# selftok-team/SelftokTokenizer

Measured on AMD Instinct MI355X. Metric: images/sec encode+decode, 256x256 512-token, higher is better.
Workload: dtype f32

## Files before the change

include/selftok_hip_ext.h:

```cpp
#ifndef SELFTOK_HIP_EXT_H
#define SELFTOK_HIP_EXT_H

#include "selftok_hip.h"

#ifdef __cplusplus
extern "C" {
#endif

int selftok_attn_kmask_f32(const selftok_attn_desc* desc, const unsigned* kmask, long kmask_bs, hipStream_t stream);

int selftok_ex_attention_kmask_f32(const float* q, long qs, const float* k1, const float* v1, long kvs1, int Tk1, int valid1, int rows1, const float* k2, const float* v2,
                                   long kvs2, int Tk2, float* out, void* workspace, int B, int H, int Tq, int D, const unsigned* kmask, long kmask_bs, hipStream_t stream);
int selftok_ex_attention_kmask_fused_f32(const float* q, long qs, const float* k1, const float* v1, long kvs1, int Tk1, int valid1, int rows1, const float* k2, const float* v2,
                                         long kvs2, int Tk2, float* out, int B, int H, int Tq, int D, const unsigned* kmask, long kmask_bs, hipStream_t stream);

size_t selftok_img_resize_crop_norm_u8_workspace_bytes(const long* table_host, int B, int S);
int selftok_img_resize_tables_layout(const long* table_host, int B, int S, long* layout4);
int selftok_img_resize_crop_norm_u8(const unsigned char* packed, size_t packed_bytes, const long* table_host, const long* table_dev, int B, int S, void* out,
                                    int out_bf16, const void* lut, void* workspace, size_t workspace_bytes, hipStream_t stream);

size_t selftok_img_views_u8_workspace_bytes(const long* views_host, int V, int S);
int selftok_img_views_tables_layout(const long* views_host, int V, int S, long* layout4);
int selftok_img_views_u8(const unsigned char* packed, size_t packed_bytes, const long* views_host, const long* views_dev, int V, int S, void* out, int out_bf16,
                         const void* lut, void* workspace, size_t workspace_bytes, hipStream_t stream);

size_t selftok_img_views_filter_u8_workspace_bytes(const long* views_host, int V, int S, int filter);
int selftok_img_views_filter_tables_layout(const long* views_host, int V, int S, int filter, long* layout4);
int selftok_img_views_filter_u8(const unsigned char* packed, size_t packed_bytes, const long* views_host, const long* views_dev, int V, int S, int filter, void* out,
                                int out_bf16, const void* lut, void* workspace, size_t workspace_bytes, hipStream_t stream);

size_t selftok_img_resize_u8_workspace_bytes(const long* frames_host, int N, int filter);
int selftok_img_resize_u8(unsigned char* packed, size_t packed_bytes, const long* frames_host, const long* frames_dev, int N, int filter, void* workspace,
                          size_t workspace_bytes, hipStream_t stream);

int selftok_img_to_u8(const void* img, int in_bf16, unsigned char* out, int B, int H, int W, hipStream_t stream);

size_t selftok_img_metrics_workspace_bytes(int B, int H, int W);
int selftok_img_metrics(const void* recon, int recon_bf16, const void* orig, int orig_bf16, int orig_signed, int quantize, const double* window11_host, double* out,
                        void* workspace, size_t workspace_bytes, int B, int H, int W, hipStream_t stream);

size_t selftok_vq_topk_workspace_bytes(int N, int C, int k);
int selftok_vq_topk_packed_f32(const float* z, const float* packed, void* ids, float* scores, void* workspace,
                               int N, int C, int D, int k, int flags, hipStream_t stream);

int selftok_linear_f16_split(const void* a_blk, const void* packed, const float* bias, float* out, void* out_blk, long ldo,
                             int M, int N, int K, int flags, int* overflow, hipStream_t stream);
int selftok_linear_f16_split_residual(const void* a_blk, const void* packed, const float* bias,
                                      const float* resid, long ldr, const float* gate, long gate_stride_b, long gate_stride_t, int T,
                                      float* out, long ldo, int M, int N, int K, int* overflow, hipStream_t stream);

int selftok_linear_f16_split_k(const void* a_blk, const void* packed, const float* bias, float* out, void* out_blk, long ldo,
                               int M, int N, int K, int flags, int ksplit, void* workspace, int* overflow, hipStream_t stream);
int selftok_linear_f16_split_residual_k(const void* a_blk, const void* packed, const float* bias,
                                        const float* resid, long ldr, const float* gate, long gate_stride_b, long gate_stride_t, int T,
                                        float* out, long ldo, int M, int N, int K, int ksplit, void* workspace, int* overflow, hipStream_t stream);

int selftok_attn_f16(const selftok_attn_desc* desc, const unsigned* kmask, long kmask_bs, hipStream_t stream);

size_t selftok_lpips_conv2d_packed_floats(int Cin, int Cout, int KH, int KW);
int selftok_lpips_conv2d_f32(const float* in, const float* packed, const float* bias, float* out, int N, int H, int W, int Cin, int Cout,
                             int KH, int KW, int stride, int pad, int relu, hipStream_t stream);
int selftok_lpips_maxpool3s2_f32(const float* in, float* out, int N, int H, int W, int C, hipStream_t stream);
int selftok_lpips_input(const void* recon, int recon_bf16, const void* orig, int orig_bf16, int orig_signed, int quantize, float* out,
                        int B, int H, int W, hipStream_t stream);
size_t selftok_lpips_distance_workspace_bytes(int B, int npix);
int selftok_lpips_distance(const float* feat, const float* w, double* out, void* workspace, size_t workspace_bytes, int B, int npix, int C,
                           int accumulate, hipStream_t stream);

int selftok_lpips_maxpool2s2_f32(const float* in, float* out, int N, int H, int W, int C, hipStream_t stream);

size_t selftok_img_ssim_workspace_bytes(int B, int H, int W, int taps);
int selftok_img_ssim(const void* recon, int recon_bf16, const void* orig, int orig_bf16, int orig_signed, int quantize, const double* window_host, int taps,
                     double cov_norm, int signed_range, double* out, void* workspace, size_t workspace_bytes, int B, int H, int W, hipStream_t stream);

int selftok_fid_conv2d_f32(const float* in, const float* packed, const float* bias, float* out, int N, int H, int W, int Cin, int Cout,
                           int KH, int KW, int stride, int pad_h, int pad_w, int ldo, int co_off, int relu, hipStream_t stream);
int selftok_fid_pool3_f32(const float* in, float* out, int N, int H, int W, int C, int mode, int ldo, int co_off, hipStream_t stream);
int selftok_fid_input(const void* src, int src_bf16, int src_signed, int quantize, float* out, int B, int H, int W, int OH, int OW,
                      const int* ytab, const int* xtab, hipStream_t stream);
int selftok_fid_spatial_mean_f32(const float* in, float* out, int N, int npix, int C, hipStream_t stream);
size_t selftok_fid_stats_workspace_bytes(int N, int D);
int selftok_fid_stats(const float* x, double* mu, double* sigma, void* workspace, size_t workspace_bytes, int N, int D, hipStream_t stream);

size_t selftok_knn_radius_f32_workspace_bytes(int N, int D, int k);
int selftok_knn_radius_f32(const float* a, float* r2, void* workspace, size_t workspace_bytes, int N, int D, int k, int split, hipStream_t stream);
size_t selftok_manifold_member_f32_workspace_bytes(int M, int N, int D);
int selftok_manifold_member_f32(const float* x, const float* a, const float* r2, int* member, void* workspace, size_t workspace_bytes, int M, int N, int D,
                                int split, hipStream_t stream);
size_t selftok_is_colmean_workspace_bytes(int N, int C, int split_size);
int selftok_is_colmean(const float* logits, double* colmean, void* workspace, size_t workspace_bytes, int N, int C, int split_size, hipStream_t stream);
size_t selftok_is_kl_rows_workspace_bytes(int N, int C, int split_size);
int selftok_is_kl_rows(const float* logits, const double* colmean, double* kl, void* workspace, size_t workspace_bytes, int N, int C, int split_size,
                       hipStream_t stream);

size_t selftok_manifold_count_nn_f32_workspace_bytes(int M, int N, int D);
int selftok_manifold_count_nn_f32(const float* x, const float* a, const float* r2, int* count, float* nn_d2, int* nn_idx, void* workspace, size_t workspace_bytes,
                                  int M, int N, int D, int split, hipStream_t stream);
size_t selftok_kid_sums_f32_workspace_bytes(int S, int m, int D);
int selftok_kid_sums_f32(const float* xs, const float* ys, double* sums, void* workspace, size_t workspace_bytes, int S, int m, int D, hipStream_t stream);

int selftok_stream_prepare(const int* step, const int* limit, const float* coef, const unsigned* pattern_words, const float* mod_table,
                           const float* mod_table_uncond, const int* segs_host, int n_segs, unsigned* kwords_out, float* coef_out,
                           float* mods_out, float* mods_uncond_out, int B, int K, int n_steps, long R, hipStream_t stream);
int selftok_unpatchify_cfg_euler_rows_f32(const float* y_cond, const float* y_uncond, const float* x, float* x_out, const float* coef_rows,
                                          const int* step, int* step_out, int B, int C, int hp, int wp, float cfg_scale, int x0_param,
                                          hipStream_t stream);

#ifdef __cplusplus
}
#endif

#endif
```

selftoktokenizer_amd/_lib.py:

```python
from __future__ import annotations

import ctypes as C
import os

_HERE = os.path.dirname(os.path.abspath(__file__))
LIB_PATH = os.environ.get("SELFTOK_HIP_LIB") or os.path.join(_HERE, "libselftok_hip.so")

_vp, _i, _f, _sz, _l, _d = C.c_void_p, C.c_int, C.c_float, C.c_size_t, C.c_long, C.c_double

SIGNATURES = {
    "selftok_version": (_i, []),
    "selftok_last_error": (C.c_char_p, []),
    "selftok_vq_workspace_bytes": (_sz, [_i, _i]),
    "selftok_vq_encode_f32": (_i, [_vp, _vp, _vp, _vp, _vp, _i, _i, _i, _i, _vp]),
    "selftok_vq_packed_bytes": (_sz, [_i, _i]),
    "selftok_vq_pack_codebook": (_i, [_vp, _vp, _i, _i, _vp]),
    "selftok_vq_encode_packed_f32": (_i, [_vp, _vp, _vp, _vp, _vp, _i, _i, _i, _i, _vp]),
    "selftok_vq_argmax_partial_packed_f32": (_i, [_vp, _vp, _vp, _vp, _i, _i, _i, _i, _vp]),
    "selftok_vq_finalize_packed": (_i, [_vp, _vp, _vp, _vp, _vp, _i, _i, _i, _i, _i, _vp]),
    "selftok_vq_ema_accumulate_f32": (_i, [_vp, _vp, _vp, _vp, _i, _i, _i, _i, _vp]),
    "selftok_vq_tpc_update_f32": (_i, [_vp, _vp, _i, _i, _i, _f, _i, _vp]),
    "selftok_vq_softmax_workspace_bytes": (_sz, [_i]),
    "selftok_vq_softmax_stats_f32": (_i, [_vp, _vp, _vp, _vp, _vp, _i, _i, _i, _i, _f, _i, _vp]),
    "selftok_vq_softmax_backward_f32": (_i, [_vp, _vp, _vp, _vp, _vp, _vp, _i, _i, _i, _i, _f, _i, _vp]),
    "selftok_code_gather_ln_f32": (_i, [_vp, _vp, _vp, _vp, _vp, _i, _i, _i, _f, _i, _vp]),
    "selftok_residual_ln_mod_f32": (_i, [_vp] * 7 + [_i, _i, _i, _l, _l, _l, _l, _f, _vp]),
    "selftok_bias_gelu_f32": (_i, [_vp, _vp, _l, _i, _vp]),
    "selftok_silu_f32": (_i, [_vp, _vp, _l, _vp]),
    "selftok_add_rows_f32": (_i, [_vp, _vp, _vp, _i, _l, _vp]),
    "selftok_timestep_embed_f32": (_i, [_vp, _vp, _vp, _i, _i, _f, _vp]),
    "selftok_patchify_f32": (_i, [_vp, _vp, _i, _i, _i, _i, _vp]),
    "selftok_unpatchify_cfg_euler_f32": (_i, [_vp] * 5 + [_i, _i, _i, _i, _f, _f, _vp]),
    "selftok_rmsnorm_f32": (_i, [_vp, _vp, _vp, _l, _i, _f, _vp]),
    "selftok_rotary_f32": (_i, [_vp, _vp, _vp, _l, _i, _i, _f, _vp]),
    "selftok_attn_f32": (_i, [_vp, _vp]),
    "selftok_residual_ln_mod_split": (_i, [_vp] * 8 + [_i, _i, _i, _l, _l, _l, _l, _f, _vp]),
    "selftok_linear_f16x2_packed_bytes": (_sz, [_i, _i]),
    "selftok_linear_f16x2_pack_weight": (_i, [_vp, _vp, _i, _i, _vp, _vp]),
    "selftok_linear_f16x2_f32": (_i, [_vp, _l, _vp, _vp, _vp, _l, _i, _i, _i, _i, _vp, _vp]),
    "selftok_split_f16x2_bytes": (_sz, [_l, _i]),
    "selftok_split_f16x2_f32": (_i, [_vp, _l, _vp, _l, _i, _vp, _vp]),
    "selftok_linear_f16x2_split": (_i, [_vp, _vp, _vp, _vp, _vp, _l, _i, _i, _i, _i, _vp, _vp]),
    "selftok_linear_f16x2_split_residual": (_i, [_vp, _vp, _vp, _vp, _l, _vp, _l, _l, _i, _vp, _l, _i, _i, _i, _vp, _vp]),
    "selftok_linear_f16x2_splitk_workspace_bytes": (_sz, [_i, _i, _i]),
    "selftok_linear_f16x2_split_k": (_i, [_vp, _vp, _vp, _vp, _vp, _l, _i, _i, _i, _i, _i, _vp, _vp, _vp]),
    "selftok_linear_f16x2_split_residual_k": (_i, [_vp, _vp, _vp, _vp, _l, _vp, _l, _l, _i, _vp, _l, _i, _i, _i, _i, _vp, _vp, _vp]),
    "selftok_groupnorm_silu_bf16": (_i, [_vp, _vp, _vp, _vp, _i, _i, _i, _i, _f, _i, _vp]),
    "selftok_latent_process_in": (_i, [_vp, _vp, _i, _i, _i, _i, _f, _f, _vp]),
    "selftok_latent_process_out": (_i, [_vp, _vp, _l, _f, _f, _vp]),
    "selftok_clamp01_bf16": (_i, [_vp, _l, _vp]),
    "selftok_conv2d_packed_bytes": (_sz, [_i, _i, _i, _i]),
    "selftok_conv2d_pack_weight_bf16": (_i, [_vp, _vp, _i, _i, _i, _i, _vp]),
    "selftok_conv2d_nhwc_bf16": (_i, [_vp, _vp, _vp, _vp, _vp] + [_i] * 11 + [_vp]),
    "selftok_groupnorm_nhwc_workspace_bytes": (_sz, [_i, _i, _i]),
    "selftok_groupnorm_silu_nhwc_bf16": (_i, [_vp, _vp, _vp, _vp, _vp, _i, _i, _i, _i, _f, _i, _vp]),
    "selftok_vx_conv2d_bf16": (_i, [_vp] * 5 + [_i] * 9 + [_vp]),
    "selftok_vx_groupnorm_workspace_bytes": (_sz, [_i, _i, _i]),
    "selftok_vx_groupnorm_bf16": (_i, [_vp] * 7 + [_i, _i, _i, _i, C.c_double, _vp]),
    "selftok_vx_silu_table_bf16": (_i, [_vp, _vp]),
    "selftok_vx_attention_workspace_bytes": (_sz, [_i, _i, _i]),
    "selftok_vx_attention_bf16": (_i, [_vp] * 5 + [_i, _i, _i, _vp]),
    "selftok_vx_expf_f32": (_i, [_vp, _vp, _l, _vp]),
    "selftok_ex_linear_f32": (_i, [_vp, _l, _vp, _vp, _vp, _l, _i, _vp, _l, _i, _vp, _l, _l, _i, _i, _i, _vp]),
    "selftok_linear_f32_workspace_bytes": (_sz, [_l, _i, _i, _i]),
    "selftok_linear_f32": (_i, [_vp, _l, _vp, _vp, _vp, _l, _i, _vp, _l, _i, _vp, _l, _l, _i, _i, _i, _vp, _sz, _vp]),
    "selftok_ex_layernorm_mod_f32": (_i, [_vp, _l, _vp, _l, _vp, _vp, _l, _i, _vp, _vp, _vp, _l, _i, _f, _vp]),
    "selftok_ex_res_layernorm_mod_f32": (_i, [_vp, _l, _vp, _l, _vp, _vp, _l, _i, _vp, _l, _vp, _l, _vp, _vp, _l, _i, _l, _i, _f, _vp]),
    "selftok_ex_unary_f32": (_i, [_vp, _vp, _l, _i, _vp]),
    "selftok_ex_attention_workspace_bytes": (_sz, [_i, _i, _i, _i, _i]),
    "selftok_ex_attention_f32": (_i, [_vp, _l, _vp, _vp, _l, _i, _i, _i, _vp, _vp, _l, _i, _vp, _vp, _i, _i, _i, _i, _vp]),
    "selftok_ex_attention_fused_supported": (_i, [_i, _i, _i]),
    "selftok_ex_attention_fused_f32": (_i, [_vp, _l, _vp, _vp, _l, _i, _i, _i, _vp, _vp, _l, _i, _vp, _i, _i, _i, _i, _vp]),
}


EXT_SIGNATURES = {
    "selftok_attn_kmask_f32": (_i, [_vp, _vp, _l, _vp]),
    "selftok_ex_attention_kmask_f32": (_i, [_vp, _l, _vp, _vp, _l, _i, _i, _i, _vp, _vp, _l, _i, _vp, _vp, _i, _i, _i, _i, _vp, _l, _vp]),
    "selftok_ex_attention_kmask_fused_f32": (_i, [_vp, _l, _vp, _vp, _l, _i, _i, _i, _vp, _vp, _l, _i, _vp, _i, _i, _i, _i, _vp, _l, _vp]),
    "selftok_img_resize_crop_norm_u8_workspace_bytes": (_sz, [_vp, _i, _i]),
    "selftok_img_resize_tables_layout": (_i, [_vp, _i, _i, _vp]),
    "selftok_img_resize_crop_norm_u8": (_i, [_vp, _sz, _vp, _vp, _i, _i, _vp, _i, _vp, _vp, _sz, _vp]),
    "selftok_img_views_u8_workspace_bytes": (_sz, [_vp, _i, _i]),
    "selftok_img_views_tables_layout": (_i, [_vp, _i, _i, _vp]),
    "selftok_img_views_u8": (_i, [_vp, _sz, _vp, _vp, _i, _i, _vp, _i, _vp, _vp, _sz, _vp]),
    "selftok_img_views_filter_u8_workspace_bytes": (_sz, [_vp, _i, _i, _i]),
    "selftok_img_views_filter_tables_layout": (_i, [_vp, _i, _i, _i, _vp]),
    "selftok_img_views_filter_u8": (_i, [_vp, _sz, _vp, _vp, _i, _i, _i, _vp, _i, _vp, _vp, _sz, _vp]),
    "selftok_img_resize_u8_workspace_bytes": (_sz, [_vp, _i, _i]),
    "selftok_img_resize_u8": (_i, [_vp, _sz, _vp, _vp, _i, _i, _vp, _sz, _vp]),
    "selftok_img_to_u8": (_i, [_vp, _i, _vp, _i, _i, _i, _vp]),
    "selftok_img_metrics_workspace_bytes": (_sz, [_i, _i, _i]),
    "selftok_img_metrics": (_i, [_vp, _i, _vp, _i, _i, _i, _vp, _vp, _vp, _sz, _i, _i, _i, _vp]),
    "selftok_vq_topk_workspace_bytes": (_sz, [_i, _i, _i]),
    "selftok_vq_topk_packed_f32": (_i, [_vp, _vp, _vp, _vp, _vp, _i, _i, _i, _i, _i, _vp]),
    "selftok_linear_f16_split": (_i, [_vp, _vp, _vp, _vp, _vp, _l, _i, _i, _i, _i, _vp, _vp]),
    "selftok_linear_f16_split_residual": (_i, [_vp, _vp, _vp, _vp, _l, _vp, _l, _l, _i, _vp, _l, _i, _i, _i, _vp, _vp]),
    "selftok_linear_f16_split_k": (_i, [_vp, _vp, _vp, _vp, _vp, _l, _i, _i, _i, _i, _i, _vp, _vp, _vp]),
    "selftok_linear_f16_split_residual_k": (_i, [_vp, _vp, _vp, _vp, _l, _vp, _l, _l, _i, _vp, _l, _i, _i, _i, _i, _vp, _vp, _vp]),
    "selftok_attn_f16": (_i, [_vp, _vp, _l, _vp]),
    "selftok_lpips_conv2d_packed_floats": (_sz, [_i, _i, _i, _i]),
    "selftok_lpips_conv2d_f32": (_i, [_vp, _vp, _vp, _vp] + [_i] * 10 + [_vp]),
    "selftok_lpips_maxpool3s2_f32": (_i, [_vp, _vp, _i, _i, _i, _i, _vp]),
    "selftok_lpips_input": (_i, [_vp, _i, _vp, _i, _i, _i, _vp, _i, _i, _i, _vp]),
    "selftok_lpips_distance_workspace_bytes": (_sz, [_i, _i]),
    "selftok_lpips_distance": (_i, [_vp, _vp, _vp, _vp, _sz, _i, _i, _i, _i, _vp]),
    "selftok_lpips_maxpool2s2_f32": (_i, [_vp, _vp, _i, _i, _i, _i, _vp]),
    "selftok_img_ssim_workspace_bytes": (_sz, [_i, _i, _i, _i]),
    "selftok_img_ssim": (_i, [_vp, _i, _vp, _i, _i, _i, _vp, _i, _d, _i, _vp, _vp, _sz, _i, _i, _i, _vp]),
    "selftok_fid_conv2d_f32": (_i, [_vp, _vp, _vp, _vp] + [_i] * 13 + [_vp]),
    "selftok_fid_pool3_f32": (_i, [_vp, _vp] + [_i] * 7 + [_vp]),
    "selftok_fid_input": (_i, [_vp, _i, _i, _i, _vp, _i, _i, _i, _i, _i, _vp, _vp, _vp]),
    "selftok_fid_spatial_mean_f32": (_i, [_vp, _vp, _i, _i, _i, _vp]),
    "selftok_fid_stats_workspace_bytes": (_sz, [_i, _i]),
    "selftok_fid_stats": (_i, [_vp, _vp, _vp, _vp, _sz, _i, _i, _vp]),
    "selftok_knn_radius_f32_workspace_bytes": (_sz, [_i, _i, _i]),
    "selftok_knn_radius_f32": (_i, [_vp, _vp, _vp, _sz, _i, _i, _i, _i, _vp]),
    "selftok_manifold_member_f32_workspace_bytes": (_sz, [_i, _i, _i]),
    "selftok_manifold_member_f32": (_i, [_vp, _vp, _vp, _vp, _vp, _sz, _i, _i, _i, _i, _vp]),
    "selftok_is_colmean_workspace_bytes": (_sz, [_i, _i, _i]),
    "selftok_is_colmean": (_i, [_vp, _vp, _vp, _sz, _i, _i, _i, _vp]),
    "selftok_is_kl_rows_workspace_bytes": (_sz, [_i, _i, _i]),
    "selftok_is_kl_rows": (_i, [_vp, _vp, _vp, _vp, _sz, _i, _i, _i, _vp]),
    "selftok_manifold_count_nn_f32_workspace_bytes": (_sz, [_i, _i, _i]),
    "selftok_manifold_count_nn_f32": (_i, [_vp, _vp, _vp, _vp, _vp, _vp, _vp, _sz, _i, _i, _i, _i, _vp]),
    "selftok_kid_sums_f32_workspace_bytes": (_sz, [_i, _i, _i]),
    "selftok_kid_sums_f32": (_i, [_vp, _vp, _vp, _vp, _sz, _i, _i, _i, _vp]),
    "selftok_stream_prepare": (_i, [_vp] * 7 + [_i] + [_vp] * 4 + [_i, _i, _i, _l, _vp]),
    "selftok_unpatchify_cfg_euler_rows_f32": (_i, [_vp] * 7 + [_i, _i, _i, _i, _f, _i, _vp]),
}


class AttnSeg(C.Structure):
    _fields_ = [("q", _vp), ("k", _vp), ("v", _vp), ("o", _vp), ("len", _i),
                ("q_rs", _l), ("k_rs", _l), ("v_rs", _l), ("o_rs", _l),
                ("q_bs", _l), ("k_bs", _l), ("v_bs", _l), ("o_bs", _l)]


class AttnDesc(C.Structure):
    _fields_ = [("seg", AttnSeg * 2), ("B", _i), ("H", _i), ("head_dim", _i), ("kvis", _vp),
                ("seg0_sees_seg1", _i), ("scale", _f), ("mode", _i), ("overflow", _vp),
                ("o_blk", _vp * 2)]

_lib = None


class SelftokHipError(RuntimeError):
    pass


def load():
    global _lib
    if _lib is None:
        if not os.path.exists(LIB_PATH):
            raise SelftokHipError(
                f"{LIB_PATH} not found: build it with `python -c 'import __graft_entry__ as g; g.build()'` "
                "(hipcc --offload-arch=gfx950). There is no CPU fallback.")
        lib = C.CDLL(LIB_PATH)
        for name, (res, args) in list(SIGNATURES.items()) + list(EXT_SIGNATURES.items()):
            fn = getattr(lib, name)
            fn.restype = res
            fn.argtypes = args
        _lib = lib
    return _lib


def check(rc: int, what: str):
    if rc != 0:
        msg = load().selftok_last_error().decode("utf-8", "replace")
        raise SelftokHipError(f"{what} failed (rc={rc}): {msg}")
```

selftoktokenizer_amd/csrc/gemm_f16.hip:

```cpp
#include "common.h"
#include "gemm_split_shared.h"
#include "selftok_hip_ext.h"

namespace selftok {

constexpr int H_A = PA_P;
constexpr int H_W = W_P;
constexpr int H_W_BASE = 2 * H_A;
constexpr int H_STAGE = 2 * (H_A + H_W);
constexpr int H_STAGES = 3;
constexpr int H_LDS_BYTES = H_STAGES * H_STAGE;

template <int ACT, int OSPLIT, int RES>
__global__ __launch_bounds__(512, 2) void linear_f16_pre_kernel(const _Float16* __restrict__ Ablk,
                                                                const _Float16* __restrict__ Wp, const float* __restrict__ bias,
                                                                float* __restrict__ out, _Float16* __restrict__ oblk, long ldo,
                                                                int M, int N, int K, int* __restrict__ overflow, int mblocks, int nblocks, ResArgs res)
{
    static_assert(!(OSPLIT && RES), "the residual form writes fp32");
    __shared__ __attribute__((aligned(16))) unsigned char smem[H_LDS_BYTES];

    const int tid = threadIdx.x, lane = tid & 63, wave = __builtin_amdgcn_readfirstlane(tid >> 6);
    const int wm = wave >> 1, wn = wave & 1;
    const int l31 = lane & 31, lh = lane >> 5;

    int mb, nb;
    tile_of_workgroup(mblocks, nblocks, mb, nb);
    const int m0 = mb * BM, n0 = nb * BN;
    const int KT = K / BK, KL = KT - 1;
    const int NI = (KT + 1) >> 1, IL = NI - 1;

    const int d_g = (lane & 3) ^ ((lane >> 4) & 3);
    const unsigned a_off = (unsigned)((lane >> 2) * 64 + d_g * 16);
    const int rb_last = (M - 1) >> 4;
    int rb0 = m0 / 16 + wave, rb1 = rb0 + 8;
    rb0 = rb0 < rb_last ? rb0 : rb_last;
    rb1 = rb1 < rb_last ? rb1 : rb_last;
    const unsigned char* const a_base[2] = {(const unsigned char*)Ablk + (size_t)rb0 * KT * 2048, (const unsigned char*)Ablk + (size_t)rb1 * KT * 2048};
    const unsigned char* const w_base = (const unsigned char*)Wp + (size_t)nb * KT * W_BYTES + (size_t)wave * 1024;
    const unsigned w_off = lane * 16;
    const unsigned lds0 = (unsigned)(size_t)(__attribute__((address_space(3))) unsigned char*)smem;
    auto dma = [&](int it, int stage) {
        const unsigned dst = lds0 + stage * H_STAGE + wave * 1024;
#pragma unroll
        for (int h = 0; h < 2; ++h) {
            int kt = 2 * it + h;
            kt = kt < KL ? kt : KL;
            lds_dma16(a_base[0] + (size_t)kt * 2048, a_off, dst + h * H_A);
            lds_dma16(a_base[1] + (size_t)kt * 2048, a_off, dst + h * H_A + 8192);
            lds_dma16(w_base + (size_t)kt * W_BYTES, w_off, dst + H_W_BASE + h * H_W);
        }
    };

    f32x16v acc[2][2];
#pragma unroll
    for (int i = 0; i < 2; ++i)
#pragma unroll
        for (int j = 0; j < 2; ++j) acc[i][j] = f32x16v{0, 0, 0, 0, 0, 0, 0, 0, 0, 0, 0, 0, 0, 0, 0, 0};

    const int a_frag = (wm * 64 + l31) * PA_ROW + ((lh ^ ((l31 >> 2) & 3)) * 16);
    const int w_frag = H_W_BASE + lh * W_G + (wn * 64 + l31) * 16;
    f16x8 af[4][2], wf[4][2];
    auto read_frags = [&](int stage) {
#pragma unroll
        for (int q = 0; q < 4; ++q) {
            const unsigned char* sa = smem + stage * H_STAGE + (q >> 1) * H_A + (a_frag ^ ((q & 1) * 32));
            const unsigned char* sw = smem + stage * H_STAGE + (q >> 1) * H_W + w_frag + (q & 1) * 2 * W_G;
#pragma unroll
            for (int b = 0; b < 2; ++b) {
                af[q][b] = *reinterpret_cast<const f16x8*>(sa + b * 32 * PA_ROW);
                wf[q][b] = *reinterpret_cast<const f16x8*>(sw + b * 32 * 16);
            }
        }
    };
    auto mfma_step = [&](int q) {
#pragma unroll
        for (int i = 0; i < 2; ++i)
#pragma unroll
            for (int j = 0; j < 2; ++j) acc[i][j] = __builtin_amdgcn_mfma_f32_32x32x16_f16(wf[q][j], af[q][i], acc[i][j], 0, 0, 0);
    };

    dma(0, 0);
    dma(1, 1);
    __builtin_amdgcn_sched_barrier(0);
    asm volatile("s_waitcnt vmcnt(6)" ::: "memory");
    __builtin_amdgcn_s_barrier();
    __builtin_amdgcn_sched_barrier(0);

    const int grp = wave >> 2;
    if (grp) __builtin_amdgcn_s_barrier();
    if (grp) __builtin_amdgcn_s_setprio(1);
    int sc = 0;
    for (int it = 0; it < NI; ++it) {
        const int s1 = sc == 2 ? 0 : sc + 1, s2 = s1 == 2 ? 0 : s1 + 1;
        __builtin_amdgcn_sched_barrier(0);
        read_frags(sc);
        __builtin_amdgcn_sched_barrier(0);
        dma(it + 2, s2);
        __builtin_amdgcn_sched_barrier(0);
        asm volatile("s_waitcnt vmcnt(6) lgkmcnt(0)" ::: "memory");
        __builtin_amdgcn_s_barrier();
        __builtin_amdgcn_sched_barrier(0);
        mfma_step(0);
        mfma_step(1);
        if (2 * it + 1 < KT) {
            mfma_step(2);
            mfma_step(3);
        }
        __builtin_amdgcn_sched_barrier(0);
        if (!(grp && it == IL)) __builtin_amdgcn_s_barrier();
        sc = s1;
    }
    asm volatile("s_waitcnt vmcnt(0)" ::: "memory");

    constexpr int STG_ROW = OSPLIT ? 144 : 272, STG_PLANE = 64 * STG_ROW;
    static_assert(8 * (OSPLIT ? 2 * STG_PLANE : STG_PLANE) <= H_LDS_BYTES, "epilogue slices exceed the ring");
    unsigned char* stg = smem + wave * (OSPLIT ? 2 * STG_PLANE : STG_PLANE);
    __syncthreads();
    float chk = 0.f;
#pragma unroll
    for (int j = 0; j < 2; ++j) {
#pragma unroll
        for (int g = 0; g < 4; ++g) {
            const int cl = j * 32 + 8 * g + 4 * lh, col = n0 + wn * 64 + cl;
            const float4 bv = bias ? *reinterpret_cast<const float4*>(bias + col) : make_float4(0.f, 0.f, 0.f, 0.f);
#pragma unroll
            for (int i = 0; i < 2; ++i) {
                const int rl = i * 32 + l31, row = m0 + wm * 64 + rl;
                float v[4];
#pragma unroll
                for (int c = 0; c < 4; ++c) {
                    v[c] = acc[i][j][4 * g + c] + 0.f + (c == 0 ? bv.x : c == 1 ? bv.y : c == 2 ? bv.z : bv.w);
                    if (ACT == 1) v[c] = gelu_tanh_f(v[c]);
                }
                if (OSPLIT) {
                    f16x4 h, l;
                    split4(make_float4(opaque_f32(v[0]), opaque_f32(v[1]), opaque_f32(v[2]), opaque_f32(v[3])), h, l);
                    *reinterpret_cast<f16x4*>(stg + rl * STG_ROW + cl * 2) = h;
                    *reinterpret_cast<f16x4*>(stg + STG_PLANE + rl * STG_ROW + cl * 2) = l;
                    if (row < M) {
#pragma unroll
                        for (int c = 0; c < 4; ++c) chk = __builtin_fmaf((float)h[c], 0.f, chk);
                    }
                } else {
                    *reinterpret_cast<float4*>(stg + rl * STG_ROW + cl * 4) = make_float4(v[0], v[1], v[2], v[3]);
                    if (row < M) {
#pragma unroll
                        for (int c = 0; c < 4; ++c) chk = __builtin_fmaf(v[c], 0.f, chk);
                    }
                }
            }
        }
    }
    if (OSPLIT) {
#pragma unroll
        for (int p = 0; p < 2; ++p)
#pragma unroll
            for (int pass = 0; pass < 8; ++pass) {
                const int rl = pass * 8 + (lane >> 3), seg = lane & 7, row = m0 + wm * 64 + rl;
                const f16x8 val = *reinterpret_cast<const f16x8*>(stg + p * STG_PLANE + rl * STG_ROW + seg * 16);
                if (row < M) *reinterpret_cast<f16x8*>(oblk + split_blk_index(row, n0 + wn * 64 + seg * 8, p, N / 32)) = val;
            }
    } else {
#pragma unroll
        for (int pass = 0; pass < 16; ++pass) {
            const int rl = pass * 4 + (lane >> 4), seg = lane & 15, row = m0 + wm * 64 + rl;
            float4 val = *reinterpret_cast<const float4*>(stg + rl * STG_ROW + seg * 16);
            if (row < M) {
                const int col = n0 + wn * 64 + seg * 4;
                if (RES) {
                    const float4 r = *reinterpret_cast<const float4*>(res.resid + (size_t)row * res.ldr + col);
                    if (res.gate) {
                        const int b = row / res.T, t = row - b * res.T;
                        const float4 g = *reinterpret_cast<const float4*>(res.gate + b * res.gsb + t * res.gst + col);
                        val.x = r.x + g.x * val.x; val.y = r.y + g.y * val.y; val.z = r.z + g.z * val.z; val.w = r.w + g.w * val.w;
                    } else {
                        val.x += r.x; val.y += r.y; val.z += r.z; val.w += r.w;
                    }
                }
                *reinterpret_cast<float4*>(out + (size_t)row * ldo + col) = val;
            }
        }
    }
    if (overflow && chk != 0.f) atomicOr(overflow, 1);
}

}

using namespace selftok;

extern "C" {

int selftok_linear_f16_split(const void* a_blk, const void* packed, const float* bias, float* out, void* out_blk, long ldo,
                             int M, int N, int K, int flags, int* overflow, hipStream_t stream)
{
    const int rc = check_split_linear("linear_f16_split", a_blk, packed, bias, out, out_blk, ldo, M, N, K);
    if (rc != SELFTOK_OK || M == 0) return rc;
    const bool osplit = out_blk != nullptr;
    const int mblocks = (M + BM - 1) / BM, nblocks = N / BN;
    const dim3 grid((unsigned)(mblocks * nblocks));
    const _Float16* ab = (const _Float16*)a_blk;
    _Float16* ob = (_Float16*)out_blk;
#define F16_LAUNCH(ACT, OS) hipLaunchKernelGGL((linear_f16_pre_kernel<ACT, OS, 0>), grid, dim3(512), 0, stream, ab, (const _Float16*)packed, bias, out, ob, ldo, M, N, K, overflow, mblocks, nblocks, ResArgs{})
    if (flags & SELFTOK_LINEAR_GELU) { if (osplit) F16_LAUNCH(1, 1); else F16_LAUNCH(1, 0); }
    else { if (osplit) F16_LAUNCH(0, 1); else F16_LAUNCH(0, 0); }
#undef F16_LAUNCH
    return check_launch("linear_f16_pre_kernel");
}

int selftok_linear_f16_split_residual(const void* a_blk, const void* packed, const float* bias,
                                      const float* resid, long ldr, const float* gate, long gate_stride_b, long gate_stride_t, int T,
                                      float* out, long ldo, int M, int N, int K, int* overflow, hipStream_t stream)
{
    const int rc = check_split_linear_residual("linear_f16_split_residual", a_blk, packed, bias, resid, ldr, gate, gate_stride_b, gate_stride_t, T, out, ldo, M, N, K);
    if (rc != SELFTOK_OK || M == 0) return rc;
    const int mblocks = (M + BM - 1) / BM, nblocks = N / BN;
    hipLaunchKernelGGL((linear_f16_pre_kernel<0, 0, 1>), dim3((unsigned)(mblocks * nblocks)), dim3(512), 0, stream,
                       (const _Float16*)a_blk, (const _Float16*)packed, bias, out, (_Float16*)nullptr, ldo,
                       M, N, K, overflow, mblocks, nblocks, ResArgs{resid, ldr, gate, gate_stride_b, gate_stride_t, T});
    return check_launch("linear_f16_pre_kernel(residual)");
}

}
```

selftoktokenizer_amd/csrc/gemm_f16_splitk.hip:

```cpp
#include "common.h"
#include "gemm_split_shared.h"
#include "selftok_hip_ext.h"

namespace selftok {

constexpr int HK_A = PA_P;
constexpr int HK_W = W_P;
constexpr int HK_W_BASE = 2 * HK_A;
constexpr int HK_STAGE = 2 * (HK_A + HK_W);
constexpr int HK_LDS_BYTES = 3 * HK_STAGE;

__global__ __launch_bounds__(512, 2) void linear_f16_splitk_partial_kernel(const _Float16* __restrict__ Ablk, const _Float16* __restrict__ Wp,
                                                                           float* __restrict__ ws, int M, int N, int K,
                                                                           int* __restrict__ overflow, int mblocks, int nblocks)
{
    __shared__ __attribute__((aligned(16))) unsigned char smem[HK_LDS_BYTES];

    const int tid = threadIdx.x, lane = tid & 63, wave = __builtin_amdgcn_readfirstlane(tid >> 6);
    const int wm = wave >> 1, wn = wave & 1;
    const int l31 = lane & 31, lh = lane >> 5;

    int mb, nb;
    tile_of_workgroup(mblocks, nblocks, mb, nb);
    const int m0 = mb * BM, n0 = nb * BN;
    const int KTA = K / BK;
    const int KT = KTA / (int)gridDim.y, KL = KT - 1;
    const int kt_off = (int)blockIdx.y * KT;
    const int NI = (KT + 1) >> 1, IL = NI - 1;
    float* const out = ws + (size_t)blockIdx.y * M * N;

    const int d_g = (lane & 3) ^ ((lane >> 4) & 3);
    const unsigned a_off = (unsigned)((lane >> 2) * 64 + d_g * 16);
    const int rb_last = (M - 1) >> 4;
    int rb0 = m0 / 16 + wave, rb1 = rb0 + 8;
    rb0 = rb0 < rb_last ? rb0 : rb_last;
    rb1 = rb1 < rb_last ? rb1 : rb_last;
    const unsigned char* const a_base[2] = {(const unsigned char*)Ablk + ((size_t)rb0 * KTA + kt_off) * 2048,
                                            (const unsigned char*)Ablk + ((size_t)rb1 * KTA + kt_off) * 2048};
    const unsigned char* const w_base = (const unsigned char*)Wp + ((size_t)nb * KTA + kt_off) * W_BYTES + (size_t)wave * 1024;
    const unsigned w_off = lane * 16;
    const unsigned lds0 = (unsigned)(size_t)(__attribute__((address_space(3))) unsigned char*)smem;
    auto dma = [&](int it, int stage) {
        const unsigned dst = lds0 + stage * HK_STAGE + wave * 1024;
#pragma unroll
        for (int h = 0; h < 2; ++h) {
            int kt = 2 * it + h;
            kt = kt < KL ? kt : KL;
            lds_dma16(a_base[0] + (size_t)kt * 2048, a_off, dst + h * HK_A);
            lds_dma16(a_base[1] + (size_t)kt * 2048, a_off, dst + h * HK_A + 8192);
            lds_dma16(w_base + (size_t)kt * W_BYTES, w_off, dst + HK_W_BASE + h * HK_W);
        }
    };

    f32x16v acc[2][2];
#pragma unroll
    for (int i = 0; i < 2; ++i)
#pragma unroll
        for (int j = 0; j < 2; ++j) acc[i][j] = f32x16v{0, 0, 0, 0, 0, 0, 0, 0, 0, 0, 0, 0, 0, 0, 0, 0};

    const int a_frag = (wm * 64 + l31) * PA_ROW + ((lh ^ ((l31 >> 2) & 3)) * 16);
    const int w_frag = HK_W_BASE + lh * W_G + (wn * 64 + l31) * 16;
    f16x8 af[4][2], wf[4][2];
    auto read_frags = [&](int stage) {
#pragma unroll
        for (int q = 0; q < 4; ++q) {
            const unsigned char* sa = smem + stage * HK_STAGE + (q >> 1) * HK_A + (a_frag ^ ((q & 1) * 32));
            const unsigned char* sw = smem + stage * HK_STAGE + (q >> 1) * HK_W + w_frag + (q & 1) * 2 * W_G;
#pragma unroll
            for (int b = 0; b < 2; ++b) {
                af[q][b] = *reinterpret_cast<const f16x8*>(sa + b * 32 * PA_ROW);
                wf[q][b] = *reinterpret_cast<const f16x8*>(sw + b * 32 * 16);
            }
        }
    };
    auto mfma_step = [&](int q) {
#pragma unroll
        for (int i = 0; i < 2; ++i)
#pragma unroll
            for (int j = 0; j < 2; ++j) acc[i][j] = __builtin_amdgcn_mfma_f32_32x32x16_f16(wf[q][j], af[q][i], acc[i][j], 0, 0, 0);
    };

    dma(0, 0);
    dma(1, 1);
    __builtin_amdgcn_sched_barrier(0);
    asm volatile("s_waitcnt vmcnt(6)" ::: "memory");
    __builtin_amdgcn_s_barrier();
    __builtin_amdgcn_sched_barrier(0);

    const int grp = wave >> 2;
    if (grp) __builtin_amdgcn_s_barrier();
    if (grp) __builtin_amdgcn_s_setprio(1);
    int sc = 0;
    for (int it = 0; it < NI; ++it) {
        const int s1 = sc == 2 ? 0 : sc + 1, s2 = s1 == 2 ? 0 : s1 + 1;
        __builtin_amdgcn_sched_barrier(0);
        read_frags(sc);
        __builtin_amdgcn_sched_barrier(0);
        dma(it + 2, s2);
        __builtin_amdgcn_sched_barrier(0);
        asm volatile("s_waitcnt vmcnt(6) lgkmcnt(0)" ::: "memory");
        __builtin_amdgcn_s_barrier();
        __builtin_amdgcn_sched_barrier(0);
        mfma_step(0);
        mfma_step(1);
        if (2 * it + 1 < KT) {
            mfma_step(2);
            mfma_step(3);
        }
        __builtin_amdgcn_sched_barrier(0);
        if (!(grp && it == IL)) __builtin_amdgcn_s_barrier();
        sc = s1;
    }
    asm volatile("s_waitcnt vmcnt(0)" ::: "memory");

    constexpr int STG_ROW = 272, STG_PLANE = 64 * STG_ROW;
    static_assert(8 * STG_PLANE <= HK_LDS_BYTES, "store slices exceed the ring");
    unsigned char* stg = smem + wave * STG_PLANE;
    __syncthreads();
    float chk = 0.f;
#pragma unroll
    for (int j = 0; j < 2; ++j) {
#pragma unroll
        for (int g = 0; g < 4; ++g) {
            const int cl = j * 32 + 8 * g + 4 * lh;
#pragma unroll
            for (int i = 0; i < 2; ++i) {
                const int rl = i * 32 + l31, row = m0 + wm * 64 + rl;
                float v[4];
#pragma unroll
                for (int c = 0; c < 4; ++c) v[c] = acc[i][j][4 * g + c] + 0.f + 0.f;
                *reinterpret_cast<float4*>(stg + rl * STG_ROW + cl * 4) = make_float4(v[0], v[1], v[2], v[3]);
                if (row < M) {
#pragma unroll
                    for (int c = 0; c < 4; ++c) chk = __builtin_fmaf(v[c], 0.f, chk);
                }
            }
        }
    }
#pragma unroll
    for (int pass = 0; pass < 16; ++pass) {
        const int rl = pass * 4 + (lane >> 4), seg = lane & 15, row = m0 + wm * 64 + rl;
        const float4 val = *reinterpret_cast<const float4*>(stg + rl * STG_ROW + seg * 16);
        if (row < M) *reinterpret_cast<float4*>(out + (size_t)row * N + n0 + wn * 64 + seg * 4) = val;
    }
    if (overflow && chk != 0.f) atomicOr(overflow, 1);
}

static int launch_f16_partials(const void* a_blk, const void* packed, float* ws, int M, int N, int K, int ksplit, int* overflow, hipStream_t stream)
{
    const int mblocks = (M + BM - 1) / BM, nblocks = N / BN;
    hipLaunchKernelGGL(linear_f16_splitk_partial_kernel, dim3((unsigned)(mblocks * nblocks), (unsigned)ksplit), dim3(512), 0, stream,
                       (const _Float16*)a_blk, (const _Float16*)packed, ws, M, N, K, overflow, mblocks, nblocks);
    return check_launch("linear_f16_splitk_partial_kernel");
}

}

using namespace selftok;

extern "C" {

int selftok_linear_f16_split_k(const void* a_blk, const void* packed, const float* bias, float* out, void* out_blk, long ldo,
                               int M, int N, int K, int flags, int ksplit, void* workspace, int* overflow, hipStream_t stream)
{
    if (ksplit == 1) return selftok_linear_f16_split(a_blk, packed, bias, out, out_blk, ldo, M, N, K, flags, overflow, stream);
    int rc = check_split_linear("linear_f16_split_k", a_blk, packed, bias, out, out_blk, ldo, M, N, K);
    if (rc != SELFTOK_OK || M == 0) return rc;
    if ((rc = check_splitk("linear_f16_split_k", K, ksplit, workspace))) return rc;
    float* ws = (float*)workspace;
    if ((rc = launch_f16_partials(a_blk, packed, ws, M, N, K, ksplit, overflow, stream))) return rc;
    return launch_splitk_finish(ws, ksplit, bias, out, out_blk, ldo, M, N, flags, overflow, nullptr, stream);
}

int selftok_linear_f16_split_residual_k(const void* a_blk, const void* packed, const float* bias,
                                        const float* resid, long ldr, const float* gate, long gate_stride_b, long gate_stride_t, int T,
                                        float* out, long ldo, int M, int N, int K, int ksplit, void* workspace, int* overflow, hipStream_t stream)
{
    if (ksplit == 1)
        return selftok_linear_f16_split_residual(a_blk, packed, bias, resid, ldr, gate, gate_stride_b, gate_stride_t, T, out, ldo, M, N, K, overflow, stream);
    int rc = check_split_linear_residual("linear_f16_split_residual_k", a_blk, packed, bias, resid, ldr, gate, gate_stride_b, gate_stride_t, T, out, ldo, M, N, K);
    if (rc != SELFTOK_OK || M == 0) return rc;
    if ((rc = check_splitk("linear_f16_split_residual_k", K, ksplit, workspace))) return rc;
    float* ws = (float*)workspace;
    if ((rc = launch_f16_partials(a_blk, packed, ws, M, N, K, ksplit, overflow, stream))) return rc;
    const ResArgs res{resid, ldr, gate, gate_stride_b, gate_stride_t, T};
    return launch_splitk_finish(ws, ksplit, bias, out, nullptr, ldo, M, N, 0, overflow, &res, stream);
}

}
```

selftoktokenizer_amd/csrc/gemm_split.hip:

```cpp
#include "common.h"
#include "gemm_split_shared.h"
#include "selftok_hip.h"
#include <stdlib.h>

namespace selftok {

constexpr int A_G = BM * 16 + 32;
constexpr int A_P = 4 * A_G;
constexpr int A_BYTES = 2 * A_P;
constexpr int A_STAGES = 2;
constexpr int W_STAGES = 5;
constexpr int W_AHEAD = 3;
constexpr int W_BASE = A_STAGES * A_BYTES;
constexpr int LDS_BYTES = W_BASE + W_STAGES * W_BYTES;

__global__ __launch_bounds__(256) void pack_weight_kernel(const float* __restrict__ W, _Float16* __restrict__ packed, int N, int K, int* __restrict__ overflow)
{
    const long idx = (long)blockIdx.x * blockDim.x + threadIdx.x;
    const int KG = K / 8;
    if (idx >= (long)N * KG) return;
    const int n = (int)(idx / KG), kg = (int)(idx % KG);
    const float4 v0 = *reinterpret_cast<const float4*>(W + (size_t)n * K + kg * 8);
    const float4 v1 = *reinterpret_cast<const float4*>(W + (size_t)n * K + kg * 8 + 4);
    f16x4 h0, l0, h1, l1;
    float mx = 0.f;
    split4(v0, h0, l0, mx);
    split4(v1, h1, l1, mx);
    const int nb = n / BN, nl = n % BN, kt = kg / 4, g = kg % 4, KT = K / BK;
    _Float16* tile = packed + ((size_t)nb * KT + kt) * (W_BYTES / 2);
    f16x8 hi = {h0[0], h0[1], h0[2], h0[3], h1[0], h1[1], h1[2], h1[3]};
    f16x8 lo = {l0[0], l0[1], l0[2], l0[3], l1[0], l1[1], l1[2], l1[3]};
    *reinterpret_cast<f16x8*>(tile + (size_t)g * (W_G / 2) + nl * 8) = hi;
    *reinterpret_cast<f16x8*>(tile + (W_P / 2) + (size_t)g * (W_G / 2) + nl * 8) = lo;
    if (!(mx < F16_MAX) && overflow) atomicOr(overflow, 2);
}

template <int ACT, int ABL = 0>
__global__ __launch_bounds__(512, 2) void linear_f16x2_kernel(const float* __restrict__ A, long lda, const _Float16* __restrict__ Wp,
                                                              const float* __restrict__ bias, float* __restrict__ out, long ldo,
                                                              int M, int N, int K, int* __restrict__ overflow, int mblocks, int nblocks)
{
    __shared__ __attribute__((aligned(16))) unsigned char smem[LDS_BYTES];

    const int tid = threadIdx.x, lane = tid & 63, wave = tid >> 6;
    const int wm = wave >> 1, wn = wave & 1;
    const int l31 = lane & 31, lh = lane >> 5;

    int mb, nb;
    tile_of_workgroup(mblocks, nblocks, mb, nb);
    const int m0 = mb * BM, n0 = nb * BN;
    const int KT = K / BK, KL = KT - 1;

    const int a_q = tid & 7, a_r = tid >> 3;
    const float* a_src[4];
#pragma unroll
    for (int i = 0; i < 4; ++i) {
        int row = m0 + a_r + 64 * i;
        row = row < M ? row : M - 1;
        a_src[i] = A + (size_t)row * lda + 4 * a_q;
    }
    const int a_dst = (a_q >> 1) * A_G + a_r * 16 + (a_q & 1) * 8;
    const _Float16* w_src = Wp + (size_t)nb * KT * (W_BYTES / 2) + (size_t)wave * 512 + lane * 8;

    f32x4v preA[4], preB[4];
    auto load_a = [&](f32x4v (&pre)[4], int kt) {
        kt = kt < KL ? kt : KL;
#pragma unroll
        for (int i = 0; i < 4; ++i) {
            const float* p = a_src[i] + (size_t)kt * BK;
            asm volatile("global_load_dwordx4 %0, %1, off" : "=v"(pre[i]) : "v"(p) : "memory");
        }
    };
    auto wait_rows = [&](f32x4v (&pre)[4]) {
        if (ABL & 6) asm volatile("s_waitcnt vmcnt(0)" : "+v"(pre[0]), "+v"(pre[1]), "+v"(pre[2]), "+v"(pre[3])::"memory");
        else asm volatile("s_waitcnt vmcnt(6)" : "+v"(pre[0]), "+v"(pre[1]), "+v"(pre[2]), "+v"(pre[3])::"memory");
    };
    auto dma_w = [&](int kt, int stage) {
        kt = kt < KL ? kt : KL;
        const _Float16* src = w_src + (size_t)kt * (W_BYTES / 2);
        unsigned char* dst = smem + W_BASE + stage * W_BYTES + wave * 1024;
        __builtin_amdgcn_global_load_lds((const __attribute__((address_space(1))) void*)src,
                                         (__attribute__((address_space(3))) void*)dst, 16, 0, 0);
        __builtin_amdgcn_global_load_lds((const __attribute__((address_space(1))) void*)(src + 8 * 512),
                                         (__attribute__((address_space(3))) void*)(dst + 8 * 1024), 16, 0, 0);
    };
    auto write_a = [&](f32x4v (&pre)[4], int stage) {
        unsigned char* base = smem + stage * A_BYTES + a_dst;
#pragma unroll
        for (int i = 0; i < 4; ++i) {
            f16x4 h, l;
            split4(pre[i], h, l);
            *reinterpret_cast<f16x4*>(base + i * 64 * 16) = h;
            *reinterpret_cast<f16x4*>(base + i * 64 * 16 + A_P) = l;
        }
    };

    f32x16v hi[2][2], lo[2][2];
#pragma unroll
    for (int i = 0; i < 2; ++i)
#pragma unroll
        for (int j = 0; j < 2; ++j) {
            hi[i][j] = f32x16v{0, 0, 0, 0, 0, 0, 0, 0, 0, 0, 0, 0, 0, 0, 0, 0};
            lo[i][j] = hi[i][j];
        }

    const int a_frag = lh * A_G + (wm * 64 + l31) * 16;
    const int w_frag = W_BASE + lh * W_G + (wn * 64 + l31) * 16;
    f16x8 af0[2][2], wf0[2][2], af1[2][2], wf1[2][2];
    auto read_frags = [&](f16x8 (&af)[2][2], f16x8 (&wf)[2][2], int a_stage, int w_stage, int s) {
        const unsigned char* sa = smem + a_stage * A_BYTES + a_frag + s * 2 * A_G;
        const unsigned char* sw = smem + w_stage * W_BYTES + w_frag + s * 2 * W_G;
#pragma unroll
        for (int b = 0; b < 2; ++b)
#pragma unroll
            for (int p = 0; p < 2; ++p) {
                af[b][p] = *reinterpret_cast<const f16x8*>(sa + b * 32 * 16 + p * A_P);
                wf[b][p] = *reinterpret_cast<const f16x8*>(sw + b * 32 * 16 + p * W_P);
            }
    };
    auto mfma_row = [&](int i, f16x8 (&af)[2][2], f16x8 (&wf)[2][2]) {
#pragma unroll
            for (int j = 0; j < 2; ++j) {
                hi[i][j] = __builtin_amdgcn_mfma_f32_32x32x16_f16(af[i][0], wf[j][0], hi[i][j], 0, 0, 0);
                lo[i][j] = __builtin_amdgcn_mfma_f32_32x32x16_f16(af[i][0], wf[j][1], lo[i][j], 0, 0, 0);
                lo[i][j] = __builtin_amdgcn_mfma_f32_32x32x16_f16(af[i][1], wf[j][0], lo[i][j], 0, 0, 0);
            }
    };

    auto iteration = [&](int kt, f32x4v (&pre)[4], int ws_cur, int ws_next, int ws_new) {
        const int as = kt & 1;
        if (!(ABL & 16)) read_frags(af1, wf1, as, ws_cur, 1);
        if (!(ABL & 8)) mfma_row(0, af0, wf0);
        __builtin_amdgcn_sched_barrier(0);
        wait_rows(pre);
        if (!(ABL & 1)) write_a(pre, as ^ 1);
        if (!(ABL & 8)) mfma_row(1, af0, wf0);
        __builtin_amdgcn_sched_barrier(0);
        asm volatile("s_waitcnt lgkmcnt(0)" ::: "memory");
        __builtin_amdgcn_s_barrier();
        __builtin_amdgcn_sched_barrier(0);
        if (!(ABL & 8)) mfma_row(0, af1, wf1);
        __builtin_amdgcn_sched_barrier(0);
        if (!(ABL & 16)) read_frags(af0, wf0, as ^ 1, ws_next, 0);
        if (!(ABL & 4)) dma_w(kt + W_AHEAD, ws_new);
        __builtin_amdgcn_sched_barrier(0);
        if (!(ABL & 2)) load_a(pre, kt + 3);
        if (!(ABL & 8)) mfma_row(1, af1, wf1);
        __builtin_amdgcn_sched_barrier(0);
    };

    dma_w(0, 0);
    load_a(preA, 0);
    asm volatile("s_waitcnt vmcnt(0)" : "+v"(preA[0]), "+v"(preA[1]), "+v"(preA[2]), "+v"(preA[3])::"memory");
    __builtin_amdgcn_sched_barrier(0);
    write_a(preA, 0);
    __builtin_amdgcn_sched_barrier(0);
    dma_w(1, 1);
    __builtin_amdgcn_sched_barrier(0);
    load_a(preB, 1);
    __builtin_amdgcn_sched_barrier(0);
    dma_w(2, 2);
    __builtin_amdgcn_sched_barrier(0);
    load_a(preA, 2);
    __builtin_amdgcn_sched_barrier(0);
    asm volatile("s_waitcnt lgkmcnt(0)" ::: "memory");
    __builtin_amdgcn_s_barrier();
    read_frags(af0, wf0, 0, 0, 0);

    auto ring = [](int x) { return x >= W_STAGES ? x - W_STAGES : x; };
    int wc = 0;
    int kt = 0;
    for (; kt + 1 < KT; kt += 2) {
        iteration(kt, preB, wc, ring(wc + 1), ring(wc + W_AHEAD));
        wc = ring(wc + 1);
        iteration(kt + 1, preA, wc, ring(wc + 1), ring(wc + W_AHEAD));
        wc = ring(wc + 1);
    }
    if (kt < KT) iteration(kt, preB, wc, ring(wc + 1), ring(wc + W_AHEAD));
    asm volatile("s_waitcnt vmcnt(0)" : "+v"(preA[0]), "+v"(preA[1]), "+v"(preA[2]), "+v"(preA[3]), "+v"(preB[0]), "+v"(preB[1]), "+v"(preB[2]), "+v"(preB[3])::"memory");

    float chk = 0.f;
#pragma unroll
    for (int j = 0; j < 2; ++j) {
        const int col = n0 + wn * 64 + j * 32 + l31;
        const float bv = bias ? bias[col] : 0.f;
#pragma unroll
        for (int i = 0; i < 2; ++i) {
            const int rbase = m0 + wm * 64 + i * 32 + 4 * lh;
#pragma unroll
            for (int r = 0; r < 16; ++r) {
                const int row = rbase + (r & 3) + 8 * (r >> 2);
                float v = hi[i][j][r] + lo[i][j][r] * LO_INV + bv;
                if (ACT == 1) v = gelu_tanh_f(v);
                if (row < M) { out[(size_t)row * ldo + col] = v; chk = __builtin_fmaf(v, 0.f, chk); }
            }
        }
    }
    if (overflow && chk != 0.f) atomicOr(overflow, 1);
}

constexpr int PA_BYTES = 2 * PA_P;
constexpr int PA_STAGES = 3, PW_STAGES = 4;
constexpr int PW_BASE = PA_STAGES * PA_BYTES;
constexpr int P_LDS_BYTES = PW_BASE + PW_STAGES * W_BYTES;

template <int ACT, int OSPLIT, int PP = 1, int ABL = 0, int RES = 0, int SK = 0>
__global__ __launch_bounds__(512, 2) void linear_f16x2_pre_kernel(const _Float16* __restrict__ Ablk,
                                                                  const _Float16* __restrict__ Wp, const float* __restrict__ bias,
                                                                  float* __restrict__ out, _Float16* __restrict__ oblk, long ldo,
                                                                  int M, int N, int K, int* __restrict__ overflow, int mblocks, int nblocks, ResArgs res)
{
    static_assert(!SK || (ACT == 0 && OSPLIT == 0 && RES == 0), "a split-K partial has no epilogue");
    __shared__ __attribute__((aligned(16))) unsigned char smem[P_LDS_BYTES];
    unsigned long long tk0 = 0, tk1 = 0, tk2 = 0, rt0 = 0;
    if (ABL & 2048) { tk0 = __builtin_readcyclecounter(); rt0 = __builtin_amdgcn_s_memrealtime(); }

    const int tid = threadIdx.x, lane = tid & 63, wave = __builtin_amdgcn_readfirstlane(tid >> 6);
    const int wm = wave >> 1, wn = wave & 1;
    const int l31 = lane & 31, lh = lane >> 5;

    int mb, nb;
    tile_of_workgroup(mblocks, nblocks, mb, nb);
    const int m0 = mb * BM, n0 = nb * BN;
    const int KTA = K / BK;
    const int KT = SK ? KTA / (int)gridDim.y : KTA, KL = KT - 1;
    const int kt_off = SK ? (int)blockIdx.y * KT : 0;
    if (SK) out += (size_t)blockIdx.y * M * ldo;

    const int d_g = (lane & 3) ^ ((lane >> 4) & 3);
    const unsigned a_off = (unsigned)((lane >> 2) * 64 + d_g * 16);
    const int rb_last = (M - 1) >> 4;
    int rb0 = m0 / 16 + wave, rb1 = rb0 + 8;
    rb0 = rb0 < rb_last ? rb0 : rb_last;
    rb1 = rb1 < rb_last ? rb1 : rb_last;
    const unsigned char* const a_base[2] = {(const unsigned char*)Ablk + ((size_t)rb0 * KTA + kt_off) * 2048, (const unsigned char*)Ablk + ((size_t)rb1 * KTA + kt_off) * 2048};
    const unsigned char* const w_base = (const unsigned char*)(Wp + ((size_t)nb * KTA + kt_off) * (W_BYTES / 2) + (size_t)wave * 512);
    const unsigned w_off = lane * 16;
    const unsigned lds0 = (unsigned)(size_t)(__attribute__((address_space(3))) unsigned char*)smem;
    auto dma_a = [&](int kt, int stage) {
        kt = kt < KL ? kt : KL;
        const unsigned dst = lds0 + stage * PA_BYTES + wave * 1024;
#pragma unroll
        for (int j = 0; j < 4; ++j) lds_dma16(a_base[j & 1] + (size_t)kt * 2048 + (j >> 1) * 1024, a_off, dst + (j & 1) * 8192 + (j >> 1) * PA_P);
    };
    auto dma_w = [&](int kt, int stage) {
        kt = kt < KL ? kt : KL;
        const unsigned char* src = w_base + (size_t)kt * W_BYTES;
        const unsigned dst = lds0 + PW_BASE + stage * W_BYTES + wave * 1024;
        lds_dma16(src, w_off, dst);
        lds_dma16(src + 8 * 1024, w_off, dst + 8 * 1024);
    };

    f32x16v hi[2][2], lo[2][2];
#pragma unroll
    for (int i = 0; i < 2; ++i)
#pragma unroll
        for (int j = 0; j < 2; ++j) {
            hi[i][j] = f32x16v{0, 0, 0, 0, 0, 0, 0, 0, 0, 0, 0, 0, 0, 0, 0, 0};
            lo[i][j] = hi[i][j];
        }

    const int a_frag = (wm * 64 + l31) * PA_ROW + ((lh ^ ((l31 >> 2) & 3)) * 16);
    const int w_frag = PW_BASE + lh * W_G + (wn * 64 + l31) * 16;
    f16x8 af0[2][2], wf0[2][2], af1[2][2], wf1[2][2];
    auto read_frags = [&](f16x8 (&af)[2][2], f16x8 (&wf)[2][2], int a_stage, int w_stage, int s) {
        const unsigned char* sa = smem + a_stage * PA_BYTES + (a_frag ^ (s * 32));
        const unsigned char* sw = smem + w_stage * W_BYTES + w_frag + s * 2 * W_G;
#pragma unroll
        for (int b = 0; b < 2; ++b)
#pragma unroll
            for (int p = 0; p < 2; ++p) {
                af[b][p] = *reinterpret_cast<const f16x8*>(sa + b * 32 * PA_ROW + p * PA_P);
                wf[b][p] = *reinterpret_cast<const f16x8*>(sw + b * 32 * 16 + p * W_P);
            }
    };
    auto mfma_row = [&](int i, f16x8 (&af)[2][2], f16x8 (&wf)[2][2]) {
#pragma unroll
            for (int j = 0; j < 2; ++j) {
                hi[i][j] = __builtin_amdgcn_mfma_f32_32x32x16_f16(wf[j][0], af[i][0], hi[i][j], 0, 0, 0);
                lo[i][j] = __builtin_amdgcn_mfma_f32_32x32x16_f16(wf[j][1], af[i][0], lo[i][j], 0, 0, 0);
                lo[i][j] = __builtin_amdgcn_mfma_f32_32x32x16_f16(wf[j][0], af[i][1], lo[i][j], 0, 0, 0);
            }
    };

    auto iteration = [&](int kt, int a_cur, int a_next, int a_new, int w_cur, int w_next, int w_new) {
        dma_a(kt + 2, a_new);
        dma_w(kt + 3, w_new);
        __builtin_amdgcn_sched_barrier(0);
        read_frags(af1, wf1, a_cur, w_cur, 1);
        mfma_row(0, af0, wf0);
        mfma_row(1, af0, wf0);
        __builtin_amdgcn_sched_barrier(0);
        asm volatile("s_waitcnt vmcnt(8) lgkmcnt(0)" ::: "memory");
        __builtin_amdgcn_s_barrier();
        __builtin_amdgcn_sched_barrier(0);
        mfma_row(0, af1, wf1);
        __builtin_amdgcn_sched_barrier(0);
        read_frags(af0, wf0, a_next, w_next, 0);
        mfma_row(1, af1, wf1);
        __builtin_amdgcn_sched_barrier(0);
    };

    dma_a(0, 0);
    dma_w(0, 0);
    dma_w(1, 1);
    dma_a(1, 1);
    dma_w(2, 2);
    __builtin_amdgcn_sched_barrier(0);
    asm volatile("s_waitcnt vmcnt(8)" ::: "memory");
    __builtin_amdgcn_s_barrier();
    __builtin_amdgcn_sched_barrier(0);

    int ac = 0, wc = 0;
    if (PP == 0) {
        read_frags(af0, wf0, 0, 0, 0);
        for (int kt = 0; kt < KT; ++kt) {
            const int a1 = ac == 2 ? 0 : ac + 1, a2 = a1 == 2 ? 0 : a1 + 1;
            iteration(kt, ac, a1, a2, wc, (wc + 1) & 3, (wc + 3) & 3);
            ac = a1;
            wc = (wc + 1) & 3;
        }
    } else {
        const int grp = wave >> 2;
        if (ABL & 2048) tk1 = __builtin_readcyclecounter();
        if (grp) __builtin_amdgcn_s_barrier();
        if (!(ABL & 64) && grp) __builtin_amdgcn_s_setprio(1);
        unsigned long long t0 = 0, t1 = 0, t2 = 0, t3 = 0, t4 = 0;
        unsigned acc_reads = 0, acc_vm = 0, acc_bar1 = 0, acc_mfma = 0, acc_bar2 = 0;
#define STAMP(t) do { if (ABL & 2048) { __builtin_amdgcn_sched_barrier(0); t = __builtin_readcyclecounter(); __builtin_amdgcn_sched_barrier(0); } } while (0)
        for (int kt = 0; kt < KT; ++kt) {
            const int a1 = ac == 2 ? 0 : ac + 1, a2 = a1 == 2 ? 0 : a1 + 1;
            STAMP(t0);
            if ((ABL & 2048) && kt > 0) acc_bar2 += (unsigned)(t0 - t4);
            __builtin_amdgcn_sched_barrier(0);
            if (!(ABL & 16)) {
                read_frags(af0, wf0, ac, wc, 0);
                read_frags(af1, wf1, ac, wc, 1);
            }
            __builtin_amdgcn_sched_barrier(0);
            if (!(ABL & 1)) dma_a(kt + 2, a2);
            if (!(ABL & 4)) dma_w(kt + 3, (wc + 3) & 3);
            __builtin_amdgcn_sched_barrier(0);
            if (ABL & 2048) {
                asm volatile("s_waitcnt lgkmcnt(0)" ::: "memory");
                STAMP(t1);
            }
            if (ABL & 5) asm volatile("s_waitcnt vmcnt(0) lgkmcnt(0)" ::: "memory");
            else asm volatile("s_waitcnt vmcnt(8) lgkmcnt(0)" ::: "memory");
            STAMP(t2);
            if (!(ABL & 32)) __builtin_amdgcn_s_barrier();
            STAMP(t3);
            __builtin_amdgcn_sched_barrier(0);
            if (!(ABL & 8)) {
                mfma_row(0, af0, wf0);
                mfma_row(1, af0, wf0);
                mfma_row(0, af1, wf1);
                mfma_row(1, af1, wf1);
            }
            __builtin_amdgcn_sched_barrier(0);
            STAMP(t4);
            if (ABL & 2048) { acc_reads += (unsigned)(t1 - t0); acc_vm += (unsigned)(t2 - t1); acc_bar1 += (unsigned)(t3 - t2); acc_mfma += (unsigned)(t4 - t3); }
            if (!(ABL & 32) && !(grp && kt == KL)) __builtin_amdgcn_s_barrier();
            ac = a1;
            wc = (wc + 1) & 3;
        }
#undef STAMP
        if (ABL & 2048) tk2 = __builtin_readcyclecounter();
        if ((ABL & 2048) && blockIdx.x == gridDim.x / 2 && lane == 0) {
            float* dbg = const_cast<float*>(bias) + N + wave * 8;
            dbg[0] = (float)acc_reads / KT; dbg[1] = (float)acc_vm / KT; dbg[2] = (float)acc_bar1 / KT;
            dbg[3] = (float)acc_mfma / KT; dbg[4] = (float)acc_bar2 / (KT - 1);
            dbg[5] = (float)(tk1 - tk0); dbg[6] = (float)(tk2 - tk1);
        }
    }
    asm volatile("s_waitcnt vmcnt(0)" ::: "memory");

    constexpr int STG_ROW = OSPLIT ? 144 : 272, STG_PLANE = 64 * STG_ROW;
    unsigned char* stg = smem + wave * (OSPLIT ? 2 * STG_PLANE : STG_PLANE);
    __syncthreads();
    float chk = 0.f;
#pragma unroll
    for (int j = 0; j < 2; ++j) {
#pragma unroll
        for (int g = 0; g < 4; ++g) {
            const int cl = j * 32 + 8 * g + 4 * lh, col = n0 + wn * 64 + cl;
            const float4 bv = bias ? *reinterpret_cast<const float4*>(bias + col) : make_float4(0.f, 0.f, 0.f, 0.f);
#pragma unroll
            for (int i = 0; i < 2; ++i) {
                const int rl = i * 32 + l31, row = m0 + wm * 64 + rl;
                float v[4];
#pragma unroll
                for (int c = 0; c < 4; ++c) {
                    v[c] = hi[i][j][4 * g + c] + lo[i][j][4 * g + c] * LO_INV + (c == 0 ? bv.x : c == 1 ? bv.y : c == 2 ? bv.z : bv.w);
                    if (ACT == 1) v[c] = gelu_tanh_f(v[c]);
                }
                if (OSPLIT) {
                    f16x4 h, l;
                    split4(make_float4(opaque_f32(v[0]), opaque_f32(v[1]), opaque_f32(v[2]), opaque_f32(v[3])), h, l);
                    *reinterpret_cast<f16x4*>(stg + rl * STG_ROW + cl * 2) = h;
                    *reinterpret_cast<f16x4*>(stg + STG_PLANE + rl * STG_ROW + cl * 2) = l;
                    if (row < M) {
#pragma unroll
                        for (int c = 0; c < 4; ++c) chk = __builtin_fmaf((float)h[c], 0.f, chk);
                    }
                } else {
                    *reinterpret_cast<float4*>(stg + rl * STG_ROW + cl * 4) = make_float4(v[0], v[1], v[2], v[3]);
                    if (row < M) {
#pragma unroll
                        for (int c = 0; c < 4; ++c) chk = __builtin_fmaf(v[c], 0.f, chk);
                    }
                }
            }
        }
    }
    if (OSPLIT) {
#pragma unroll
        for (int p = 0; p < 2; ++p)
#pragma unroll
            for (int pass = 0; pass < 8; ++pass) {
                const int rl = pass * 8 + (lane >> 3), seg = lane & 7, row = m0 + wm * 64 + rl;
                const f16x8 val = *reinterpret_cast<const f16x8*>(stg + p * STG_PLANE + rl * STG_ROW + seg * 16);
                if (row < M) *reinterpret_cast<f16x8*>(oblk + split_blk_index(row, n0 + wn * 64 + seg * 8, p, N / 32)) = val;
            }
    } else {
#pragma unroll
        for (int pass = 0; pass < 16; ++pass) {
            const int rl = pass * 4 + (lane >> 4), seg = lane & 15, row = m0 + wm * 64 + rl;
            float4 val = *reinterpret_cast<const float4*>(stg + rl * STG_ROW + seg * 16);
            if (row < M) {
                const int col = n0 + wn * 64 + seg * 4;
                if (RES) {
                    const float4 r = *reinterpret_cast<const float4*>(res.resid + (size_t)row * res.ldr + col);
                    if (res.gate) {
                        const int b = row / res.T, t = row - b * res.T;
                        const float4 g = *reinterpret_cast<const float4*>(res.gate + b * res.gsb + t * res.gst + col);
                        val.x = r.x + g.x * val.x; val.y = r.y + g.y * val.y; val.z = r.z + g.z * val.z; val.w = r.w + g.w * val.w;
                    } else {
                        val.x += r.x; val.y += r.y; val.z += r.z; val.w += r.w;
                    }
                }
                *reinterpret_cast<float4*>(out + (size_t)row * ldo + col) = val;
            }
        }
    }
    if (overflow && chk != 0.f) atomicOr(overflow, 1);
    if ((ABL & 2048) && blockIdx.x == gridDim.x / 2 && lane == 0) {
        asm volatile("s_waitcnt vmcnt(0)" ::: "memory");
        const_cast<float*>(bias)[N + wave * 8 + 7] = (float)(__builtin_readcyclecounter() - tk2);
    }
    if ((ABL & 2048) && overflow && tid == 0) {
        asm volatile("s_waitcnt vmcnt(0)" ::: "memory");
        int* rec = overflow + 8 + (size_t)blockIdx.x * 8;
        const unsigned long long rt1 = __builtin_amdgcn_s_memrealtime(), tk3 = __builtin_readcyclecounter();
        rec[0] = (int)(unsigned)rt0; rec[1] = (int)(unsigned)rt1; rec[2] = (int)(unsigned)(tk3 - tk0);
        rec[3] = (int)__builtin_amdgcn_s_getreg((31 << 11) | 4); rec[4] = (int)__builtin_amdgcn_s_getreg((31 << 11) | 20);
    }
}

__global__ __launch_bounds__(256) void split_rows_kernel(const float* __restrict__ x, long ld, _Float16* __restrict__ blk,
                                                         long rows, int cols, int* __restrict__ overflow)
{
    const long idx = (long)blockIdx.x * blockDim.x + threadIdx.x;
    const int c4 = cols / 4;
    if (idx >= rows * c4) return;
    const long r = idx / c4;
    const int c = (int)(idx % c4) * 4;
    const float4 v = *reinterpret_cast<const float4*>(x + r * ld + c);
    f16x4 h, l;
    float mx = 0.f;
    split4(v, h, l, mx);
    *reinterpret_cast<f16x4*>(blk + split_blk_index(r, c, 0, cols / 32)) = h;
    *reinterpret_cast<f16x4*>(blk + split_blk_index(r, c, 1, cols / 32)) = l;
    if (!(mx < F16_MAX) && overflow) atomicOr(overflow, 1);
}

template <int ACT, int OSPLIT, int RES>
__global__ __launch_bounds__(256) void splitk_finish_kernel(const float* __restrict__ ws, int S, const float* __restrict__ bias,
                                                            float* __restrict__ out, _Float16* __restrict__ oblk, long ldo,
                                                            int M, int N, int* __restrict__ overflow, ResArgs res)
{
    const long idx = (long)blockIdx.x * blockDim.x + threadIdx.x;
    const int n8 = N >> 3;
    if (idx >= (long)M * n8) return;
    const int row = (int)(idx / n8), col = (int)(idx - (long)row * n8) << 3;
    const float* p = ws + (size_t)row * N + col;
    const size_t plane = (size_t)M * N;
    float4 a = *reinterpret_cast<const float4*>(p), b = *reinterpret_cast<const float4*>(p + 4);
    for (int s_ = 1; s_ < S; ++s_) {
        const float4 c = *reinterpret_cast<const float4*>(p + s_ * plane), d = *reinterpret_cast<const float4*>(p + s_ * plane + 4);
        a.x += c.x; a.y += c.y; a.z += c.z; a.w += c.w;
        b.x += d.x; b.y += d.y; b.z += d.z; b.w += d.w;
    }
    float v[8] = {a.x, a.y, a.z, a.w, b.x, b.y, b.z, b.w};
    if (bias) {
        const float4 b0 = *reinterpret_cast<const float4*>(bias + col), b1 = *reinterpret_cast<const float4*>(bias + col + 4);
        v[0] += b0.x; v[1] += b0.y; v[2] += b0.z; v[3] += b0.w; v[4] += b1.x; v[5] += b1.y; v[6] += b1.z; v[7] += b1.w;
    }
    if (ACT == 1) {
#pragma unroll
        for (int c = 0; c < 8; ++c) v[c] = gelu_tanh_f(v[c]);
    }
    float chk = 0.f;
    if (OSPLIT) {
        f16x4 h0, l0, h1, l1;
        split4(make_float4(opaque_f32(v[0]), opaque_f32(v[1]), opaque_f32(v[2]), opaque_f32(v[3])), h0, l0);
        split4(make_float4(opaque_f32(v[4]), opaque_f32(v[5]), opaque_f32(v[6]), opaque_f32(v[7])), h1, l1);
        const f16x8 h = {h0[0], h0[1], h0[2], h0[3], h1[0], h1[1], h1[2], h1[3]}, l = {l0[0], l0[1], l0[2], l0[3], l1[0], l1[1], l1[2], l1[3]};
#pragma unroll
        for (int c = 0; c < 8; ++c) chk = __builtin_fmaf((float)h[c], 0.f, chk);
        *reinterpret_cast<f16x8*>(oblk + split_blk_index(row, col, 0, N / 32)) = h;
        *reinterpret_cast<f16x8*>(oblk + split_blk_index(row, col, 1, N / 32)) = l;
    } else {
#pragma unroll
        for (int c = 0; c < 8; ++c) chk = __builtin_fmaf(v[c], 0.f, chk);
        if (RES) {
            const float* rp = res.resid + (size_t)row * res.ldr + col;
            const float4 r0 = *reinterpret_cast<const float4*>(rp), r1 = *reinterpret_cast<const float4*>(rp + 4);
            const float r[8] = {r0.x, r0.y, r0.z, r0.w, r1.x, r1.y, r1.z, r1.w};
            if (res.gate) {
                const int bb = row / res.T, t = row - bb * res.T;
                const float* gp = res.gate + bb * res.gsb + t * res.gst + col;
                const float4 g0 = *reinterpret_cast<const float4*>(gp), g1 = *reinterpret_cast<const float4*>(gp + 4);
                const float g[8] = {g0.x, g0.y, g0.z, g0.w, g1.x, g1.y, g1.z, g1.w};
#pragma unroll
                for (int c = 0; c < 8; ++c) v[c] = r[c] + g[c] * v[c];
            } else {
#pragma unroll
                for (int c = 0; c < 8; ++c) v[c] += r[c];
            }
        }
        float* op = out + (size_t)row * ldo + col;
        *reinterpret_cast<float4*>(op) = make_float4(v[0], v[1], v[2], v[3]);
        *reinterpret_cast<float4*>(op + 4) = make_float4(v[4], v[5], v[6], v[7]);
    }
    if (overflow && chk != 0.f) atomicOr(overflow, 1);
}

static int launch_splitk_partials(const void* a_blk, const void* packed, float* ws, int M, int N, int K, int ksplit, int* overflow, hipStream_t stream)
{
    const int mblocks = (M + BM - 1) / BM, nblocks = N / BN;
    hipLaunchKernelGGL((linear_f16x2_pre_kernel<0, 0, 1, 0, 0, 1>), dim3((unsigned)(mblocks * nblocks), (unsigned)ksplit), dim3(512), 0, stream,
                       (const _Float16*)a_blk, (const _Float16*)packed, (const float*)nullptr, ws, (_Float16*)nullptr, (long)N,
                       M, N, K, overflow, mblocks, nblocks, ResArgs{});
    return check_launch("linear_f16x2_pre_kernel(split-K partials)");
}

}

using namespace selftok;

extern "C" {

size_t selftok_linear_f16x2_packed_bytes(int N, int K)
{
    if (N <= 0 || K <= 0 || N % BN || K % BK) return 0;
    return (size_t)N * K * 4;
}

int selftok_linear_f16x2_pack_weight(const float* W, void* packed, int N, int K, int* overflow, hipStream_t stream)
{
    if (!W || !packed || N <= 0 || K <= 0 || N % BN || K % BK) { set_last_error("linear_f16x2_pack_weight: need N % 128 == 0 and K % 32 == 0"); return SELFTOK_EINVAL; }
    const long n = (long)N * (K / 8);
    hipLaunchKernelGGL(pack_weight_kernel, dim3((unsigned)((n + 255) / 256)), dim3(256), 0, stream, W, (_Float16*)packed, N, K, overflow);
    return check_launch("pack_weight_kernel");
}

int selftok_linear_f16x2_f32(const float* A, long lda, const void* packed, const float* bias, float* out, long ldo,
                             int M, int N, int K, int flags, int* overflow, hipStream_t stream)
{
    if (M < 0 || N <= 0 || K <= 0 || N % BN || K % BK) { set_last_error("linear_f16x2: need N % 128 == 0 and K % 32 == 0"); return SELFTOK_EINVAL; }
    if (M == 0) return SELFTOK_OK;
    if (!A || !packed || !out || lda < K || ldo < N || (lda & 3)) { set_last_error("linear_f16x2: bad pointers/strides (lda % 4 == 0, lda >= K, ldo >= N)"); return SELFTOK_EINVAL; }
    const int mblocks = (M + BM - 1) / BM, nblocks = N / BN;
    const dim3 grid((unsigned)(mblocks * nblocks));
#ifdef SELFTOK_GEMM_ABLATE
    {
        const char* e = getenv("SELFTOK_GEMM_ABL");
        const int abl = e ? atoi(e) : 0;
#define ABL_CASE(v) if (abl == v) { hipLaunchKernelGGL((linear_f16x2_kernel<0, v>), grid, dim3(512), 0, stream, A, lda, (const _Float16*)packed, bias, out, ldo, M, N, K, overflow, mblocks, nblocks); return check_launch("linear_f16x2_kernel(ablated)"); }
        ABL_CASE(1) ABL_CASE(2) ABL_CASE(3) ABL_CASE(4) ABL_CASE(7) ABL_CASE(8) ABL_CASE(16) ABL_CASE(24) ABL_CASE(23) ABL_CASE(31)
#undef ABL_CASE
    }
#endif
    if (flags & SELFTOK_LINEAR_GELU)
        hipLaunchKernelGGL(linear_f16x2_kernel<1>, grid, dim3(512), 0, stream, A, lda, (const _Float16*)packed, bias, out, ldo, M, N, K, overflow, mblocks, nblocks);
    else
        hipLaunchKernelGGL(linear_f16x2_kernel<0>, grid, dim3(512), 0, stream, A, lda, (const _Float16*)packed, bias, out, ldo, M, N, K, overflow, mblocks, nblocks);
    return check_launch("linear_f16x2_kernel");
}

size_t selftok_split_f16x2_bytes(long rows, int cols)
{
    if (rows < 0 || cols <= 0 || cols % 32) return 0;
    return (size_t)((rows + 15) / 16) * 16 * cols * 4;
}

int selftok_split_f16x2_f32(const float* x, long ld, void* blk, long rows, int cols, int* overflow, hipStream_t stream)
{
    if (rows < 0 || cols <= 0 || (cols & 31) || (ld & 3) || ld < cols) { set_last_error("split_f16x2: cols % 32 == 0, ld % 4 == 0, ld >= cols"); return SELFTOK_EINVAL; }
    if (rows == 0) return SELFTOK_OK;
    if (!x || !blk || ((size_t)blk & 15) || ((size_t)x & 15)) { set_last_error("split_f16x2: null / unaligned pointer"); return SELFTOK_EINVAL; }
    const long n = rows * (cols / 4);
    hipLaunchKernelGGL(split_rows_kernel, dim3((unsigned)((n + 255) / 256)), dim3(256), 0, stream, x, ld, (_Float16*)blk, rows, cols, overflow);
    return check_launch("split_rows_kernel");
}

int selftok_linear_f16x2_split(const void* a_blk, const void* packed, const float* bias, float* out, void* out_blk, long ldo,
                               int M, int N, int K, int flags, int* overflow, hipStream_t stream)
{
    const int rc = check_split_linear("linear_f16x2_split", a_blk, packed, bias, out, out_blk, ldo, M, N, K);
    if (rc != SELFTOK_OK || M == 0) return rc;
    const bool osplit = out_blk != nullptr;
    const int mblocks = (M + BM - 1) / BM, nblocks = N / BN;
    const dim3 grid((unsigned)(mblocks * nblocks));
    const _Float16* ab = (const _Float16*)a_blk;
    _Float16* ob = (_Float16*)out_blk;
#ifdef SELFTOK_GEMM_ABLATE
    {
        const char* e = getenv("SELFTOK_GEMM_ABL");
        const int abl = e ? atoi(e) : 0;
#define PRE_ABL(pp, v) if (abl == (pp ? v : 1000 + v)) { hipLaunchKernelGGL((linear_f16x2_pre_kernel<0, 0, pp, v>), grid, dim3(512), 0, stream, ab, (const _Float16*)packed, bias, out, ob, ldo, M, N, K, overflow, mblocks, nblocks, ResArgs{}); return check_launch("linear_f16x2_pre_kernel(ablated)"); }
        PRE_ABL(0, 0) PRE_ABL(1, 1) PRE_ABL(1, 4) PRE_ABL(1, 5) PRE_ABL(1, 8) PRE_ABL(1, 16) PRE_ABL(1, 21) PRE_ABL(1, 24) PRE_ABL(1, 32) PRE_ABL(1, 64) PRE_ABL(1, 13) PRE_ABL(1, 37) PRE_ABL(1, 2048)
#undef PRE_ABL
    }
#endif
#define PRE_LAUNCH(ACT, OS) hipLaunchKernelGGL((linear_f16x2_pre_kernel<ACT, OS>), grid, dim3(512), 0, stream, ab, (const _Float16*)packed, bias, out, ob, ldo, M, N, K, overflow, mblocks, nblocks, ResArgs{})
    if (flags & SELFTOK_LINEAR_GELU) { if (osplit) PRE_LAUNCH(1, 1); else PRE_LAUNCH(1, 0); }
    else { if (osplit) PRE_LAUNCH(0, 1); else PRE_LAUNCH(0, 0); }
#undef PRE_LAUNCH
    return check_launch("linear_f16x2_pre_kernel");
}

int selftok_linear_f16x2_split_residual(const void* a_blk, const void* packed, const float* bias,
                                        const float* resid, long ldr, const float* gate, long gate_stride_b, long gate_stride_t, int T,
                                        float* out, long ldo, int M, int N, int K, int* overflow, hipStream_t stream)
{
    const int rc = check_split_linear_residual("linear_f16x2_split_residual", a_blk, packed, bias, resid, ldr, gate, gate_stride_b, gate_stride_t, T, out, ldo, M, N, K);
    if (rc != SELFTOK_OK || M == 0) return rc;
    const int mblocks = (M + BM - 1) / BM, nblocks = N / BN;
    hipLaunchKernelGGL((linear_f16x2_pre_kernel<0, 0, 1, 0, 1>), dim3((unsigned)(mblocks * nblocks)), dim3(512), 0, stream,
                       (const _Float16*)a_blk, (const _Float16*)packed, bias, out, (_Float16*)nullptr, ldo,
                       M, N, K, overflow, mblocks, nblocks, ResArgs{resid, ldr, gate, gate_stride_b, gate_stride_t, T});
    return check_launch("linear_f16x2_pre_kernel(residual)");
}

}

int selftok::launch_splitk_finish(const float* ws, int ksplit, const float* bias, float* out, void* out_blk, long ldo, int M, int N, int flags,
                                  int* overflow, const ResArgs* res, hipStream_t stream)
{
    const long n = (long)M * (N / 8);
    const dim3 grid((unsigned)((n + 255) / 256));
    if (!res) {
        const bool osplit = out_blk != nullptr;
        _Float16* ob = (_Float16*)out_blk;
#define FIN_LAUNCH(ACT, OS) hipLaunchKernelGGL((splitk_finish_kernel<ACT, OS, 0>), grid, dim3(256), 0, stream, ws, ksplit, bias, out, ob, ldo, M, N, overflow, ResArgs{})
        if (flags & SELFTOK_LINEAR_GELU) { if (osplit) FIN_LAUNCH(1, 1); else FIN_LAUNCH(1, 0); }
        else { if (osplit) FIN_LAUNCH(0, 1); else FIN_LAUNCH(0, 0); }
#undef FIN_LAUNCH
        return check_launch("splitk_finish_kernel");
    }
    hipLaunchKernelGGL((splitk_finish_kernel<0, 0, 1>), grid, dim3(256), 0, stream, ws, ksplit, bias, out, (_Float16*)nullptr, ldo, M, N, overflow, *res);
    return check_launch("splitk_finish_kernel(residual)");
}

extern "C" {

size_t selftok_linear_f16x2_splitk_workspace_bytes(int M, int N, int ksplit)
{
    if (M <= 0 || N <= 0 || ksplit <= 1) return 0;
    return (size_t)ksplit * M * N * sizeof(float);
}

int selftok_linear_f16x2_split_k(const void* a_blk, const void* packed, const float* bias, float* out, void* out_blk, long ldo,
                                 int M, int N, int K, int flags, int ksplit, void* workspace, int* overflow, hipStream_t stream)
{
    if (ksplit == 1) return selftok_linear_f16x2_split(a_blk, packed, bias, out, out_blk, ldo, M, N, K, flags, overflow, stream);
    int rc = check_split_linear("linear_f16x2_split_k", a_blk, packed, bias, out, out_blk, ldo, M, N, K);
    if (rc != SELFTOK_OK || M == 0) return rc;
    if ((rc = check_splitk("linear_f16x2_split_k", K, ksplit, workspace))) return rc;
    float* ws = (float*)workspace;
    if (int rc = launch_splitk_partials(a_blk, packed, ws, M, N, K, ksplit, overflow, stream)) return rc;
    return launch_splitk_finish(ws, ksplit, bias, out, out_blk, ldo, M, N, flags, overflow, nullptr, stream);
}

int selftok_linear_f16x2_split_residual_k(const void* a_blk, const void* packed, const float* bias,
                                          const float* resid, long ldr, const float* gate, long gate_stride_b, long gate_stride_t, int T,
                                          float* out, long ldo, int M, int N, int K, int ksplit, void* workspace, int* overflow, hipStream_t stream)
{
    if (ksplit == 1)
        return selftok_linear_f16x2_split_residual(a_blk, packed, bias, resid, ldr, gate, gate_stride_b, gate_stride_t, T, out, ldo, M, N, K, overflow, stream);
    int rc = check_split_linear_residual("linear_f16x2_split_residual_k", a_blk, packed, bias, resid, ldr, gate, gate_stride_b, gate_stride_t, T, out, ldo, M, N, K);
    if (rc != SELFTOK_OK || M == 0) return rc;
    if ((rc = check_splitk("linear_f16x2_split_residual_k", K, ksplit, workspace))) return rc;
    float* ws = (float*)workspace;
    if (int rc = launch_splitk_partials(a_blk, packed, ws, M, N, K, ksplit, overflow, stream)) return rc;
    const ResArgs res{resid, ldr, gate, gate_stride_b, gate_stride_t, T};
    return launch_splitk_finish(ws, ksplit, bias, out, nullptr, ldo, M, N, 0, overflow, &res, stream);
}

}
```

selftoktokenizer_amd/csrc/gemm_split_shared.h:

```cpp
#pragma once
#include "common.h"
#include <stdio.h>

namespace selftok {

typedef _Float16 f16x8 __attribute__((ext_vector_type(8)));
typedef _Float16 f16x4 __attribute__((ext_vector_type(4)));
typedef float f32x16v __attribute__((ext_vector_type(16)));
typedef float f32x4v __attribute__((ext_vector_type(4)));

constexpr int BM = 256, BN = 128, BK = 32;
constexpr float LO_SCALE = 2048.0f, LO_INV = 1.0f / 2048.0f;
constexpr float F16_MAX = 65504.0f;

constexpr int W_G = BN * 16;
constexpr int W_P = 4 * W_G;
constexpr int W_BYTES = 2 * W_P;
constexpr int GROUP_M = 4;

__device__ __forceinline__ void tile_of_workgroup(int mblocks, int nblocks, int& mb, int& nb)
{
    const int T = gridDim.x, orig = blockIdx.x;
    const int q8 = T >> 3, r8 = T & 7, xcd = orig & 7, idx = orig >> 3;
    const int w = (xcd < r8 ? xcd * (q8 + 1) : r8 * (q8 + 1) + (xcd - r8) * q8) + idx;
    const int per_group = GROUP_M * nblocks;
    const int group = w / per_group, first_m = group * GROUP_M;
    const int gsz = (mblocks - first_m) < GROUP_M ? (mblocks - first_m) : GROUP_M;
    const int in = w - group * per_group;
    mb = first_m + in % gsz;
    nb = in / gsz;
}

__device__ __forceinline__ float gelu_tanh_f(float x)
{
    const float k0 = 0.7978845608028654f, k1 = 0.044715f;
    const float u = k0 * (x + k1 * x * x * x);
    const float e = __builtin_amdgcn_exp2f(u * (-2.0f * 1.4426950408889634f));
    return x * __builtin_amdgcn_rcpf(1.0f + e);
}

typedef float f32x2v __attribute__((ext_vector_type(2)));
typedef _Float16 f16x2 __attribute__((ext_vector_type(2)));

template <typename V4>
__device__ __forceinline__ void split4(const V4& v, f16x4& hi, f16x4& lo)
{
    const f32x2v a = {v.x, v.y}, b = {v.z, v.w};
    const f16x2 ha = __builtin_convertvector(a, f16x2), hb = __builtin_convertvector(b, f16x2);
    const f32x2v ra = (a - __builtin_convertvector(ha, f32x2v)) * LO_SCALE;
    const f32x2v rb = (b - __builtin_convertvector(hb, f32x2v)) * LO_SCALE;
    const f16x2 la = __builtin_convertvector(ra, f16x2), lb = __builtin_convertvector(rb, f16x2);
    hi[0] = ha[0]; hi[1] = ha[1]; hi[2] = hb[0]; hi[3] = hb[1];
    lo[0] = la[0]; lo[1] = la[1]; lo[2] = lb[0]; lo[3] = lb[1];
}
template <typename V4>
__device__ __forceinline__ void split4(const V4& v, f16x4& hi, f16x4& lo, float& mx)
{
    split4(v, hi, lo);
    mx = fmaxf(mx, fmaxf(fmaxf(fabsf(v.x), fabsf(v.y)), fmaxf(fabsf(v.z), fabsf(v.w))));
}

constexpr int PA_ROW = 64;
constexpr int PA_P = BM * PA_ROW;

__device__ __forceinline__ void lds_dma16(const void* base, unsigned voff, unsigned lds)
{
    asm volatile("s_mov_b32 m0, %2\n\ts_nop 0\n\tglobal_load_lds_dwordx4 %0, %1" ::"v"(voff), "s"(base), "s"(lds) : "memory", "m0");
}

struct ResArgs { const float* resid; long ldr; const float* gate; long gsb, gst; int T; };

inline int refuse_args(const char* who, const char* what)
{
    char msg[256];
    snprintf(msg, sizeof msg, "%s: %s", who, what);
    set_last_error(msg);
    return SELFTOK_EINVAL;
}

inline int check_split_linear(const char* who, const void* a_blk, const void* packed, const float* bias, const float* out, const void* out_blk,
                              long ldo, int M, int N, int K)
{
    if (M < 0 || N <= 0 || K <= 0 || N % BN || K % BK) return refuse_args(who, "need N % 128 == 0 and K % 32 == 0");
    if (M == 0) return SELFTOK_OK;
    if (!a_blk || !packed || ((size_t)a_blk & 15) || ((size_t)out & 15) || ((size_t)out_blk & 15) || (bias && ((size_t)bias & 15))
        || (out_blk ? out != nullptr : (!out || ldo < N || (ldo & 3))))
        return refuse_args(who, "bad pointers/strides (a_blk, out, out_blk and bias 16-byte aligned; either out with ldo % 4 == 0, ldo >= N, or out_blk)");
    return SELFTOK_OK;
}

inline int check_split_linear_residual(const char* who, const void* a_blk, const void* packed, const float* bias, const float* resid, long ldr,
                                       const float* gate, long gate_stride_b, long gate_stride_t, int T, const float* out, long ldo,
                                       int M, int N, int K)
{
    if (int rc = check_split_linear(who, a_blk, packed, bias, out, nullptr, ldo, M, N, K)) return rc;
    if (M == 0) return SELFTOK_OK;
    if (!resid || ldr < N || (ldr & 3) || T <= 0 || ((size_t)resid & 15)
        || (gate && (((size_t)gate & 15) || (gate_stride_b & 3) || (gate_stride_t & 3))))
        return refuse_args(who, "bad residual arguments (resid and gate 16-byte aligned, ldr >= N, ldr and the gate strides multiples of 4, T > 0)");
    return SELFTOK_OK;
}

inline int check_splitk(const char* who, int K, int ksplit, const void* workspace)
{
    if (ksplit >= 2 && ksplit <= 64 && (K / BK) % ksplit == 0 && workspace && !((size_t)workspace & 15)) return SELFTOK_OK;
    return refuse_args(who, "ksplit not in 2..64 / not a divisor of K / 32, or no 16-byte aligned workspace");
}

int launch_splitk_finish(const float* ws, int ksplit, const float* bias, float* out, void* out_blk, long ldo, int M, int N, int flags,
                         int* overflow, const ResArgs* res, hipStream_t stream);

}
```

selftoktokenizer_amd/ops.py:

```python
from __future__ import annotations

import functools
from typing import Optional

import torch

from . import _lib

IDS_I32 = 1
PRENORMED = 2
VQ_F16COARSE = 8
VQ_F16COARSE1 = 16
VQ_DEFAULT_COARSE = True
VQ_COARSE_MFMAS = 1


def _coarse_flags(coarse) -> int:
    if coarse is None:
        coarse = VQ_DEFAULT_COARSE
    if coarse is False or coarse == 0:
        return 0
    n = VQ_COARSE_MFMAS if coarse is True else int(coarse)
    if n not in (1, 3):
        raise ValueError(f"coarse = {coarse!r}: expected None, False, True, 1 or 3")
    return VQ_F16COARSE | (VQ_F16COARSE1 if n == 1 else 0)
VQ_EVENTS = None


def _stream():
    return torch.cuda.current_stream().cuda_stream


def _need_cuda(*ts):
    cur = None
    for t in ts:
        if t is None:
            continue
        if not t.is_cuda:
            raise _lib.SelftokHipError("selftok HIP ops need device tensors (there is no CPU fallback)")
        if cur is None:
            cur = torch.cuda.current_device()
        if t.device.index != cur:
            raise _lib.SelftokHipError(f"tensor on {t.device} but the current device is cuda:{cur}: "
                                       "call torch.cuda.set_device / use `with torch.cuda.device(...)` first")


def _p(t):
    return None if t is None else t.data_ptr()


def vq_pack_codebook(codebook: torch.Tensor) -> torch.Tensor:
    _need_cuda(codebook)
    cb = codebook.contiguous().float()
    C, D = cb.shape
    lib = _lib.load()
    packed = torch.zeros(lib.selftok_vq_packed_bytes(C, D) // 4, dtype=torch.float32, device=cb.device)
    _lib.check(lib.selftok_vq_pack_codebook(_p(cb), _p(packed), C, D, _stream()), "selftok_vq_pack_codebook")
    return packed


def packed_codes(packed: torch.Tensor, D: int = 16) -> int:
    return (packed.numel() - 64) // (2 * D)


def vq_encode(z: torch.Tensor, codebook: torch.Tensor, *, packed: bool = False, return_best: bool = False,
              ids_dtype=torch.int64, prenormed: bool = False, rt: int = 0, split: int = 0, coarse=None):
    _need_cuda(z, codebook)
    lib = _lib.load()
    cflags = _coarse_flags(coarse) if packed else 0
    if packed and VQ_EVENTS is not None and not return_best and not prenormed and z.numel() > 0:
        ids, launch_main, launch_fin = vq_encode_split_launch(z, codebook, ids_dtype, _flags=cflags)
        e0, e1, e2 = (torch.cuda.Event(enable_timing=True) for _ in range(3))
        e0.record()
        launch_main()
        e1.record()
        launch_fin()
        e2.record()
        VQ_EVENTS.append((e0, e1, e2))
        return ids
    zz = z.contiguous().float().reshape(-1, z.shape[-1])
    N, D = zz.shape
    C = packed_codes(codebook, D) if packed else codebook.shape[0]
    ids = torch.empty(N, dtype=ids_dtype, device=z.device)
    best = torch.empty(N, dtype=torch.float32, device=z.device) if return_best else None
    ws = torch.empty(lib.selftok_vq_workspace_bytes(N, C), dtype=torch.uint8, device=z.device)
    flags = ((IDS_I32 if ids_dtype == torch.int32 else 0) | (PRENORMED if prenormed else 0) | ((rt & 0xF) << 8) | ((split & 0xFF) << 16)
             | cflags)
    fn = lib.selftok_vq_encode_packed_f32 if packed else lib.selftok_vq_encode_f32
    _lib.check(fn(_p(zz), _p(codebook), _p(ids), _p(best), _p(ws), N, C, D, flags, _stream()),
               "selftok_vq_encode_packed_f32" if packed else "selftok_vq_encode_f32")
    ids = ids.reshape(z.shape[:-1])
    if return_best:
        return ids, best.reshape(z.shape[:-1])
    return ids


def vq_topk(z: torch.Tensor, packed_codebook: torch.Tensor, k: int, ids_dtype=torch.int64, prenormed: bool = False, *, rt: int = 0, split: int = 0):
    _need_cuda(z, packed_codebook)
    if ids_dtype not in (torch.int64, torch.int32):
        raise TypeError(f"ids_dtype must be torch.int64 or torch.int32, got {ids_dtype}")
    lib = _lib.load()
    k = int(k)
    zz = z.contiguous().float().reshape(-1, z.shape[-1])
    N, D = zz.shape
    C = packed_codes(packed_codebook, D)
    ids = torch.empty((N, max(k, 0)), dtype=ids_dtype, device=z.device)
    scores = torch.empty((N, max(k, 0)), dtype=torch.float32, device=z.device)
    ws = torch.empty(lib.selftok_vq_topk_workspace_bytes(N, C, k), dtype=torch.uint8, device=z.device)
    flags = (IDS_I32 if ids_dtype == torch.int32 else 0) | (PRENORMED if prenormed else 0) | ((rt & 0xF) << 8) | ((split & 0xFF) << 16)
    _lib.check(lib.selftok_vq_topk_packed_f32(_p(zz), _p(packed_codebook), _p(ids), _p(scores), _p(ws), N, C, D, k, flags, _stream()),
               "selftok_vq_topk_packed_f32")
    return ids.reshape(z.shape[:-1] + (k,)), scores.reshape(z.shape[:-1] + (k,))


def vq_ema_accumulate(z: torch.Tensor, ids: torch.Tensor, C: int, prenormed: bool = False):
    _need_cuda(z, ids)
    zz = z.contiguous().float().reshape(-1, z.shape[-1])
    flat = ids.contiguous().reshape(-1)
    if flat.dtype not in (torch.int32, torch.int64):
        flat = flat.to(torch.int64)
    assert flat.numel() == zz.shape[0]
    bins = torch.zeros(C, dtype=torch.float32, device=z.device)
    esum = torch.zeros(C, zz.shape[1], dtype=torch.float32, device=z.device)
    flags = (IDS_I32 if flat.dtype == torch.int32 else 0) | (PRENORMED if prenormed else 0)
    _lib.check(_lib.load().selftok_vq_ema_accumulate_f32(_p(zz), _p(flat), _p(bins), _p(esum), zz.shape[0], C, zz.shape[1], flags, _stream()),
               "selftok_vq_ema_accumulate_f32")
    return bins, esum


def vq_softmax_stats(z: torch.Tensor, codebook: torch.Tensor, scale: float = 10.0, colmean: bool = True, prenormed: bool = False):
    _need_cuda(z, codebook)
    assert z.dim() == 3 and codebook.dim() == 2 and z.shape[-1] == codebook.shape[1]
    zz, cb = z.contiguous().float(), codebook.contiguous().float()
    B, K, Dm = zz.shape
    C = cb.shape[0]
    lib = _lib.load()
    rows = torch.empty(B * K, 2, dtype=torch.float32, device=z.device)
    cm = torch.empty(K, C, dtype=torch.float32, device=z.device) if colmean else None
    ws = torch.empty(lib.selftok_vq_softmax_workspace_bytes(B * K), dtype=torch.uint8, device=z.device)
    _lib.check(lib.selftok_vq_softmax_stats_f32(_p(zz), _p(cb), _p(rows), _p(cm), _p(ws), B, K, C, Dm, float(scale), PRENORMED if prenormed else 0, _stream()),
               "selftok_vq_softmax_stats_f32")
    return rows, cm


def vq_softmax_backward(z: torch.Tensor, codebook: torch.Tensor, rowstats: torch.Tensor, g_colmean: torch.Tensor, scale: float = 10.0,
                        prenormed: bool = False) -> torch.Tensor:
    _need_cuda(z, codebook, rowstats, g_colmean)
    zz, cb, g = z.contiguous().float(), codebook.contiguous().float(), g_colmean.contiguous().float()
    B, K, Dm = zz.shape
    C = cb.shape[0]
    assert tuple(g.shape) == (K, C) and tuple(rowstats.shape) == (B * K, 2) and rowstats.is_contiguous() and rowstats.dtype == torch.float32
    lib = _lib.load()
    grad = torch.empty_like(zz)
    ws = torch.empty(lib.selftok_vq_softmax_workspace_bytes(B * K), dtype=torch.uint8, device=z.device)
    _lib.check(lib.selftok_vq_softmax_backward_f32(_p(zz), _p(cb), _p(rowstats), _p(g), _p(grad), _p(ws), B, K, C, Dm, float(scale),
                                                   PRENORMED if prenormed else 0, _stream()), "selftok_vq_softmax_backward_f32")
    return grad


def vq_tpc_update_(tpc: torch.Tensor, ids: torch.Tensor, weight: float) -> torch.Tensor:
    _need_cuda(tpc, ids)
    assert tpc.is_contiguous() and tpc.dtype == torch.float32 and ids.dim() == 2 and ids.shape[1] == tpc.shape[0]
    flat = ids.contiguous()
    if flat.dtype not in (torch.int32, torch.int64):
        flat = flat.to(torch.int64)
    K, C = tpc.shape
    _lib.check(_lib.load().selftok_vq_tpc_update_f32(_p(tpc), _p(flat), flat.shape[0], K, C, float(weight), IDS_I32 if flat.dtype == torch.int32 else 0,
                                                     _stream()), "selftok_vq_tpc_update_f32")
    return tpc


def code_gather_ln(ids: torch.Tensor, codebook: torch.Tensor, ln_w=None, ln_b=None, eps: float = 1e-6) -> torch.Tensor:
    _need_cuda(ids, codebook)
    if ids.is_floating_point() or ids.is_complex() or ids.dtype == torch.bool:
        raise TypeError(f"code_gather_ln: ids must be an integer tensor, got {ids.dtype}")
    if ids.dtype not in (torch.int32, torch.int64):
        ids = ids.to(torch.int64)
    flat = ids.contiguous().reshape(-1)
    n = flat.numel()
    C, D = codebook.shape
    out = torch.empty(n, D, dtype=torch.float32, device=ids.device)
    flags = IDS_I32 if flat.dtype == torch.int32 else 0
    _lib.check(_lib.load().selftok_code_gather_ln_f32(_p(flat), _p(codebook), _p(ln_w), _p(ln_b), _p(out), n, C, D,
                                                      eps, flags, _stream()), "selftok_code_gather_ln_f32")
    return out.reshape(*ids.shape, D)



def _table_strides(t, per_sample: bool, B: int, T: int, H: int):
    if t is None:
        return 0, 0
    assert t.dim() == 2 and t.stride(1) == 1 and t.shape == ((B, H) if per_sample else (T, H))
    return (t.stride(0), 0) if per_sample else (0, t.stride(0))


def residual_ln_mod(x, *, y=None, gate=None, shift=None, scale=None, per_sample=False, gate_per_sample=None,
                    want_x=True, want_n=True, eps=1e-6, split=False, overflow=None):
    _need_cuda(x)
    B, T, H = x.shape
    assert x.is_contiguous() and x.dtype == torch.float32

    if shift is not None:
        assert scale is not None and shift.stride(0) == scale.stride(0)
    msb, mst = _table_strides(shift, per_sample, B, T, H)
    gsb, gst = _table_strides(gate, per_sample if gate_per_sample is None else gate_per_sample, B, T, H)
    if y is not None:
        assert y.is_contiguous() and y.shape == x.shape
    x_out = torch.empty_like(x) if (y is not None and want_x) else None
    if split and want_n:
        n_s = SplitAct((B, T, H), x.device)
        _lib.check(_lib.load().selftok_residual_ln_mod_split(_p(x), _p(y), _p(gate), _p(shift), _p(scale), _p(x_out), _p(n_s.data),
                                                             _p(overflow), B, T, H, msb, mst, gsb, gst, eps, _stream()), "selftok_residual_ln_mod_split")
        return (x_out if y is not None else x), n_s
    n_out = torch.empty_like(x) if want_n else None
    _lib.check(_lib.load().selftok_residual_ln_mod_f32(_p(x), _p(y), _p(gate), _p(shift), _p(scale), _p(x_out), _p(n_out),
                                                       B, T, H, msb, mst, gsb, gst, eps, _stream()), "selftok_residual_ln_mod_f32")
    return (x_out if y is not None else x), n_out


def bias_gelu_(h, bias=None):
    _need_cuda(h)
    assert h.is_contiguous() and h.dtype == torch.float32
    cols = h.shape[-1]
    _lib.check(_lib.load().selftok_bias_gelu_f32(_p(h), _p(bias), h.numel() // cols, cols, _stream()), "selftok_bias_gelu_f32")
    return h


def linear_gelu(x, weight, bias):
    _need_cuda(x, weight)
    shp = x.shape
    out = torch._addmm_activation(bias, x.reshape(-1, shp[-1]), weight.t(), use_gelu=True)
    return out.reshape(*shp[:-1], weight.shape[0])


LINEAR_GELU = 1


def linear_f16x2_supported(N: int, K: int) -> bool:
    return N % 128 == 0 and K % 32 == 0


def linear_f16x2_pack(weight: torch.Tensor, overflow: torch.Tensor = None) -> torch.Tensor:
    _need_cuda(weight)
    w = weight.contiguous().float()
    N, K = w.shape
    lib = _lib.load()
    nbytes = lib.selftok_linear_f16x2_packed_bytes(N, K)
    if nbytes == 0:
        raise _lib.SelftokHipError(f"linear_f16x2: weight {N}x{K} needs N % 128 == 0 and K % 32 == 0")
    packed = torch.empty(nbytes // 2, dtype=torch.float16, device=w.device)
    _lib.check(lib.selftok_linear_f16x2_pack_weight(_p(w), _p(packed), N, K, _p(overflow), _stream()), "selftok_linear_f16x2_pack_weight")
    return packed


def _rows16(x: torch.Tensor):
    K = x.shape[-1]
    x2 = x.reshape(-1, K)
    if x2.stride(1) != 1 or (x2.shape[0] > 1 and (x2.stride(0) % 4 or x2.stride(0) < K)) or x2.data_ptr() % 16:
        x2 = x2.contiguous()
    return x2, (x2.stride(0) if x2.shape[0] > 1 else K)


def linear_f16x2(x: torch.Tensor, packed: torch.Tensor, bias, N: int, gelu: bool = False, overflow: torch.Tensor = None) -> torch.Tensor:
    _need_cuda(x, packed)
    K = x.shape[-1]
    assert x.dtype == torch.float32 and packed.numel() * 2 == 4 * N * K, "packed weight does not match (N, K)"
    x2, lda = _rows16(x)
    M = x2.shape[0]
    out = torch.empty(M, N, dtype=torch.float32, device=x.device)
    _lib.check(_lib.load().selftok_linear_f16x2_f32(_p(x2), lda, _p(packed), _p(bias), _p(out), N, M, N, K,
                                                    LINEAR_GELU if gelu else 0, _p(overflow), _stream()), "selftok_linear_f16x2_f32")
    return out.reshape(*x.shape[:-1], N)


class SplitAct:
    dtype = torch.float16

    def __init__(self, shape, device, zero: bool = False):
        self.shape = tuple(int(v) for v in shape)
        K = self.shape[-1]
        assert K % 32 == 0, "split activations need K % 32 == 0"
        self.rows = 1
        for v in self.shape[:-1]:
            self.rows *= v
        self.data = (torch.zeros if zero else torch.empty)((self.rows + 15) // 16, K // 32, 2, 16, 32, dtype=torch.float16, device=device)

    @property
    def device(self):
        return self.data.device

    def planes(self) -> torch.Tensor:
        K = self.shape[-1]
        p = self.data.permute(2, 0, 3, 1, 4).reshape(2, -1, K)[:, :self.rows]
        return p.reshape(2, *self.shape)


def split_f16x2(x: torch.Tensor, overflow: torch.Tensor = None) -> SplitAct:
    _need_cuda(x)
    x2, ld = _rows16(x)
    out = SplitAct(x.shape, x.device)
    _lib.check(_lib.load().selftok_split_f16x2_f32(_p(x2), ld, _p(out.data), out.rows, x.shape[-1],
                                                   _p(overflow), _stream()), "selftok_split_f16x2_f32")
    return out


def split_to_f32(xs: SplitAct) -> torch.Tensor:
    p = xs.planes()
    return p[0].float() + p[1].float() * (1.0 / 2048.0)


@functools.lru_cache(maxsize=None)
def _cu_count() -> int:
    return int(torch.cuda.get_device_properties(torch.cuda.current_device()).multi_processor_count) if torch.cuda.is_available() else 256


SPLITK_MAX_ROWS = 1024


@functools.lru_cache(maxsize=4096)
def f16x2_ksplit(M: int, N: int, K: int) -> int:
    if M <= 0 or M > SPLITK_MAX_ROWS:
        return 1
    tiles = ((M + 255) // 256) * (N // 128)
    kt = K // 32
    cus = _cu_count()
    best, best_cost = 1, 0.42 * kt
    for s in range(2, 65):
        if kt % s or kt // s < 3 or tiles * s > cus:
            continue
        cost = 0.42 * (kt // s) + 1.2e-6 * s * M * N + 4.0
        if cost < best_cost:
            best, best_cost = s, cost
    return best


def _linear_split(xs: SplitAct, packed: torch.Tensor, bias, N: int, *, single_pass: bool, gelu: bool = False, out_split: bool = False, resid=None,
                  gate=None, gate_per_sample: bool = False, ksplit: Optional[int] = None, overflow: torch.Tensor = None):
    _need_cuda(xs.data, packed, resid)
    K = xs.shape[-1]
    assert packed.numel() * 2 == 4 * N * K, "packed weight does not match (N, K)"
    M, lead = xs.rows, xs.shape[:-1]
    lib = _lib.load()
    name = "selftok_linear_f16_split" if single_pass else "selftok_linear_f16x2_split"
    tail = (_p(overflow), _stream())
    k_entry = not single_pass or ksplit is not None
    if k_entry:
        ksplit = 1 if ksplit is None else int(ksplit)
        ws = torch.empty(ksplit * M * N, dtype=torch.float32, device=xs.device) if (ksplit > 1 and M > 0) else None
        tail = (ksplit, _p(ws)) + tail
    if resid is not None:
        assert not gelu and not out_split
        assert resid.dim() == 3 and resid.is_contiguous() and resid.dtype == torch.float32 and resid.shape[-1] == N
        B, T, _ = resid.shape
        assert M == B * T
        gsb, gst = _table_strides(gate, gate_per_sample, B, T, N)
        out = torch.empty_like(resid)
        name += "_residual_k" if k_entry else "_residual"
        _lib.check(getattr(lib, name)(_p(xs.data), _p(packed), _p(bias), _p(resid), N, _p(gate), gsb, gst, T, _p(out), N, M, N, K, *tail), name)
        return out
    out = SplitAct((*lead, N), xs.device) if out_split else torch.empty(M, N, dtype=torch.float32, device=xs.device)
    name += "_k" if k_entry else ""
    _lib.check(getattr(lib, name)(_p(xs.data), _p(packed), _p(bias), None if out_split else _p(out), _p(out.data) if out_split else None, N, M, N, K,
                                  LINEAR_GELU if gelu else 0, *tail), name)
    return out if out_split else out.reshape(*lead, N)


def linear_f16x2_split(xs: SplitAct, packed: torch.Tensor, bias, N: int, gelu: bool = False, overflow: torch.Tensor = None,
                       out_split: bool = False, ksplit: int = 1):
    return _linear_split(xs, packed, bias, N, single_pass=False, gelu=gelu, out_split=out_split, ksplit=ksplit, overflow=overflow)


def linear_f16x2_split_residual(xs: SplitAct, packed: torch.Tensor, bias, N: int, resid: torch.Tensor, gate=None,
                                gate_per_sample: bool = False, overflow: torch.Tensor = None, ksplit: int = 1) -> torch.Tensor:
    return _linear_split(xs, packed, bias, N, single_pass=False, resid=resid, gate=gate, gate_per_sample=gate_per_sample, ksplit=ksplit, overflow=overflow)


def _as_split(x, overflow) -> SplitAct:
    return x if isinstance(x, SplitAct) else split_f16x2(x, overflow)


def linear_f16_split(xs, packed: torch.Tensor, bias, N: int, gelu: bool = False, overflow: torch.Tensor = None, out_split: bool = False):
    return _linear_split(_as_split(xs, overflow), packed, bias, N, single_pass=True, gelu=gelu, out_split=out_split, overflow=overflow)


def linear_f16_split_residual(xs, packed: torch.Tensor, bias, N: int, resid: torch.Tensor, gate=None,
                              gate_per_sample: bool = False, overflow: torch.Tensor = None) -> torch.Tensor:
    return _linear_split(_as_split(xs, overflow), packed, bias, N, single_pass=True, resid=resid, gate=gate, gate_per_sample=gate_per_sample, overflow=overflow)


F16_SPLITK_COST = (0.23, 1.2e-6, 2.0, 3)


@functools.lru_cache(maxsize=4096)
def f16_ksplit(M: int, N: int, K: int) -> int:
    if M <= 0 or M > SPLITK_MAX_ROWS:
        return 1
    if F16_SPLITK_COST is None:
        return f16x2_ksplit(M, N, K)
    per_tile, per_partial, second, min_tiles = F16_SPLITK_COST
    tiles = ((M + 255) // 256) * (N // 128)
    kt = K // 32
    cus = _cu_count()
    best, best_cost = 1, per_tile * kt
    for s in range(2, 65):
        if kt % s or kt // s < min_tiles or tiles * s > cus:
            continue
        cost = per_tile * (kt // s) + per_partial * s * M * N + second
        if cost < best_cost:
            best, best_cost = s, cost
    return best


def linear_f16_split_k(xs, packed: torch.Tensor, bias, N: int, ksplit: int, gelu: bool = False, overflow: torch.Tensor = None, out_split: bool = False):
    return _linear_split(_as_split(xs, overflow), packed, bias, N, single_pass=True, gelu=gelu, out_split=out_split, ksplit=int(ksplit), overflow=overflow)


def linear_f16_split_residual_k(xs, packed: torch.Tensor, bias, N: int, resid: torch.Tensor, ksplit: int, gate=None,
                                gate_per_sample: bool = False, overflow: torch.Tensor = None) -> torch.Tensor:
    return _linear_split(_as_split(xs, overflow), packed, bias, N, single_pass=True, resid=resid, gate=gate, gate_per_sample=gate_per_sample,
                         ksplit=int(ksplit), overflow=overflow)


def silu(x):
    _need_cuda(x)
    x = x.contiguous()
    out = torch.empty_like(x)
    _lib.check(_lib.load().selftok_silu_f32(_p(x), _p(out), x.numel(), _stream()), "selftok_silu_f32")
    return out


def add_rows_(x, table):
    _need_cuda(x, table)
    assert x.is_contiguous() and table.is_contiguous() and x[0].numel() == table.numel()
    _lib.check(_lib.load().selftok_add_rows_f32(_p(x), _p(table), _p(x), x.shape[0], table.numel(), _stream()), "selftok_add_rows_f32")
    return x


def timestep_embed(t, freqs, t_scale=1.0):
    _need_cuda(t, freqs)
    t = t.contiguous().float()
    n, half = t.numel(), freqs.numel()
    out = torch.empty(n, 2 * half, dtype=torch.float32, device=t.device)
    _lib.check(_lib.load().selftok_timestep_embed_f32(_p(t), _p(freqs), _p(out), n, 2 * half, float(t_scale), _stream()), "selftok_timestep_embed_f32")
    return out


def patchify(x):
    _need_cuda(x)
    x = x.contiguous().float()
    B, C, H, W = x.shape
    out = torch.empty(B, (H // 2) * (W // 2), 4 * C, dtype=torch.float32, device=x.device)
    _lib.check(_lib.load().selftok_patchify_f32(_p(x), _p(out), B, C, H, W, _stream()), "selftok_patchify_f32")
    return out


def unpatchify_cfg_euler(y_cond, x=None, dt=0.0, y_uncond=None, cfg_scale=1.0, C=16, hp=16, wp=16, want_v=False):
    _need_cuda(y_cond)
    B = y_cond.shape[0]
    assert y_cond.is_contiguous() and y_cond.shape[1] == hp * wp and y_cond.shape[2] == 4 * C
    x_out = torch.empty(B, C, 2 * hp, 2 * wp, dtype=torch.float32, device=y_cond.device) if x is not None else None
    v_out = torch.empty(B, C, 2 * hp, 2 * wp, dtype=torch.float32, device=y_cond.device) if (want_v or x is None) else None
    if x is not None:
        assert x.is_contiguous()
    _lib.check(_lib.load().selftok_unpatchify_cfg_euler_f32(_p(y_cond), _p(y_uncond), _p(x), _p(x_out), _p(v_out), B, C, hp, wp,
                                                            float(dt), float(cfg_scale), _stream()), "selftok_unpatchify_cfg_euler_f32")
    return x_out, v_out


def rmsnorm(x, w=None, eps=1e-6):
    _need_cuda(x)
    x = x.contiguous().float()
    out = torch.empty_like(x)
    dim = x.shape[-1]
    _lib.check(_lib.load().selftok_rmsnorm_f32(_p(x), _p(w), _p(out), x.numel() // dim, dim, eps, _stream()), "selftok_rmsnorm_f32")
    return out


def rotary(t, freqs, start_index: int = 0, scale: float = 1.0):
    _need_cuda(t, freqs)
    t = t.contiguous().float()
    freqs = freqs.contiguous().float()
    seq, rot = freqs.shape
    dim = t.shape[-1]
    if rot > dim - start_index:
        raise ValueError(f"feature dimension {dim} is not of sufficient size to rotate in all the positions {rot}")
    mid = t if (start_index == 0 and rot == dim) else t[..., start_index:start_index + rot].contiguous()
    out = torch.empty_like(mid)
    _lib.check(_lib.load().selftok_rotary_f32(_p(mid), _p(freqs), _p(out), mid.numel() // rot, seq, rot, float(scale), _stream()), "selftok_rotary_f32")
    if mid is t:
        return out
    return torch.cat((t[..., :start_index], out, t[..., start_index + rot:]), dim=-1)



def _seg(q, k, v, o):
    s = _lib.AttnSeg()
    if k is None:
        return s
    if isinstance(o, SplitAct):
        assert o.shape == (k.shape[0], q.shape[1], q.shape[2])
        o = None
    for name, t in (("q", q), ("k", k), ("v", v), ("o", o)):
        if t is None:
            continue
        assert t.dim() == 3 and t.stride(2) == 1 and t.dtype == torch.float32
        setattr(s, name, t.data_ptr())
        setattr(s, name + "_rs", t.stride(1))
        setattr(s, name + "_bs", t.stride(0))
    s.len = k.shape[1]
    return s


ATTN_F16X2 = 1
ATTN_F16 = 2


def pack_key_mask(mask: torch.Tensor) -> torch.Tensor:
    B, K = mask.shape
    W = (K + 31) // 32
    m = torch.zeros(B, W * 32, dtype=torch.int64, device=mask.device)
    m[:, :K] = mask != 0
    words = (m.view(B, W, 32) << torch.arange(32, device=mask.device, dtype=torch.int64)).sum(dim=2)
    return torch.where(words >= (1 << 31), words - (1 << 32), words).to(torch.int32).contiguous()


def attention(seg0, seg1, heads, head_dim, kvis=None, seg0_sees_seg1=True, scale=None, mode: int = 0, overflow=None,
              kmask=None, kmask_bs=None):
    lib = _lib.load()
    d = _lib.AttnDesc()
    ref = seg1 if seg1 is not None else seg0
    _need_cuda(ref[1])
    d.seg[0] = _seg(*seg0) if seg0 is not None else _lib.AttnSeg()
    d.seg[1] = _seg(*seg1) if seg1 is not None else _lib.AttnSeg()
    for i, sg in enumerate((seg0, seg1)):
        if sg is not None and isinstance(sg[3], SplitAct):
            d.o_blk[i] = sg[3].data.data_ptr()
    d.B, d.H, d.head_dim = ref[1].shape[0], heads, head_dim
    if kvis is not None:
        assert kvis.dtype == torch.int32 and kvis.is_cuda and kvis.numel() == d.B
        d.kvis = kvis.data_ptr()
    d.seg0_sees_seg1 = 1 if seg0_sees_seg1 else 0
    d.scale = float(scale if scale is not None else head_dim ** -0.5)
    f16 = int(mode) == ATTN_F16
    d.mode = int(mode) if (head_dim == 64 and not f16) else 0
    d.overflow = _p(overflow)
    import ctypes
    bs = 0
    if kmask is not None:
        assert kmask.dtype in (torch.int32, getattr(torch, "uint32", torch.int32)) and kmask.is_cuda and kmask.dim() == 2
        assert kmask.shape[0] == d.B and kmask.stride(1) == 1
        bs = int(kmask.stride(0) if kmask_bs is None else kmask_bs)
    if f16:
        _lib.check(lib.selftok_attn_f16(ctypes.byref(d), _p(kmask), bs, _stream()), "selftok_attn_f16")
        return
    if kmask is not None:
        _lib.check(lib.selftok_attn_kmask_f32(ctypes.byref(d), kmask.data_ptr(), bs, _stream()), "selftok_attn_kmask_f32")
        return
    _lib.check(lib.selftok_attn_f32(ctypes.byref(d), _stream()), "selftok_attn_f32")



def groupnorm_silu(x, weight, bias, groups=32, eps=1e-6, silu_act=True):
    _need_cuda(x)
    assert x.dtype == torch.bfloat16 and x.is_contiguous()
    B, C, H, W = x.shape
    out = torch.empty_like(x)
    _lib.check(_lib.load().selftok_groupnorm_silu_bf16(_p(x), _p(weight), _p(bias), _p(out), B, C, H * W, groups, eps,
                                                       1 if silu_act else 0, _stream()), "selftok_groupnorm_silu_bf16")
    return out


class PackedConv:
    __slots__ = ("packed", "bias", "cout", "cin", "ksize", "bn")

    def __init__(self, weight: torch.Tensor, bias: Optional[torch.Tensor]):
        _need_cuda(weight, bias)
        assert weight.dtype == torch.bfloat16 and weight.dim() == 4 and weight.shape[2] == weight.shape[3] and weight.shape[2] in (1, 3)
        w = weight.contiguous()
        self.cout, self.cin, self.ksize = int(w.shape[0]), int(w.shape[1]), int(w.shape[2])
        self.bn = 128 if self.cout >= 64 else 32
        lib = _lib.load()
        self.packed = torch.empty(lib.selftok_conv2d_packed_bytes(self.cout, self.cin, self.ksize, self.bn), dtype=torch.uint8, device=w.device)
        _lib.check(lib.selftok_conv2d_pack_weight_bf16(_p(w), _p(self.packed), self.cout, self.cin, self.ksize, self.bn, _stream()), "selftok_conv2d_pack_weight_bf16")
        self.bias = None if bias is None else bias.to(torch.bfloat16).contiguous()


def conv2d_nhwc(x: torch.Tensor, pc: PackedConv, stride: int = 1, upsample: bool = False, residual: Optional[torch.Tensor] = None,
                cstore: Optional[int] = None) -> torch.Tensor:
    _need_cuda(x, residual)
    assert x.dtype == torch.bfloat16 and x.is_contiguous() and x.dim() == 4
    B, H, W, Cin = x.shape
    assert Cin % 8 == 0 and (Cin + 31) // 32 == (pc.cin + 31) // 32 and Cin >= pc.cin, (Cin, pc.cin)
    cs = (pc.cout + 3) // 4 * 4 if cstore is None else cstore
    assert cs % 4 == 0 and cs >= pc.cout and (cs + pc.bn - 1) // pc.bn == (pc.cout + pc.bn - 1) // pc.bn, (cs, pc.cout, pc.bn)
    Hi, Wi = (H * 2, W * 2) if upsample else (H, W)
    Ho, Wo = (Hi // 2, Wi // 2) if stride == 2 else (Hi, Wi)
    out = torch.empty(B, Ho, Wo, cs, dtype=torch.bfloat16, device=x.device)
    if residual is not None:
        assert residual.shape == out.shape and residual.is_contiguous() and residual.dtype == torch.bfloat16
    _lib.check(_lib.load().selftok_conv2d_nhwc_bf16(_p(x), _p(pc.packed), _p(pc.bias), _p(residual), _p(out), B, H, W, Cin, pc.cout, cs, cs, pc.ksize, stride,
                                                    1 if upsample else 0, pc.bn, _stream()), "selftok_conv2d_nhwc_bf16")
    return out


def groupnorm_silu_nhwc(x, weight, bias, groups=32, eps=1e-6, silu_act=True):
    _need_cuda(x, weight, bias)
    assert x.dtype == torch.bfloat16 and x.is_contiguous()
    B, C = x.shape[0], x.shape[-1]
    HW = x.numel() // (B * C)
    lib = _lib.load()
    out = torch.empty_like(x)
    ws = torch.empty(lib.selftok_groupnorm_nhwc_workspace_bytes(B, HW, C), dtype=torch.uint8, device=x.device)
    _lib.check(lib.selftok_groupnorm_silu_nhwc_bf16(_p(x), _p(weight), _p(bias), _p(out), _p(ws), B, HW, C, groups, eps, 1 if silu_act else 0, _stream()),
               "selftok_groupnorm_silu_nhwc_bf16")
    return out


def latent_process_in(moments, c_keep=16, shift=0.0609, scale=1.5305):
    _need_cuda(moments)
    assert moments.dtype == torch.bfloat16 and moments.is_contiguous()
    B, Cin, H, W = moments.shape
    out = torch.empty(B, c_keep, H, W, dtype=torch.float32, device=moments.device)
    _lib.check(_lib.load().selftok_latent_process_in(_p(moments), _p(out), B, Cin, c_keep, H * W, shift, scale, _stream()), "selftok_latent_process_in")
    return out


def latent_process_out(z, shift=0.0609, scale=1.5305):
    _need_cuda(z)
    z = z.contiguous().float()
    out = torch.empty(z.shape, dtype=torch.bfloat16, device=z.device)
    _lib.check(_lib.load().selftok_latent_process_out(_p(z), _p(out), z.numel(), shift, scale, _stream()), "selftok_latent_process_out")
    return out


def clamp01_(img):
    _need_cuda(img)
    assert img.dtype == torch.bfloat16 and img.is_contiguous()
    _lib.check(_lib.load().selftok_clamp01_bf16(_p(img), img.numel(), _stream()), "selftok_clamp01_bf16")
    return img


def vq_encode_split_launch(z, packed_codebook, ids_dtype=torch.int64, coarse=None, _flags: Optional[int] = None):
    import ctypes
    lib = _lib.load()
    zz = z.contiguous().float().reshape(-1, z.shape[-1])
    N, D = zz.shape
    C = packed_codes(packed_codebook, D)
    ids = torch.empty(N, dtype=ids_dtype, device=z.device)
    ws = torch.empty(lib.selftok_vq_workspace_bytes(N, C), dtype=torch.uint8, device=z.device)
    flags = (IDS_I32 if ids_dtype == torch.int32 else 0) | (int(_flags) if _flags is not None else _coarse_flags(coarse))
    nsplit = ctypes.c_int(0)

    def launch_main():
        _lib.check(lib.selftok_vq_argmax_partial_packed_f32(_p(zz), _p(packed_codebook), _p(ws), ctypes.addressof(nsplit), N, C, D,
                                                            flags, _stream()), "selftok_vq_argmax_partial_packed_f32")

    def launch_finalize():
        _lib.check(lib.selftok_vq_finalize_packed(_p(ws), _p(zz), _p(packed_codebook), _p(ids), None, N, C, D, nsplit.value, flags,
                                                  _stream()), "selftok_vq_finalize_packed")

    return ids.reshape(z.shape[:-1]), launch_main, launch_finalize


VX_UPSAMPLE2X = 8


def vx_conv2d(x: torch.Tensor, w: torch.Tensor, bias: torch.Tensor, stride: int = 1, residual: Optional[torch.Tensor] = None, order: int = 0,
              cin: Optional[int] = None, upsample: bool = False) -> torch.Tensor:
    _need_cuda(x, w, bias, residual)
    assert x.dtype == w.dtype == bias.dtype == torch.bfloat16 and x.is_contiguous() and w.is_contiguous() and x.dim() == 4 and w.dim() == 4
    B, H, W, ldx = x.shape
    Cout, k, k2, Cin = w.shape
    assert k == k2 and (cin is None or cin == Cin)
    if upsample:
        assert stride == 1
        H, W, order = 2 * H, 2 * W, order | VX_UPSAMPLE2X
    Ho, Wo = (H // 2, W // 2) if stride == 2 else (H, W)
    out = torch.empty(B, Ho, Wo, Cout, dtype=torch.bfloat16, device=x.device)
    if residual is not None:
        assert residual.shape == out.shape and residual.is_contiguous() and residual.dtype == torch.bfloat16
    _lib.check(_lib.load().selftok_vx_conv2d_bf16(_p(x), _p(w), _p(bias), _p(residual), _p(out), B, H, W, ldx, Cin, Cout, k, stride, order, _stream()),
               "selftok_vx_conv2d_bf16")
    return out


def vx_silu_table(device) -> torch.Tensor:
    t = torch.empty(65536, dtype=torch.int16, device=device)
    with torch.cuda.device(t.device):
        _lib.check(_lib.load().selftok_vx_silu_table_bf16(_p(t), _stream()), "selftok_vx_silu_table_bf16")
    return t


def vx_groupnorm(x: torch.Tensor, gamma: torch.Tensor, beta: torch.Tensor, silu_table: Optional[torch.Tensor] = None, groups: int = 32, eps: float = 1e-6,
                 want_stats: bool = False):
    _need_cuda(x, gamma, beta, silu_table)
    assert x.dtype == torch.bfloat16 and x.is_contiguous()
    B, C = x.shape[0], x.shape[-1]
    if B == 0:
        return (torch.empty_like(x), torch.empty(0, groups, 2, dtype=torch.float32, device=x.device)) if want_stats else torch.empty_like(x)
    HW = x.numel() // (B * C)
    lib = _lib.load()
    nbytes = lib.selftok_vx_groupnorm_workspace_bytes(B, HW, C)
    if nbytes == 0:
        raise _lib.SelftokHipError(f"vx_groupnorm: unsupported shape B={B} HW={HW} C={C}")
    out = torch.empty_like(x)
    ws = torch.empty(nbytes, dtype=torch.uint8, device=x.device)
    stats = torch.empty(B, groups, 2, dtype=torch.float32, device=x.device) if want_stats else None
    _lib.check(lib.selftok_vx_groupnorm_bf16(_p(x), _p(gamma), _p(beta), _p(out), _p(ws), _p(silu_table), _p(stats), B, HW, C, groups, float(eps), _stream()),
               "selftok_vx_groupnorm_bf16")
    return (out, stats) if want_stats else out


def vx_attention(q: torch.Tensor, k: torch.Tensor, v: torch.Tensor) -> torch.Tensor:
    _need_cuda(q, k, v)
    assert q.dtype == k.dtype == v.dtype == torch.bfloat16 and q.is_contiguous() and k.is_contiguous() and v.is_contiguous() and q.shape == k.shape == v.shape
    B, T, C = q.shape
    lib = _lib.load()
    out = torch.empty_like(q)
    if B == 0:
        return out
    ws = torch.empty(lib.selftok_vx_attention_workspace_bytes(B, T, C), dtype=torch.uint8, device=q.device)
    _lib.check(lib.selftok_vx_attention_bf16(_p(q), _p(k), _p(v), _p(out), _p(ws), B, T, C, _stream()), "selftok_vx_attention_bf16")
    return out


def vx_expf(x: torch.Tensor) -> torch.Tensor:
    _need_cuda(x)
    assert x.dtype == torch.float32 and x.is_contiguous()
    y = torch.empty_like(x)
    _lib.check(_lib.load().selftok_vx_expf_f32(_p(x), _p(y), x.numel(), _stream()), "selftok_vx_expf_f32")
    return y



def _rows2d(t: torch.Tensor):
    assert t.dtype == torch.float32 and t.stride(-1) == 1
    ld = t.stride(-2) if t.dim() > 1 else t.shape[-1]
    rows = t.numel() // t.shape[-1]
    for d in range(t.dim() - 2, 0, -1):
        assert t.shape[d - 1] == 1 or t.stride(d - 1) == t.stride(d) * t.shape[d], "rows are not equally strided"
    return rows, ld


EX_LINEAR_GELU_ON_XE = True
EX_LINEAR_SG_MIN_ROWS = 256


def ex_linear(x: torch.Tensor, weight: torch.Tensor, bias=None, *, gelu: bool = False, res=None, res_mod: int = 0, gate=None, gate_mod: int = 0,
              out: Optional[torch.Tensor] = None, bias_last: bool = False, kernel: str = "auto") -> torch.Tensor:
    N, K = weight.shape
    if kernel not in ("auto", "xe", "sg"):
        raise ValueError(f"ex_linear kernel {kernel!r}: expected 'auto', 'xe' or 'sg'")
    sg_ok = not (gelu and (res is not None or gate is not None or (out is not None and not out.is_contiguous())))
    if kernel == "sg" or (kernel == "auto" and sg_ok and linear_f32_supported(N, K, mkl_order=True) and x.numel() // max(K, 1) >= EX_LINEAR_SG_MIN_ROWS
                          and not (gelu and EX_LINEAR_GELU_ON_XE)):
        return linear_f32(x, weight, bias, mkl_order=True, gelu=gelu, res=res, res_mod=res_mod, gate=gate, gate_mod=gate_mod, out=out, bias_last=bias_last)
    _need_cuda(x, weight, bias, res, gate)
    assert weight.dtype == torch.float32 and weight.is_contiguous() and x.shape[-1] == K
    M, ldx = _rows2d(x)
    if out is None:
        out = torch.empty(x.shape[:-1] + (N,), dtype=torch.float32, device=x.device)
    assert out.is_contiguous() or out.stride(-1) == 1
    _, ldo = _rows2d(out)
    ldr = _rows2d(res)[1] if res is not None else 0
    ldg = _rows2d(gate)[1] if gate is not None else 0
    _lib.check(_lib.load().selftok_ex_linear_f32(_p(x), ldx, _p(weight), _p(bias), _p(res), ldr, int(res_mod), _p(gate), ldg, int(gate_mod), _p(out), ldo,
                                                 M, N, K, int(bool(gelu)) | (2 if bias_last else 0), _stream()), "selftok_ex_linear_f32")
    return out


LINEAR_BIAS_LAST, LINEAR_MKL_ORDER = 2, 4
_LINEAR_WS = {}


def _linear_ws(device, nbytes: int):
    key = (device.index, int(torch.cuda.current_stream(device).cuda_stream))
    held = _LINEAR_WS.setdefault(key, [])
    if not held or held[-1].numel() < nbytes:
        held.append(torch.empty(max(nbytes, 64 << 20), dtype=torch.uint8, device=device))
    return held[-1]


def linear_f32(x: torch.Tensor, weight: torch.Tensor, bias=None, *, mkl_order: bool = False, gelu: bool = False, res=None, res_mod: int = 0, gate=None,
               gate_mod: int = 0, out: Optional[torch.Tensor] = None, bias_last: bool = False, split: int = 0, use_workspace: bool = True, _flags: int = 0) -> torch.Tensor:
    _need_cuda(x, weight, bias, res, gate)
    N, K = weight.shape
    assert weight.dtype == torch.float32 and weight.is_contiguous() and x.shape[-1] == K
    M, ldx = _rows2d(x)
    if out is None:
        out = torch.empty(x.shape[:-1] + (N,), dtype=torch.float32, device=x.device)
    assert out.is_contiguous() or out.stride(-1) == 1
    _, ldo = _rows2d(out)
    ldr = _rows2d(res)[1] if res is not None else 0
    ldg = _rows2d(gate)[1] if gate is not None else 0
    flags = (1 if gelu else 0) | (LINEAR_BIAS_LAST if bias_last else 0) | (LINEAR_MKL_ORDER if mkl_order else 0) | ((int(split) & 0xFF) << 8) | int(_flags)
    lib = _lib.load()
    ws, nws = None, 0
    if use_workspace:
        nws = int(lib.selftok_linear_f32_workspace_bytes(M, N, K, flags))
        ws = _linear_ws(x.device, nws) if nws else None
    _lib.check(lib.selftok_linear_f32(_p(x), ldx, _p(weight), _p(bias), _p(res), ldr, int(res_mod), _p(gate), ldg, int(gate_mod), _p(out), ldo, M, N, K, flags,
                                      _p(ws), (ws.numel() if ws is not None else 0), _stream()), "selftok_linear_f32")
    return out


def linear_f32_supported(N: int, K: int, mkl_order: bool = False) -> bool:
    return N % 128 == 0 and K % 32 == 0 and not (mkl_order and 384 < K < 768)


def ex_layernorm_mod(x: torch.Tensor, shift=None, scale=None, gamma=None, beta=None, eps: float = 1e-6, want_stats: bool = False, per_sample: bool = False):
    _need_cuda(x, shift, scale, gamma, beta)
    N = x.shape[-1]
    rows, ldx = _rows2d(x)
    out = torch.empty(x.shape, dtype=torch.float32, device=x.device)
    T, ldt = 0, 0
    if shift is not None:
        assert scale is not None and shift.dim() == 2 and shift.shape == scale.shape and shift.stride(0) == scale.stride(0) and shift.stride(1) == 1 == scale.stride(1)
        T, ldt = shift.shape[0], shift.stride(0)
        if per_sample:
            assert x.dim() == 3 and shift.shape[0] == x.shape[0]
            T = -x.shape[1]
    stats = torch.empty(rows, 2, dtype=torch.float32, device=x.device) if want_stats else None
    _lib.check(_lib.load().selftok_ex_layernorm_mod_f32(_p(x), ldx, _p(out), N, _p(shift), _p(scale), ldt, T, _p(gamma), _p(beta), _p(stats), rows, N, float(eps),
                                                        _stream()), "selftok_ex_layernorm_mod_f32")
    return (out, stats) if want_stats else out


def ex_res_layernorm_mod(x: torch.Tensor, lin: torch.Tensor, *, lin_bias=None, gate=None, gate_mod: int = 0, shift=None, scale=None, eps: float = 1e-6,
                         per_sample: bool = False, x_out: Optional[torch.Tensor] = None):
    _need_cuda(x, lin, lin_bias, gate, shift, scale)
    N = x.shape[-1]
    rows, ldx = _rows2d(x)
    rl, ldl = _rows2d(lin)
    assert rl == rows and lin.shape[-1] == N
    xo = torch.empty(x.shape, dtype=torch.float32, device=x.device) if x_out is None else x_out
    out = torch.empty(x.shape, dtype=torch.float32, device=x.device)
    ldg = _rows2d(gate)[1] if gate is not None else 0
    T, ldt = 0, 0
    if shift is not None:
        assert scale is not None and shift.dim() == 2 and shift.shape == scale.shape and shift.stride(0) == scale.stride(0) and shift.stride(1) == 1 == scale.stride(1)
        T, ldt = shift.shape[0], shift.stride(0)
        if per_sample:
            assert x.dim() == 3 and shift.shape[0] == x.shape[0]
            T = -x.shape[1]
    _lib.check(_lib.load().selftok_ex_res_layernorm_mod_f32(_p(x), ldx, _p(lin), ldl, _p(lin_bias), _p(gate), ldg, int(gate_mod), _p(xo), _rows2d(xo)[1], _p(out), N,
                                                            _p(shift), _p(scale), ldt, T, rows, N, float(eps), _stream()), "selftok_ex_res_layernorm_mod_f32")
    return xo, out


EX_UNARY = {"gelu_tanh": 0, "silu": 1, "sleef_expf": 2, "sleef_tanhf": 3, "exp_u20": 4}


def ex_unary(x: torch.Tensor, kind: str, out: Optional[torch.Tensor] = None) -> torch.Tensor:
    _need_cuda(x)
    assert x.dtype == torch.float32 and x.is_contiguous()
    y = torch.empty_like(x) if out is None else out
    assert y.dtype == torch.float32 and y.is_contiguous() and y.numel() == x.numel()
    _lib.check(_lib.load().selftok_ex_unary_f32(_p(x), _p(y), x.numel(), EX_UNARY[kind], _stream()), "selftok_ex_unary_f32")
    return y


EX_ATTENTION_WS_LIMIT = 6 << 30
EX_ATTENTION_DEFAULT = "auto"


def ex_attention(q: torch.Tensor, k1, v1, heads: int, k2=None, v2=None, slots1: Optional[int] = None, kernel: str = "auto",
                 kmask: Optional[torch.Tensor] = None, valid1: Optional[int] = None) -> torch.Tensor:
    if kernel == "auto":
        kernel = EX_ATTENTION_DEFAULT
    if kernel not in ("auto", "fused", "unfused"):
        raise ValueError(f"ex_attention kernel {kernel!r}: expected 'auto', 'fused' or 'unfused'")
    _need_cuda(q, k1, v1, k2, v2)
    B, Tq, HD = q.shape
    D = HD // heads
    _, qs = _rows2d(q)
    rows1, ks1 = 0, 0
    if k1 is not None:
        _, ks1 = _rows2d(k1)
        assert _rows2d(v1)[1] == ks1 and k1.shape == v1.shape
        rows1 = k1.shape[1]
    else:
        assert slots1 is not None and k2 is not None
    Tk1 = rows1 if slots1 is None else int(slots1)
    Tk2, ks2 = 0, 0
    if k2 is not None:
        Tk2, ks2 = k2.shape[1], _rows2d(k2)[1]
        assert _rows2d(v2)[1] == ks2 and k2.shape == v2.shape
    lib = _lib.load()
    km_bs = 0
    nv1 = rows1
    if valid1 is not None:
        assert kmask is not None and 0 <= int(valid1) <= rows1
        nv1 = int(valid1)
    if kmask is not None:
        assert kmask.dtype in (torch.int32, getattr(torch, "uint32", torch.int32)) and kmask.is_cuda and kmask.dim() == 2 and kmask.stride(1) == 1
        assert kmask.shape[0] in (1, B) and kmask.shape[1] * 32 >= Tk1 and Tk1 <= 2048, (tuple(kmask.shape), B, Tk1)
        km_bs = int(kmask.stride(0)) if kmask.shape[0] == B and B > 1 else 0
    out = (torch.zeros if (kmask is not None and Tk2 == 0) else torch.empty)(B, Tq, HD, dtype=torch.float32, device=q.device)
    if B == 0:
        return out
    fused = kernel == "fused" or (kernel == "auto" and lib.selftok_ex_attention_fused_supported(Tk1, Tk2, D))
    if fused and kmask is not None:
        _lib.check(lib.selftok_ex_attention_kmask_fused_f32(_p(q), qs, _p(k1), _p(v1), ks1, Tk1, nv1, rows1, _p(k2), _p(v2), ks2, Tk2, _p(out), B, heads, Tq, D,
                                                            _p(kmask), km_bs, _stream()), "selftok_ex_attention_kmask_fused_f32")
        return out
    if fused:
        _lib.check(lib.selftok_ex_attention_fused_f32(_p(q), qs, _p(k1), _p(v1), ks1, Tk1, rows1, rows1, _p(k2), _p(v2), ks2, Tk2, _p(out), B, heads, Tq, D, _stream()),
                   "selftok_ex_attention_fused_f32")
        return out
    per = int(lib.selftok_ex_attention_workspace_bytes(1, heads, Tq, Tk1 + Tk2, D))
    nb = max(1, min(B, EX_ATTENTION_WS_LIMIT // max(per, 1), 65535 // max(heads, 1)))
    ws = torch.empty(int(lib.selftok_ex_attention_workspace_bytes(nb, heads, Tq, Tk1 + Tk2, D)), dtype=torch.uint8, device=q.device)
    for b0 in range(0, B, nb):
        n = min(nb, B - b0)
        sl = lambda t: None if t is None else t[b0:b0 + n]
        if kmask is not None:
            _lib.check(lib.selftok_ex_attention_kmask_f32(_p(sl(q)), qs, _p(sl(k1)), _p(sl(v1)), ks1, Tk1, nv1, rows1, _p(sl(k2)), _p(sl(v2)), ks2, Tk2, _p(out[b0:b0 + n]), _p(ws),
                                                          n, heads, Tq, D, _p(kmask[b0:b0 + n] if km_bs else kmask), km_bs, _stream()), "selftok_ex_attention_kmask_f32")
            continue
        _lib.check(lib.selftok_ex_attention_f32(_p(sl(q)), qs, _p(sl(k1)), _p(sl(v1)), ks1, Tk1, rows1, rows1, _p(sl(k2)), _p(sl(v2)), ks2, Tk2, _p(out[b0:b0 + n]), _p(ws),
                                                n, heads, Tq, D, _stream()), "selftok_ex_attention_f32")
    return out


_IMG_LUT = {}


def image_norm_lut(device, dtype=torch.bfloat16) -> torch.Tensor:
    import numpy as np
    device = torch.device(device)
    key = (device, dtype)
    if key not in _IMG_LUT:
        from .pipeline import NormalizeToTensor
        lut = NormalizeToTensor()(np.arange(256, dtype=np.uint8).reshape(1, 256, 1)).reshape(256)
        _IMG_LUT[key] = lut.to(dtype).to(device)
    return _IMG_LUT[key]


def _img_table(table):
    import numpy as np
    t = np.ascontiguousarray(np.asarray(table), dtype=np.int64)
    if t.ndim != 2 or t.shape[1] != 3:
        raise _lib.SelftokHipError(f"image table: expected [B, 3] (byte offset, width, height), got {t.shape}")
    return t


IMAGE_FILTERS = {"bilinear": 2, "bicubic": 3, "box": 4}
_UNSERVED_FILTERS = {0: "NEAREST", 1: "LANCZOS", 5: "HAMMING", "nearest": "NEAREST", "lanczos": "LANCZOS", "hamming": "HAMMING"}


def image_filter_code(filter, fn="image filter") -> int:
    key = filter.lower() if isinstance(filter, str) else int(filter)
    if key in _UNSERVED_FILTERS:
        name = _UNSERVED_FILTERS[key]
        why = "Pillow does not resample it through coefficient tables" if name == "NEAREST" else "its weights are libm's sin / cos, whose bits the device does not promise"
        raise _lib.SelftokHipError(f"{fn}: Pillow's {name} filter is not served on the device ({why}); BILINEAR, BICUBIC and BOX are")
    if key in IMAGE_FILTERS:
        return IMAGE_FILTERS[key]
    if key in IMAGE_FILTERS.values():
        return key
    raise _lib.SelftokHipError(f"{fn}: unknown filter {filter!r}: expected one of {sorted(IMAGE_FILTERS)} or Pillow's codes 2, 3, 4")


def _image_resample(fn, entry, layout, dev_name, packed, t, size, dtype, out, t_dev, return_tables, empty_ok=False, filter=None):
    import numpy as np
    _need_cuda(packed, out, t_dev)
    if packed.dtype != torch.uint8 or packed.dim() != 1 or not packed.is_contiguous():
        raise _lib.SelftokHipError(f"{fn}: `packed` must be a contiguous 1-D uint8 tensor, got {packed.dtype} {tuple(packed.shape)}")
    if dtype not in (torch.bfloat16, torch.float32):
        raise _lib.SelftokHipError(f"{fn}: output dtype {dtype}: expected bfloat16 or float32")
    (N, cols), S = t.shape, int(size)
    if out is None:
        out = torch.empty(N, 3, max(S, 0), max(S, 0), dtype=dtype, device=packed.device)
    elif out.dtype != dtype or tuple(out.shape) != (N, 3, S, S) or not out.is_contiguous():
        raise _lib.SelftokHipError(f"{fn}: `out` must be a contiguous {dtype} [{N}, 3, {S}, {S}] tensor")
    if N == 0 and empty_ok:
        return (out, {}) if return_tables else out
    lib = _lib.load()
    fa = () if filter is None else (int(filter),)
    nbytes = getattr(lib, entry + "_workspace_bytes")(t.ctypes.data, N, S, *fa)
    if nbytes == 0:
        _lib.check(-1, entry + "_workspace_bytes")
    if t_dev is None:
        t_dev = torch.from_numpy(t).to(packed.device)
    elif t_dev.dtype != torch.int64 or t_dev.numel() != cols * N or not t_dev.is_contiguous():
        raise _lib.SelftokHipError(f"{fn}: `{dev_name}` must be the contiguous int64 [{'B' if cols == 3 else 'V'}, {cols}] table")
    ws = torch.empty(nbytes, dtype=torch.uint8, device=packed.device)
    lut = image_norm_lut(packed.device, dtype)
    _lib.check(getattr(lib, entry)(_p(packed), packed.numel(), t.ctypes.data, _p(t_dev), N, S, *fa, _p(out), int(dtype == torch.bfloat16), _p(lut), _p(ws), nbytes, _stream()), entry)
    if not return_tables:
        return out
    lay = np.zeros(4, dtype=np.int64)
    _lib.check(getattr(lib, layout)(t.ctypes.data, N, S, *fa, lay.ctypes.data), layout)
    wi = ws[:(nbytes // 4) * 4].view(torch.int32).cpu().numpy()
    tabs = {}
    for name, base, ks in (("h", int(lay[0]), int(lay[1])), ("v", int(lay[2]), int(lay[3]))):
        rows = wi[base:base + N * S * ks].reshape(N, S, ks)
        tabs[name] = (rows[:, :, 0].copy(), rows[:, :, 1].copy(), rows[:, :, 2:].copy())
    return out, tabs


def image_resize_crop_norm(packed: torch.Tensor, table, size: int, dtype=torch.bfloat16, out: Optional[torch.Tensor] = None,
                           table_dev: Optional[torch.Tensor] = None, return_tables: bool = False):
    return _image_resample("image_resize_crop_norm", "selftok_img_resize_crop_norm_u8", "selftok_img_resize_tables_layout", "table_dev",
                           packed, _img_table(table), size, dtype, out, table_dev, return_tables)


def image_view_rows(sources_table, views):
    import numpy as np
    src = _img_table(sources_table)
    v = np.ascontiguousarray(np.asarray(views), dtype=np.int64)
    if v.ndim != 2 or v.shape[1] != 10:
        raise _lib.SelftokHipError(f"image views: expected [V, 10] (source index, x0, y0, bw, bh, rw, rh, left, top, flip), got {v.shape}")
    if v.shape[0] and (v[:, 0].min() < 0 or v[:, 0].max() >= src.shape[0]):
        raise _lib.SelftokHipError(f"image views: a source index outside 0 .. {src.shape[0] - 1}")
    return np.ascontiguousarray(np.concatenate([src[v[:, 0]], v[:, 1:]], axis=1))


def image_views(packed: torch.Tensor, sources_table, views, size: int, dtype=torch.bfloat16, out: Optional[torch.Tensor] = None,
                rows_dev: Optional[torch.Tensor] = None, return_tables: bool = False, rows=None, filter="bilinear"):
    import numpy as np
    code = image_filter_code(filter, "image_views")
    if rows is None:
        rows = image_view_rows(sources_table, views)
    elif not isinstance(rows, np.ndarray) or rows.dtype != np.int64 or rows.ndim != 2 or rows.shape[1] != 12 or not rows.flags["C_CONTIGUOUS"]:
        raise _lib.SelftokHipError("image_views: `rows` must be the contiguous int64 numpy [V, 12] table of image_view_rows")
    if code == IMAGE_FILTERS["bilinear"]:
        return _image_resample("image_views", "selftok_img_views_u8", "selftok_img_views_tables_layout", "rows_dev", packed, rows, size, dtype, out, rows_dev, return_tables,
                               empty_ok=True)
    return _image_resample("image_views", "selftok_img_views_filter_u8", "selftok_img_views_filter_tables_layout", "rows_dev", packed, rows, size, dtype, out, rows_dev,
                           return_tables, empty_ok=True, filter=code)


def image_resize(packed: torch.Tensor, frames, filter, frames_dev: Optional[torch.Tensor] = None) -> torch.Tensor:
    import numpy as np
    code = image_filter_code(filter, "image_resize")
    t = np.ascontiguousarray(np.asarray(frames), dtype=np.int64)
    if t.ndim != 2 or t.shape[1] != 6:
        raise _lib.SelftokHipError(f"image_resize: expected [N, 6] (source offset, W, H, destination offset, ow, oh), got {t.shape}")
    _need_cuda(packed, frames_dev)
    if packed.dtype != torch.uint8 or packed.dim() != 1 or not packed.is_contiguous():
        raise _lib.SelftokHipError(f"image_resize: `packed` must be a contiguous 1-D uint8 tensor, got {packed.dtype} {tuple(packed.shape)}")
    N = t.shape[0]
    if N == 0:
        return packed
    lib = _lib.load()
    nbytes = lib.selftok_img_resize_u8_workspace_bytes(t.ctypes.data, N, code)
    if nbytes == 0:
        _lib.check(-1, "selftok_img_resize_u8_workspace_bytes")
    if frames_dev is None:
        frames_dev = torch.from_numpy(t).to(packed.device)
    elif frames_dev.dtype != torch.int64 or frames_dev.numel() != 6 * N or not frames_dev.is_contiguous():
        raise _lib.SelftokHipError("image_resize: `frames_dev` must be the contiguous int64 [N, 6] table")
    ws = torch.empty(nbytes, dtype=torch.uint8, device=packed.device)
    _lib.check(lib.selftok_img_resize_u8(_p(packed), packed.numel(), t.ctypes.data, _p(frames_dev), N, code, _p(ws), nbytes, _stream()), "selftok_img_resize_u8")
    return packed


def image_to_u8(img: torch.Tensor) -> torch.Tensor:
    _need_cuda(img)
    if img.dtype not in (torch.bfloat16, torch.float32):
        raise _lib.SelftokHipError(f"image_to_u8: dtype {img.dtype}: expected bfloat16 or float32")
    if img.dim() != 4 or img.shape[1] != 3:
        raise _lib.SelftokHipError(f"image_to_u8: expected [B, 3, H, W], got {tuple(img.shape)}")
    img = img.contiguous()
    B, _, H, W = img.shape
    out = torch.empty(B, H, W, 3, dtype=torch.uint8, device=img.device)
    _lib.check(_lib.load().selftok_img_to_u8(_p(img), int(img.dtype == torch.bfloat16), _p(out), B, H, W, _stream()), "selftok_img_to_u8")
    return out


_IMG_METRICS_WS = {}


def _img_metrics_ws(device, nbytes: int):
    key = (device.index, int(torch.cuda.current_stream(device).cuda_stream))
    held = _IMG_METRICS_WS.setdefault(key, [])
    if not held or held[-1].numel() < nbytes:
        held.append(torch.empty(max(nbytes, 1 << 20), dtype=torch.uint8, device=device))
    return held[-1]


def image_metrics(recon: torch.Tensor, original: torch.Tensor, original_signed: bool = True, quantize: bool = False) -> torch.Tensor:
    _need_cuda(recon, original)
    for name, t in (("recon", recon), ("original", original)):
        if t.dtype not in (torch.bfloat16, torch.float32):
            raise _lib.SelftokHipError(f"image_metrics: `{name}` dtype {t.dtype}: expected bfloat16 or float32")
    if recon.dim() != 4 or recon.shape[1] != 3 or tuple(original.shape) != tuple(recon.shape):
        raise _lib.SelftokHipError(f"image_metrics: expected two [B, 3, H, W] tensors of one shape, got {tuple(recon.shape)} and {tuple(original.shape)}")
    from .evaluate import ssim_window
    win = ssim_window()
    recon, original = recon.contiguous(), original.contiguous()
    B, _, H, W = recon.shape
    lib = _lib.load()
    nbytes = lib.selftok_img_metrics_workspace_bytes(B, H, W)
    if nbytes == 0:
        _lib.check(-1, "selftok_img_metrics_workspace_bytes")
    ws = _img_metrics_ws(recon.device, nbytes)
    out = torch.empty(B, 2, dtype=torch.float64, device=recon.device)
    _lib.check(lib.selftok_img_metrics(_p(recon), int(recon.dtype == torch.bfloat16), _p(original), int(original.dtype == torch.bfloat16), int(bool(original_signed)),
                                       int(bool(quantize)), win.ctypes.data, _p(out), _p(ws), ws.numel(), B, H, W, _stream()), "selftok_img_metrics")
    return out


SSIM_PRESETS = ("gaussian", "skimage")


def ssim_preset(name: str):
    from .evaluate import ssim_uniform_window, ssim_window
    if name == "gaussian":
        return ssim_window(), 1.0
    if name == "skimage":
        return ssim_uniform_window(7), 49.0 / 48.0
    raise ValueError(f"SSIM preset {name!r}: expected one of {SSIM_PRESETS}")


def image_ssim(recon: torch.Tensor, original: torch.Tensor, window="skimage", cov_norm: Optional[float] = None, signed_range: bool = True,
               original_signed: bool = True, quantize: bool = False) -> torch.Tensor:
    if isinstance(window, str):
        if cov_norm is not None:
            raise ValueError(f"image_ssim: the preset {window!r} sets cov_norm itself")
        window, cov_norm = ssim_preset(window)
    elif cov_norm is None:
        raise ValueError("image_ssim: a window given as weights needs cov_norm (1.0: population moments)")
    _need_cuda(recon, original)
    for name, t in (("recon", recon), ("original", original)):
        if t.dtype not in (torch.bfloat16, torch.float32):
            raise _lib.SelftokHipError(f"image_ssim: `{name}` dtype {t.dtype}: expected bfloat16 or float32")
    if recon.dim() != 4 or recon.shape[1] != 3 or tuple(original.shape) != tuple(recon.shape):
        raise _lib.SelftokHipError(f"image_ssim: expected two [B, 3, H, W] tensors of one shape, got {tuple(recon.shape)} and {tuple(original.shape)}")
    import numpy as np
    win = np.ascontiguousarray(window, dtype=np.float64).reshape(-1)
    recon, original = recon.contiguous(), original.contiguous()
    B, _, H, W = recon.shape
    lib = _lib.load()
    nbytes = lib.selftok_img_ssim_workspace_bytes(B, H, W, int(win.size))
    if nbytes == 0:
        _lib.check(-1, "selftok_img_ssim_workspace_bytes")
    ws = _img_metrics_ws(recon.device, nbytes)
    out = torch.empty(B, dtype=torch.float64, device=recon.device)
    _lib.check(lib.selftok_img_ssim(_p(recon), int(recon.dtype == torch.bfloat16), _p(original), int(original.dtype == torch.bfloat16), int(bool(original_signed)),
                                    int(bool(quantize)), win.ctypes.data, int(win.size), float(cov_norm), int(bool(signed_range)), _p(out), _p(ws), ws.numel(), B, H, W,
                                    _stream()), "selftok_img_ssim")
    return out


def _lpips_f32(name: str, t: torch.Tensor, dim: int) -> torch.Tensor:
    if t.dtype != torch.float32 or t.dim() != dim:
        raise _lib.SelftokHipError(f"lpips: `{name}` must be a float32 tensor of {dim} dimensions, got {t.dtype} {tuple(t.shape)}")
    return t.contiguous()


def lpips_pack_conv_weight(weight: torch.Tensor) -> torch.Tensor:
    if weight.dim() != 4:
        raise _lib.SelftokHipError(f"lpips_pack_conv_weight: expected [Cout, Cin, KH, KW], got {tuple(weight.shape)}")
    Cout, Cin, KH, KW = weight.shape
    n = _lib.load().selftok_lpips_conv2d_packed_floats(Cin, Cout, KH, KW)
    if n == 0:
        _lib.check(-1, "selftok_lpips_conv2d_packed_floats")
    K, CP = KH * KW * Cin, -(-Cout // 64) * 64
    out = torch.zeros(n // CP, CP, dtype=torch.float32, device=weight.device)
    out[:K, :Cout] = weight.detach().float().permute(2, 3, 1, 0).reshape(K, Cout)
    return out


def lpips_conv2d(x: torch.Tensor, packed: torch.Tensor, bias: Optional[torch.Tensor], Cout: int, KH: int, KW: int, stride: int, pad: int, relu: bool,
                 out: Optional[torch.Tensor] = None) -> torch.Tensor:
    _need_cuda(x, packed, bias, out)
    x, packed = _lpips_f32("x", x, 4), _lpips_f32("packed", packed, 2)
    bias = None if bias is None else _lpips_f32("bias", bias, 1)
    N, H, W, Cin = x.shape
    lib = _lib.load()
    if packed.numel() != lib.selftok_lpips_conv2d_packed_floats(Cin, Cout, KH, KW) or (bias is not None and bias.numel() != Cout):
        raise _lib.SelftokHipError(f"lpips_conv2d: packed weight of {packed.numel()} floats / bias do not belong to Cin {Cin}, Cout {Cout}, {KH} x {KW}")
    OH, OW = (H + 2 * pad - KH) // stride + 1, (W + 2 * pad - KW) // stride + 1
    if out is None:
        out = torch.empty(N, max(OH, 0), max(OW, 0), Cout, dtype=torch.float32, device=x.device)
    elif out.dtype != torch.float32 or tuple(out.shape) != (N, OH, OW, Cout) or not out.is_contiguous():
        raise _lib.SelftokHipError(f"lpips_conv2d: `out` must be a contiguous float32 {(N, OH, OW, Cout)}, got {out.dtype} {tuple(out.shape)}")
    _lib.check(lib.selftok_lpips_conv2d_f32(_p(x), _p(packed), _p(bias), _p(out), N, H, W, Cin, Cout, KH, KW, stride, pad, int(bool(relu)), _stream()),
               "selftok_lpips_conv2d_f32")
    return out


def lpips_maxpool3s2(x: torch.Tensor, out: Optional[torch.Tensor] = None) -> torch.Tensor:
    _need_cuda(x, out)
    x = _lpips_f32("x", x, 4)
    N, H, W, C = x.shape
    shape = (N, max((H - 3) // 2 + 1, 0), max((W - 3) // 2 + 1, 0), C)
    if out is None:
        out = torch.empty(shape, dtype=torch.float32, device=x.device)
    elif out.dtype != torch.float32 or tuple(out.shape) != shape or not out.is_contiguous():
        raise _lib.SelftokHipError(f"lpips_maxpool3s2: `out` must be a contiguous float32 {shape}, got {out.dtype} {tuple(out.shape)}")
    _lib.check(_lib.load().selftok_lpips_maxpool3s2_f32(_p(x), _p(out), N, H, W, C, _stream()), "selftok_lpips_maxpool3s2_f32")
    return out


def lpips_maxpool2s2(x: torch.Tensor, out: Optional[torch.Tensor] = None) -> torch.Tensor:
    _need_cuda(x, out)
    x = _lpips_f32("x", x, 4)
    N, H, W, C = x.shape
    shape = (N, H // 2, W // 2, C)
    if out is None:
        out = torch.empty(shape, dtype=torch.float32, device=x.device)
    elif out.dtype != torch.float32 or tuple(out.shape) != shape or not out.is_contiguous():
        raise _lib.SelftokHipError(f"lpips_maxpool2s2: `out` must be a contiguous float32 {shape}, got {out.dtype} {tuple(out.shape)}")
    _lib.check(_lib.load().selftok_lpips_maxpool2s2_f32(_p(x), _p(out), N, H, W, C, _stream()), "selftok_lpips_maxpool2s2_f32")
    return out


def lpips_input(recon: torch.Tensor, original: torch.Tensor, original_signed: bool = True, quantize: bool = False, out: Optional[torch.Tensor] = None) -> torch.Tensor:
    for name, t in (("recon", recon), ("original", original)):
        if t.dtype not in (torch.bfloat16, torch.float32):
            raise _lib.SelftokHipError(f"lpips_input: `{name}` dtype {t.dtype}: expected bfloat16 or float32")
    if recon.dim() != 4 or recon.shape[1] != 3 or tuple(original.shape) != tuple(recon.shape):
        raise _lib.SelftokHipError(f"lpips_input: expected two [B, 3, H, W] tensors of one shape, got {tuple(recon.shape)} and {tuple(original.shape)}")
    _need_cuda(recon, original, out)
    recon, original = recon.contiguous(), original.contiguous()
    B, _, H, W = recon.shape
    if out is None:
        out = torch.empty(2 * B, H, W, 3, dtype=torch.float32, device=recon.device)
    elif out.dtype != torch.float32 or tuple(out.shape) != (2 * B, H, W, 3) or not out.is_contiguous():
        raise _lib.SelftokHipError(f"lpips_input: `out` must be a contiguous float32 {(2 * B, H, W, 3)}, got {out.dtype} {tuple(out.shape)}")
    _lib.check(_lib.load().selftok_lpips_input(_p(recon), int(recon.dtype == torch.bfloat16), _p(original), int(original.dtype == torch.bfloat16),
                                               int(bool(original_signed)), int(bool(quantize)), _p(out), B, H, W, _stream()), "selftok_lpips_input")
    return out


_LPIPS_WS = {}


def lpips_workspace(device, nbytes: int) -> torch.Tensor:
    key = (device.index, int(torch.cuda.current_stream(device).cuda_stream))
    held = _LPIPS_WS.setdefault(key, [])
    if not held or held[-1].numel() < nbytes:
        held.append(torch.empty(max(nbytes, 1 << 20), dtype=torch.uint8, device=device))
    return held[-1]


def lpips_distance(feat: torch.Tensor, w: torch.Tensor, out: Optional[torch.Tensor] = None, accumulate: bool = False, workspace: Optional[torch.Tensor] = None) -> torch.Tensor:
    _need_cuda(feat, w, out, workspace)
    feat, w = _lpips_f32("feat", feat, 4), _lpips_f32("w", w, 1)
    N, h, wd, C = feat.shape
    if N < 2 or N % 2 or w.numel() != C:
        raise _lib.SelftokHipError(f"lpips_distance: expected feat [2B, h, w, C] and w [C], got {tuple(feat.shape)} and {tuple(w.shape)}")
    B = N // 2
    if out is None:
        if accumulate:
            raise _lib.SelftokHipError("lpips_distance: accumulate needs `out`")
        out = torch.empty(B, dtype=torch.float64, device=feat.device)
    elif out.dtype != torch.float64 or tuple(out.shape) != (B,) or not out.is_contiguous():
        raise _lib.SelftokHipError(f"lpips_distance: `out` must be a contiguous float64 [{B}], got {out.dtype} {tuple(out.shape)}")
    lib = _lib.load()
    nbytes = lib.selftok_lpips_distance_workspace_bytes(B, h * wd)
    if nbytes == 0:
        _lib.check(-1, "selftok_lpips_distance_workspace_bytes")
    ws = lpips_workspace(feat.device, nbytes) if workspace is None else workspace
    _lib.check(lib.selftok_lpips_distance(_p(feat), _p(w), _p(out), _p(ws), ws.numel() * ws.element_size(), B, h * wd, C, int(bool(accumulate)), _stream()),
               "selftok_lpips_distance")
    return out


FID_POOL_MODES = {"max_s2": 0, "max_s1p1": 1, "avg_s1p1": 2}


def _fid_slice_out(what: str, out: Optional[torch.Tensor], shape, C: int, co_off: int, device):
    N, OH, OW = shape
    if out is None:
        if co_off:
            raise _lib.SelftokHipError(f"{what}: a channel offset needs the `out` map it points into")
        return torch.empty(N, max(OH, 0), max(OW, 0), C, dtype=torch.float32, device=device)
    if out.dtype != torch.float32 or out.dim() != 4 or tuple(out.shape[:3]) != (N, OH, OW) or not out.is_contiguous() or co_off < 0 or out.shape[3] < co_off + C:
        raise _lib.SelftokHipError(f"{what}: `out` must be a contiguous float32 [{N}, {OH}, {OW}, ldo >= {co_off} + {C}], got {out.dtype} {tuple(out.shape)}")
    return out


def fid_conv2d(x: torch.Tensor, packed: torch.Tensor, bias: Optional[torch.Tensor], Cout: int, KH: int, KW: int, stride: int, pad_h: int, pad_w: int, relu: bool = True,
               out: Optional[torch.Tensor] = None, co_off: int = 0) -> torch.Tensor:
    _need_cuda(x, packed, bias, out)
    x, packed = _lpips_f32("x", x, 4), _lpips_f32("packed", packed, 2)
    bias = None if bias is None else _lpips_f32("bias", bias, 1)
    N, H, W, Cin = x.shape
    lib = _lib.load()
    if packed.numel() != lib.selftok_lpips_conv2d_packed_floats(Cin, Cout, KH, KW) or (bias is not None and bias.numel() != Cout):
        raise _lib.SelftokHipError(f"fid_conv2d: packed weight of {packed.numel()} floats / bias do not belong to Cin {Cin}, Cout {Cout}, {KH} x {KW}")
    OH, OW = (H + 2 * pad_h - KH) // stride + 1, (W + 2 * pad_w - KW) // stride + 1
    if H + 2 * pad_h < KH or W + 2 * pad_w < KW:
        raise _lib.SelftokHipError(f"fid_conv2d: {H} x {W} input has no output pixel under a {KH} x {KW} kernel with pad {pad_h}, {pad_w}")
    out = _fid_slice_out("fid_conv2d", out, (N, OH, OW), Cout, co_off, x.device)
    _lib.check(lib.selftok_fid_conv2d_f32(_p(x), _p(packed), _p(bias), _p(out), N, H, W, Cin, Cout, KH, KW, stride, pad_h, pad_w, out.shape[3], co_off,
                                          int(bool(relu)), _stream()), "selftok_fid_conv2d_f32")
    return out


def fid_pool3(x: torch.Tensor, mode: str, out: Optional[torch.Tensor] = None, co_off: int = 0) -> torch.Tensor:
    _need_cuda(x, out)
    x = _lpips_f32("x", x, 4)
    if mode not in FID_POOL_MODES:
        raise _lib.SelftokHipError(f"fid_pool3: mode {mode!r}: expected one of {sorted(FID_POOL_MODES)}")
    N, H, W, C = x.shape
    if mode == "max_s2" and min(H, W) < 3:
        raise _lib.SelftokHipError(f"fid_pool3: max_s2 needs H, W >= 3 (one window), got {H} x {W}")
    PH, PW = ((H - 3) // 2 + 1, (W - 3) // 2 + 1) if mode == "max_s2" else (H, W)
    out = _fid_slice_out("fid_pool3", out, (N, PH, PW), C, co_off, x.device)
    _lib.check(_lib.load().selftok_fid_pool3_f32(_p(x), _p(out), N, H, W, C, FID_POOL_MODES[mode], out.shape[3], co_off, _stream()), "selftok_fid_pool3_f32")
    return out


def fid_input(images: torch.Tensor, signed: bool, quantize: bool = False, tables=None, out: Optional[torch.Tensor] = None) -> torch.Tensor:
    if images.dtype not in (torch.bfloat16, torch.float32):
        raise _lib.SelftokHipError(f"fid_input: dtype {images.dtype}: expected bfloat16 or float32")
    if images.dim() != 4 or images.shape[1] != 3:
        raise _lib.SelftokHipError(f"fid_input: expected a [B, 3, H, W] tensor, got {tuple(images.shape)}")
    _need_cuda(images, out)
    images = images.contiguous()
    B, _, H, W = images.shape
    OH, OW, ytab, xtab = H, W, None, None
    if tables is not None:
        ytab, xtab = tables
        _need_cuda(ytab, xtab)
        for t in (ytab, xtab):
            if t.dtype != torch.int32 or t.dim() != 2 or t.shape[0] != 3 or not t.is_contiguous():
                raise _lib.SelftokHipError(f"fid_input: a tap table must be a contiguous int32 [3, n], got {t.dtype} {tuple(t.shape)}")
        OH, OW = ytab.shape[1], xtab.shape[1]
    if out is None:
        out = torch.empty(B, OH, OW, 3, dtype=torch.float32, device=images.device)
    elif out.dtype != torch.float32 or tuple(out.shape) != (B, OH, OW, 3) or not out.is_contiguous():
        raise _lib.SelftokHipError(f"fid_input: `out` must be a contiguous float32 {(B, OH, OW, 3)}, got {out.dtype} {tuple(out.shape)}")
    _lib.check(_lib.load().selftok_fid_input(_p(images), int(images.dtype == torch.bfloat16), int(bool(signed)), int(bool(quantize)), _p(out), B, H, W, OH, OW,
                                             _p(ytab), _p(xtab), _stream()), "selftok_fid_input")
    return out


def fid_spatial_mean(x: torch.Tensor, out: Optional[torch.Tensor] = None) -> torch.Tensor:
    _need_cuda(x, out)
    x = _lpips_f32("x", x, 4)
    N, h, w, C = x.shape
    if out is None:
        out = torch.empty(N, C, dtype=torch.float32, device=x.device)
    elif out.dtype != torch.float32 or tuple(out.shape) != (N, C) or not out.is_contiguous():
        raise _lib.SelftokHipError(f"fid_spatial_mean: `out` must be a contiguous float32 {(N, C)}, got {out.dtype} {tuple(out.shape)}")
    _lib.check(_lib.load().selftok_fid_spatial_mean_f32(_p(x), _p(out), N, h * w, C, _stream()), "selftok_fid_spatial_mean_f32")
    return out


def fid_stats(x: torch.Tensor, mu: Optional[torch.Tensor] = None, sigma: Optional[torch.Tensor] = None, workspace: Optional[torch.Tensor] = None):
    _need_cuda(x, mu, sigma, workspace)
    x = _lpips_f32("x", x, 2)
    N, D = x.shape
    lib = _lib.load()
    nbytes = lib.selftok_fid_stats_workspace_bytes(N, D)
    if nbytes == 0:
        _lib.check(-1, "selftok_fid_stats_workspace_bytes")
    for name, t, shape in (("mu", mu, (D,)), ("sigma", sigma, (D, D))):
        if t is not None and (t.dtype != torch.float64 or tuple(t.shape) != shape or not t.is_contiguous()):
            raise _lib.SelftokHipError(f"fid_stats: `{name}` must be a contiguous float64 {shape}, got {t.dtype} {tuple(t.shape)}")
    mu = torch.empty(D, dtype=torch.float64, device=x.device) if mu is None else mu
    sigma = torch.empty(D, D, dtype=torch.float64, device=x.device) if sigma is None else sigma
    ws = lpips_workspace(x.device, nbytes) if workspace is None else workspace
    _lib.check(lib.selftok_fid_stats(_p(x), _p(mu), _p(sigma), _p(ws), ws.numel() * ws.element_size(), N, D, _stream()), "selftok_fid_stats")
    return mu, sigma


def _gm_rows(name: str, t: torch.Tensor) -> torch.Tensor:
    if t.dim() != 2 or t.dtype != torch.float32:
        raise _lib.SelftokHipError(f"{name}: expected a float32 [rows, D] tensor, got {t.dtype} {tuple(t.shape)}")
    return t.contiguous()


def _gm_workspace(what: str, nbytes: int, device, workspace: Optional[torch.Tensor]) -> torch.Tensor:
    if nbytes == 0:
        _lib.check(-1, what)
    return lpips_workspace(device, nbytes) if workspace is None else workspace


def knn_radius(a: torch.Tensor, k: int = 3, *, split: int = 0, out: Optional[torch.Tensor] = None, workspace: Optional[torch.Tensor] = None) -> torch.Tensor:
    a = _gm_rows("knn_radius", a)
    _need_cuda(a, out, workspace)
    N, D = a.shape
    lib = _lib.load()
    ws = _gm_workspace("selftok_knn_radius_f32_workspace_bytes", lib.selftok_knn_radius_f32_workspace_bytes(N, D, int(k)), a.device, workspace)
    if out is None:
        out = torch.empty(N, dtype=torch.float32, device=a.device)
    elif out.dtype != torch.float32 or tuple(out.shape) != (N,) or not out.is_contiguous():
        raise _lib.SelftokHipError(f"knn_radius: `out` must be a contiguous float32 [{N}], got {out.dtype} {tuple(out.shape)}")
    _lib.check(lib.selftok_knn_radius_f32(_p(a), _p(out), _p(ws), ws.numel() * ws.element_size(), N, D, int(k), int(split), _stream()), "selftok_knn_radius_f32")
    return out


def manifold_member(x: torch.Tensor, a: torch.Tensor, r2: torch.Tensor, *, split: int = 0, out: Optional[torch.Tensor] = None,
                    workspace: Optional[torch.Tensor] = None) -> torch.Tensor:
    x, a = _gm_rows("manifold_member", x), _gm_rows("manifold_member", a)
    _need_cuda(x, a, r2, out, workspace)
    M, D = x.shape
    N = a.shape[0]
    if a.shape[1] != D or r2.dtype != torch.float32 or tuple(r2.shape) != (N,):
        raise _lib.SelftokHipError(f"manifold_member: expected x [M, D], a [N, D] and a float32 r2 [N], got {tuple(x.shape)}, {tuple(a.shape)}, {r2.dtype} {tuple(r2.shape)}")
    r2 = r2.contiguous()
    lib = _lib.load()
    ws = _gm_workspace("selftok_manifold_member_f32_workspace_bytes", lib.selftok_manifold_member_f32_workspace_bytes(M, N, D), x.device, workspace)
    if out is None:
        out = torch.empty(M, dtype=torch.int32, device=x.device)
    elif out.dtype != torch.int32 or tuple(out.shape) != (M,) or not out.is_contiguous():
        raise _lib.SelftokHipError(f"manifold_member: `out` must be a contiguous int32 [{M}], got {out.dtype} {tuple(out.shape)}")
    _lib.check(lib.selftok_manifold_member_f32(_p(x) if M else None, _p(a), _p(r2), _p(out) if M else None, _p(ws), ws.numel() * ws.element_size(), M, N, D, int(split),
                                               _stream()), "selftok_manifold_member_f32")
    return out


def _is_logits(name: str, logits: torch.Tensor) -> torch.Tensor:
    if logits.dim() != 2 or logits.dtype != torch.float32:
        raise _lib.SelftokHipError(f"{name}: expected float32 logits [N, C], got {logits.dtype} {tuple(logits.shape)}")
    return logits.contiguous()


def is_colmean(logits: torch.Tensor, split_size: int, workspace: Optional[torch.Tensor] = None) -> torch.Tensor:
    _need_cuda(logits, workspace)
    logits = _is_logits("is_colmean", logits)
    N, C = logits.shape
    lib = _lib.load()
    ws = _gm_workspace("selftok_is_colmean_workspace_bytes", lib.selftok_is_colmean_workspace_bytes(N, C, int(split_size)), logits.device, workspace)
    out = torch.empty(-(-N // int(split_size)), C, dtype=torch.float64, device=logits.device)
    _lib.check(lib.selftok_is_colmean(_p(logits), _p(out), _p(ws), ws.numel() * ws.element_size(), N, C, int(split_size), _stream()), "selftok_is_colmean")
    return out


def is_kl_rows(logits: torch.Tensor, colmean: torch.Tensor, split_size: int, workspace: Optional[torch.Tensor] = None) -> torch.Tensor:
    _need_cuda(logits, colmean, workspace)
    logits = _is_logits("is_kl_rows", logits)
    N, C = logits.shape
    lib = _lib.load()
    ws = _gm_workspace("selftok_is_kl_rows_workspace_bytes", lib.selftok_is_kl_rows_workspace_bytes(N, C, int(split_size)), logits.device, workspace)
    if colmean.dtype != torch.float64 or tuple(colmean.shape) != (-(-N // int(split_size)), C) or not colmean.is_contiguous():
        raise _lib.SelftokHipError(f"is_kl_rows: `colmean` must be a contiguous float64 {(-(-N // int(split_size)), C)}, got {colmean.dtype} {tuple(colmean.shape)}")
    out = torch.empty(N, dtype=torch.float64, device=logits.device)
    _lib.check(lib.selftok_is_kl_rows(_p(logits), _p(colmean), _p(out), _p(ws), ws.numel() * ws.element_size(), N, C, int(split_size), _stream()), "selftok_is_kl_rows")
    return out


def manifold_count_nn(x: torch.Tensor, a: torch.Tensor, r2: Optional[torch.Tensor] = None, *, split: int = 0, out_count: Optional[torch.Tensor] = None,
                      out_d2: Optional[torch.Tensor] = None, out_idx: Optional[torch.Tensor] = None, workspace: Optional[torch.Tensor] = None):
    x, a = _gm_rows("manifold_count_nn", x), _gm_rows("manifold_count_nn", a)
    _need_cuda(x, a, r2, out_count, out_d2, out_idx, workspace)
    M, D = x.shape
    N = a.shape[0]
    if a.shape[1] != D or (r2 is not None and (r2.dtype != torch.float32 or tuple(r2.shape) != (N,))):
        raise _lib.SelftokHipError(f"manifold_count_nn: expected x [M, D], a [N, D] and a float32 r2 [N] or None, got {tuple(x.shape)}, {tuple(a.shape)}, "
                                   f"{None if r2 is None else (r2.dtype, tuple(r2.shape))}")
    if r2 is None and out_count is not None:
        raise _lib.SelftokHipError("manifold_count_nn: `out_count` without r2 (no radii, no count)")
    r2 = None if r2 is None else r2.contiguous()
    lib = _lib.load()
    ws = _gm_workspace("selftok_manifold_count_nn_f32_workspace_bytes", lib.selftok_manifold_count_nn_f32_workspace_bytes(M, N, D), x.device, workspace)
    outs = []
    for name, t, dtype, want in (("out_count", out_count, torch.int32, r2 is not None), ("out_d2", out_d2, torch.float32, True), ("out_idx", out_idx, torch.int32, True)):
        if not want:
            outs.append(None)
        elif t is None:
            outs.append(torch.empty(M, dtype=dtype, device=x.device))
        elif t.dtype != dtype or tuple(t.shape) != (M,) or not t.is_contiguous():
            raise _lib.SelftokHipError(f"manifold_count_nn: `{name}` must be a contiguous {dtype} [{M}], got {t.dtype} {tuple(t.shape)}")
        else:
            outs.append(t)
    count, d2, idx = outs
    if M:
        _lib.check(lib.selftok_manifold_count_nn_f32(_p(x), _p(a), _p(r2), _p(count), _p(d2), _p(idx), _p(ws), ws.numel() * ws.element_size(), M, N, D, int(split), _stream()),
                   "selftok_manifold_count_nn_f32")
    return count, d2, idx


def kid_sums(xs: torch.Tensor, ys: torch.Tensor, S: int, m: int, *, out: Optional[torch.Tensor] = None, workspace: Optional[torch.Tensor] = None) -> torch.Tensor:
    xs, ys = _gm_rows("kid_sums", xs), _gm_rows("kid_sums", ys)
    _need_cuda(xs, ys, out, workspace)
    S, m = int(S), int(m)
    D = xs.shape[1]
    if tuple(xs.shape) != (S * m, D) or tuple(ys.shape) != (S * m, D) or S < 1:
        raise _lib.SelftokHipError(f"kid_sums: expected xs and ys [S * m, D] = [{S * m}, D], got {tuple(xs.shape)} and {tuple(ys.shape)}")
    lib = _lib.load()
    ws = _gm_workspace("selftok_kid_sums_f32_workspace_bytes", lib.selftok_kid_sums_f32_workspace_bytes(S, m, D), xs.device, workspace)
    if out is None:
        out = torch.empty(S, 3, dtype=torch.float64, device=xs.device)
    elif out.dtype != torch.float64 or tuple(out.shape) != (S, 3) or not out.is_contiguous():
        raise _lib.SelftokHipError(f"kid_sums: `out` must be a contiguous float64 [{S}, 3], got {out.dtype} {tuple(out.shape)}")
    _lib.check(lib.selftok_kid_sums_f32(_p(xs), _p(ys), _p(out), _p(ws), ws.numel() * ws.element_size(), S, m, D, _stream()), "selftok_kid_sums_f32")
    return out



def _stream_check(what: str, t, dtype, shape):
    if t.dtype != dtype or tuple(t.shape) != tuple(shape) or not t.is_contiguous():
        raise _lib.SelftokHipError(f"{what}: expected a contiguous {dtype} {list(shape)}, got {t.dtype} {list(t.shape)}")


def stream_prepare(step, limit, coef, pattern_words, table, table_uncond, segs, kwords_out, coef_out, mods_out, mods_uncond_out=None, *, K: int):
    import numpy as np
    _need_cuda(step, limit, coef, pattern_words, table, table_uncond, kwords_out, coef_out, mods_out, mods_uncond_out)
    if not isinstance(segs, np.ndarray) or segs.dtype != np.int32 or segs.ndim != 2 or segs.shape[1] != 2 or not segs.flags.c_contiguous:
        raise _lib.SelftokHipError("stream_prepare: `segs` must be a C-contiguous host numpy int32 [S, 2]")
    B, W = step.shape[0], (int(K) + 31) // 32
    n_steps, R = table.shape
    _stream_check("stream_prepare: step", step, torch.int32, (B,))
    _stream_check("stream_prepare: limit", limit, torch.int32, (n_steps,))
    _stream_check("stream_prepare: coef", coef, torch.float32, (n_steps, 4))
    _stream_check("stream_prepare: table", table, torch.float32, (n_steps, R))
    _stream_check("stream_prepare: kwords_out", kwords_out, torch.int32, (B, W))
    _stream_check("stream_prepare: coef_out", coef_out, torch.float32, (B, 4))
    _stream_check("stream_prepare: mods_out", mods_out, torch.float32, (B * R,))
    if pattern_words is not None:
        _stream_check("stream_prepare: pattern_words", pattern_words, torch.int32, (B, W))
    if (table_uncond is None) != (mods_uncond_out is None):
        raise _lib.SelftokHipError("stream_prepare: table_uncond and mods_uncond_out come together")
    if table_uncond is not None:
        _stream_check("stream_prepare: table_uncond", table_uncond, torch.float32, (n_steps, R))
        _stream_check("stream_prepare: mods_uncond_out", mods_uncond_out, torch.float32, (B * R,))
    _lib.check(_lib.load().selftok_stream_prepare(_p(step), _p(limit), _p(coef), _p(pattern_words), _p(table), _p(table_uncond), segs.ctypes.data, segs.shape[0],
                                                  _p(kwords_out), _p(coef_out), _p(mods_out), _p(mods_uncond_out), B, int(K), n_steps, R, _stream()),
               "selftok_stream_prepare")


def unpatchify_cfg_euler_rows(y_cond, y_uncond, x, coef_rows, step, *, cfg_scale: float = 1.0, x0_param: bool = False, x_out=None, step_out=None):
    _need_cuda(y_cond, y_uncond, x, coef_rows, step, x_out, step_out)
    B, C, Hh, Ww = x.shape
    hp, wp = Hh // 2, Ww // 2
    x_out = x if x_out is None else x_out
    step_out = step if step_out is None else step_out
    _stream_check("unpatchify_cfg_euler_rows: x", x, torch.float32, (B, C, 2 * hp, 2 * wp))
    _stream_check("unpatchify_cfg_euler_rows: x_out", x_out, torch.float32, (B, C, 2 * hp, 2 * wp))
    _stream_check("unpatchify_cfg_euler_rows: y_cond", y_cond, torch.float32, (B, hp * wp, 4 * C))
    if y_uncond is not None:
        _stream_check("unpatchify_cfg_euler_rows: y_uncond", y_uncond, torch.float32, (B, hp * wp, 4 * C))
    _stream_check("unpatchify_cfg_euler_rows: coef_rows", coef_rows, torch.float32, (B, 4))
    _stream_check("unpatchify_cfg_euler_rows: step", step, torch.int32, (B,))
    _stream_check("unpatchify_cfg_euler_rows: step_out", step_out, torch.int32, (B,))
    _lib.check(_lib.load().selftok_unpatchify_cfg_euler_rows_f32(_p(y_cond), _p(y_uncond), _p(x), _p(x_out), _p(coef_rows), _p(step), _p(step_out), B, C, hp, wp,
                                                                 float(cfg_scale), int(bool(x0_param)), _stream()), "selftok_unpatchify_cfg_euler_rows_f32")
    return x_out, step_out
```

Baseline: 3.205.

## Make split-f16 GEMM kernel persistent, walking tiles with cross-tile DMA prefetch

The f16x2 split linear kernel becomes persistent: the grid is capped at the CU count and each workgroup loops over output tiles, with the A/W LDS DMA pointers rolling over into the next tile so loads for the next tile overlap the current tile's tail and epilogue. The epilogue staging now reuses freed pipeline LDS slots per 32x32 subtile instead of a separate full staging area, and a walk-cap setter is exposed. This targets launch/tail wave quantization and prologue latency per tile, but adds per-tile syncs, index bookkeeping and a smaller staging layout that could cost epilogue efficiency.

```diff
diff --git a/include/selftok_hip_ext.h b/include/selftok_hip_ext.h
--- a/include/selftok_hip_ext.h
+++ b/include/selftok_hip_ext.h
@@ -55,6 +55,8 @@
                                         const float* resid, long ldr, const float* gate, long gate_stride_b, long gate_stride_t, int T,
                                         float* out, long ldo, int M, int N, int K, int ksplit, void* workspace, int* overflow, hipStream_t stream);
 
+int selftok_linear_f16x2_walk_cap(int cap);
+
 int selftok_attn_f16(const selftok_attn_desc* desc, const unsigned* kmask, long kmask_bs, hipStream_t stream);
 
 size_t selftok_lpips_conv2d_packed_floats(int Cin, int Cout, int KH, int KW);
diff --git a/selftoktokenizer_amd/_lib.py b/selftoktokenizer_amd/_lib.py
--- a/selftoktokenizer_amd/_lib.py
+++ b/selftoktokenizer_amd/_lib.py
@@ -98,6 +98,7 @@
     "selftok_linear_f16_split_residual": (_i, [_vp, _vp, _vp, _vp, _l, _vp, _l, _l, _i, _vp, _l, _i, _i, _i, _vp, _vp]),
     "selftok_linear_f16_split_k": (_i, [_vp, _vp, _vp, _vp, _vp, _l, _i, _i, _i, _i, _i, _vp, _vp, _vp]),
     "selftok_linear_f16_split_residual_k": (_i, [_vp, _vp, _vp, _vp, _l, _vp, _l, _l, _i, _vp, _l, _i, _i, _i, _i, _vp, _vp, _vp]),
+    "selftok_linear_f16x2_walk_cap": (_i, [_i]),
     "selftok_attn_f16": (_i, [_vp, _vp, _l, _vp]),
     "selftok_lpips_conv2d_packed_floats": (_sz, [_i, _i, _i, _i]),
     "selftok_lpips_conv2d_f32": (_i, [_vp, _vp, _vp, _vp] + [_i] * 10 + [_vp]),
diff --git a/selftoktokenizer_amd/csrc/gemm_f16.hip b/selftoktokenizer_amd/csrc/gemm_f16.hip
--- a/selftoktokenizer_amd/csrc/gemm_f16.hip
+++ b/selftoktokenizer_amd/csrc/gemm_f16.hip
@@ -25,7 +25,7 @@
     const int l31 = lane & 31, lh = lane >> 5;
 
     int mb, nb;
-    tile_of_workgroup(mblocks, nblocks, mb, nb);
+    tile_of_workgroup(blockIdx.x, gridDim.x, mblocks, nblocks, mb, nb);
     const int m0 = mb * BM, n0 = nb * BN;
     const int KT = K / BK, KL = KT - 1;
     const int NI = (KT + 1) >> 1, IL = NI - 1;
diff --git a/selftoktokenizer_amd/csrc/gemm_f16_splitk.hip b/selftoktokenizer_amd/csrc/gemm_f16_splitk.hip
--- a/selftoktokenizer_amd/csrc/gemm_f16_splitk.hip
+++ b/selftoktokenizer_amd/csrc/gemm_f16_splitk.hip
@@ -21,7 +21,7 @@
     const int l31 = lane & 31, lh = lane >> 5;
 
     int mb, nb;
-    tile_of_workgroup(mblocks, nblocks, mb, nb);
+    tile_of_workgroup(blockIdx.x, gridDim.x, mblocks, nblocks, mb, nb);
     const int m0 = mb * BM, n0 = nb * BN;
     const int KTA = K / BK;
     const int KT = KTA / (int)gridDim.y, KL = KT - 1;
diff --git a/selftoktokenizer_amd/csrc/gemm_split.hip b/selftoktokenizer_amd/csrc/gemm_split.hip
--- a/selftoktokenizer_amd/csrc/gemm_split.hip
+++ b/selftoktokenizer_amd/csrc/gemm_split.hip
@@ -1,7 +1,9 @@
 #include "common.h"
 #include "gemm_split_shared.h"
 #include "selftok_hip.h"
+#include "selftok_hip_ext.h"
 #include <stdlib.h>
+#include <atomic>
 
 namespace selftok {
 
@@ -47,7 +49,7 @@
     const int l31 = lane & 31, lh = lane >> 5;
 
     int mb, nb;
-    tile_of_workgroup(mblocks, nblocks, mb, nb);
+    tile_of_workgroup(blockIdx.x, gridDim.x, mblocks, nblocks, mb, nb);
     const int m0 = mb * BM, n0 = nb * BN;
     const int KT = K / BK, KL = KT - 1;
 
@@ -219,9 +221,7 @@
     const int wm = wave >> 1, wn = wave & 1;
     const int l31 = lane & 31, lh = lane >> 5;
 
-    int mb, nb;
-    tile_of_workgroup(mblocks, nblocks, mb, nb);
-    const int m0 = mb * BM, n0 = nb * BN;
+    const int T = mblocks * nblocks, G = (int)gridDim.x;
     const int KTA = K / BK;
     const int KT = SK ? KTA / (int)gridDim.y : KTA, KL = KT - 1;
     const int kt_off = SK ? (int)blockIdx.y * KT : 0;
@@ -230,35 +230,42 @@
     const int d_g = (lane & 3) ^ ((lane >> 4) & 3);
     const unsigned a_off = (unsigned)((lane >> 2) * 64 + d_g * 16);
     const int rb_last = (M - 1) >> 4;
-    int rb0 = m0 / 16 + wave, rb1 = rb0 + 8;
-    rb0 = rb0 < rb_last ? rb0 : rb_last;
-    rb1 = rb1 < rb_last ? rb1 : rb_last;
-    const unsigned char* const a_base[2] = {(const unsigned char*)Ablk + ((size_t)rb0 * KTA + kt_off) * 2048, (const unsigned char*)Ablk + ((size_t)rb1 * KTA + kt_off) * 2048};
-    const unsigned char* const w_base = (const unsigned char*)(Wp + ((size_t)nb * KTA + kt_off) * (W_BYTES / 2) + (size_t)wave * 512);
     const unsigned w_off = lane * 16;
     const unsigned lds0 = (unsigned)(size_t)(__attribute__((address_space(3))) unsigned char*)smem;
-    auto dma_a = [&](int kt, int stage) {
-        kt = kt < KL ? kt : KL;
+    int pa_t = blockIdx.x, pa_k = 0, pw_t = blockIdx.x, pw_k = 0;
+    const unsigned char *pa0, *pa1, *pw;
+    auto a_tile = [&](int t) {
+        int mb, nb;
+        tile_of_workgroup(t, T, mblocks, nblocks, mb, nb);
+        int rb0 = mb * (BM / 16) + wave, rb1 = rb0 + 8;
+        rb0 = rb0 < rb_last ? rb0 : rb_last;
+        rb1 = rb1 < rb_last ? rb1 : rb_last;
+        pa0 = (const unsigned char*)Ablk + ((size_t)rb0 * KTA + kt_off) * 2048;
+        pa1 = (const unsigned char*)Ablk + ((size_t)rb1 * KTA + kt_off) * 2048;
+    };
+    auto w_tile = [&](int t) {
+        int mb, nb;
+        tile_of_workgroup(t, T, mblocks, nblocks, mb, nb);
+        pw = (const unsigned char*)(Wp + ((size_t)nb * KTA + kt_off) * (W_BYTES / 2) + (size_t)wave * 512);
+    };
+    a_tile(pa_t);
+    w_tile(pw_t);
+    auto dma_a = [&](int stage) {
         const unsigned dst = lds0 + stage * PA_BYTES + wave * 1024;
 #pragma unroll
-        for (int j = 0; j < 4; ++j) lds_dma16(a_base[j & 1] + (size_t)kt * 2048 + (j >> 1) * 1024, a_off, dst + (j & 1) * 8192 + (j >> 1) * PA_P);
-    };
-    auto dma_w = [&](int kt, int stage) {
-        kt = kt < KL ? kt : KL;
-        const unsigned char* src = w_base + (size_t)kt * W_BYTES;
+        for (int j = 0; j < 4; ++j) lds_dma16(((j & 1) ? pa1 : pa0) + (j >> 1) * 1024, a_off, dst + (j & 1) * 8192 + (j >> 1) * PA_P);
+        if (pa_k < KL) { ++pa_k; pa0 += 2048; pa1 += 2048; }
+        else if (pa_t + G < T) { pa_t += G; pa_k = 0; a_tile(pa_t); }
+    };
+    auto dma_w = [&](int stage) {
         const unsigned dst = lds0 + PW_BASE + stage * W_BYTES + wave * 1024;
-        lds_dma16(src, w_off, dst);
-        lds_dma16(src + 8 * 1024, w_off, dst + 8 * 1024);
+        lds_dma16(pw, w_off, dst);
+        lds_dma16(pw + 8 * 1024, w_off, dst + 8 * 1024);
+        if (pw_k < KL) { ++pw_k; pw += W_BYTES; }
+        else if (pw_t + G < T) { pw_t += G; pw_k = 0; w_tile(pw_t); }
     };
 
     f32x16v hi[2][2], lo[2][2];
-#pragma unroll
-    for (int i = 0; i < 2; ++i)
-#pragma unroll
-        for (int j = 0; j < 2; ++j) {
-            hi[i][j] = f32x16v{0, 0, 0, 0, 0, 0, 0, 0, 0, 0, 0, 0, 0, 0, 0, 0};
-            lo[i][j] = hi[i][j];
-        }
 
     const int a_frag = (wm * 64 + l31) * PA_ROW + ((lh ^ ((l31 >> 2) & 3)) * 16);
     const int w_frag = PW_BASE + lh * W_G + (wn * 64 + l31) * 16;
@@ -283,9 +290,9 @@
             }
     };
 
-    auto iteration = [&](int kt, int a_cur, int a_next, int a_new, int w_cur, int w_next, int w_new) {
-        dma_a(kt + 2, a_new);
-        dma_w(kt + 3, w_new);
+    auto iteration = [&](int a_cur, int a_next, int a_new, int w_cur, int w_next, int w_new) {
+        dma_a(a_new);
+        dma_w(w_new);
         __builtin_amdgcn_sched_barrier(0);
         read_frags(af1, wf1, a_cur, w_cur, 1);
         mfma_row(0, af0, wf0);
@@ -301,152 +308,176 @@
         __builtin_amdgcn_sched_barrier(0);
     };
 
-    dma_a(0, 0);
-    dma_w(0, 0);
-    dma_w(1, 1);
-    dma_a(1, 1);
-    dma_w(2, 2);
+    dma_a(0);
+    dma_w(0);
+    dma_w(1);
+    dma_a(1);
+    dma_w(2);
     __builtin_amdgcn_sched_barrier(0);
     asm volatile("s_waitcnt vmcnt(8)" ::: "memory");
     __builtin_amdgcn_s_barrier();
     __builtin_amdgcn_sched_barrier(0);
 
     int ac = 0, wc = 0;
-    if (PP == 0) {
-        read_frags(af0, wf0, 0, 0, 0);
-        for (int kt = 0; kt < KT; ++kt) {
-            const int a1 = ac == 2 ? 0 : ac + 1, a2 = a1 == 2 ? 0 : a1 + 1;
-            iteration(kt, ac, a1, a2, wc, (wc + 1) & 3, (wc + 3) & 3);
-            ac = a1;
-            wc = (wc + 1) & 3;
-        }
-    } else {
-        const int grp = wave >> 2;
-        if (ABL & 2048) tk1 = __builtin_readcyclecounter();
-        if (grp) __builtin_amdgcn_s_barrier();
-        if (!(ABL & 64) && grp) __builtin_amdgcn_s_setprio(1);
-        unsigned long long t0 = 0, t1 = 0, t2 = 0, t3 = 0, t4 = 0;
-        unsigned acc_reads = 0, acc_vm = 0, acc_bar1 = 0, acc_mfma = 0, acc_bar2 = 0;
+    const int grp = wave >> 2;
+    if (PP == 0) read_frags(af0, wf0, 0, 0, 0);
+    else if (!(ABL & 64) && grp) __builtin_amdgcn_s_setprio(1);
+    float chk = 0.f;
+    unsigned long long t0 = 0, t1 = 0, t2 = 0, t3 = 0, t4 = 0, tkp = tk0;
+    unsigned acc_reads = 0, acc_vm = 0, acc_bar1 = 0, acc_mfma = 0, acc_bar2 = 0, cyc_pre = 0, cyc_loop = 0, cyc_epi = 0, walked = 0;
+
+    for (int tile = blockIdx.x; tile < T; tile += G) {
+        int mb, nb;
+        tile_of_workgroup(tile, T, mblocks, nblocks, mb, nb);
+        const int m0 = mb * BM, n0 = nb * BN;
+#pragma unroll
+        for (int i = 0; i < 2; ++i)
+#pragma unroll
+            for (int j = 0; j < 2; ++j) {
+                hi[i][j] = f32x16v{0, 0, 0, 0, 0, 0, 0, 0, 0, 0, 0, 0, 0, 0, 0, 0};
+                lo[i][j] = hi[i][j];
+            }
+        if (PP == 0) {
+            for (int kt = 0; kt < KT; ++kt) {
+                const int a1 = ac == 2 ? 0 : ac + 1, a2 = a1 == 2 ? 0 : a1 + 1;
+                iteration(ac, a1, a2, wc, (wc + 1) & 3, (wc + 3) & 3);
+                ac = a1;
+                wc = (wc + 1) & 3;
+            }
+        } else {
+            if (ABL & 2048) { tk1 = __builtin_readcyclecounter(); cyc_pre += (unsigned)(tk1 - tkp); }
+            if (grp) __builtin_amdgcn_s_barrier();
 #define STAMP(t) do { if (ABL & 2048) { __builtin_amdgcn_sched_barrier(0); t = __builtin_readcyclecounter(); __builtin_amdgcn_sched_barrier(0); } } while (0)
-        for (int kt = 0; kt < KT; ++kt) {
-            const int a1 = ac == 2 ? 0 : ac + 1, a2 = a1 == 2 ? 0 : a1 + 1;
-            STAMP(t0);
-            if ((ABL & 2048) && kt > 0) acc_bar2 += (unsigned)(t0 - t4);
-            __builtin_amdgcn_sched_barrier(0);
-            if (!(ABL & 16)) {
-                read_frags(af0, wf0, ac, wc, 0);
-                read_frags(af1, wf1, ac, wc, 1);
-            }
-            __builtin_amdgcn_sched_barrier(0);
-            if (!(ABL & 1)) dma_a(kt + 2, a2);
-            if (!(ABL & 4)) dma_w(kt + 3, (wc + 3) & 3);
-            __builtin_amdgcn_sched_barrier(0);
-            if (ABL & 2048) {
-                asm volatile("s_waitcnt lgkmcnt(0)" ::: "memory");
-                STAMP(t1);
-            }
-            if (ABL & 5) asm volatile("s_waitcnt vmcnt(0) lgkmcnt(0)" ::: "memory");
-            else asm volatile("s_waitcnt vmcnt(8) lgkmcnt(0)" ::: "memory");
-            STAMP(t2);
-            if (!(ABL & 32)) __builtin_amdgcn_s_barrier();
-            STAMP(t3);
-            __builtin_amdgcn_sched_barrier(0);
-            if (!(ABL & 8)) {
-                mfma_row(0, af0, wf0);
-                mfma_row(1, af0, wf0);
-                mfma_row(0, af1, wf1);
-                mfma_row(1, af1, wf1);
-            }
-            __builtin_amdgcn_sched_barrier(0);
-            STAMP(t4);
-            if (ABL & 2048) { acc_reads += (unsigned)(t1 - t0); acc_vm += (unsigned)(t2 - t1); acc_bar1 += (unsigned)(t3 - t2); acc_mfma += (unsigned)(t4 - t3); }
-            if (!(ABL & 32) && !(grp && kt == KL)) __builtin_amdgcn_s_barrier();
-            ac = a1;
-            wc = (wc + 1) & 3;
-        }
+            for (int kt = 0; kt < KT; ++kt) {
+                const int a1 = ac == 2 ? 0 : ac + 1, a2 = a1 == 2 ? 0 : a1 + 1;
+                STAMP(t0);
+                if ((ABL & 2048) && kt > 0) acc_bar2 += (unsigned)(t0 - t4);
+                __builtin_amdgcn_sched_barrier(0);
+                if (!(ABL & 16)) {
+                    read_frags(af0, wf0, ac, wc, 0);
+                    read_frags(af1, wf1, ac, wc, 1);
+                }
+                __builtin_amdgcn_sched_barrier(0);
+                if (!(ABL & 1)) dma_a(a2);
+                if (!(ABL & 4)) dma_w((wc + 3) & 3);
+                __builtin_amdgcn_sched_barrier(0);
+                if (ABL & 2048) {
+                    asm volatile("s_waitcnt lgkmcnt(0)" ::: "memory");
+                    STAMP(t1);
+                }
+                if (ABL & 5) asm volatile("s_waitcnt vmcnt(0) lgkmcnt(0)" ::: "memory");
+                else asm volatile("s_waitcnt vmcnt(8) lgkmcnt(0)" ::: "memory");
+                STAMP(t2);
+                if (!(ABL & 32)) __builtin_amdgcn_s_barrier();
+                STAMP(t3);
+                __builtin_amdgcn_sched_barrier(0);
+                if (!(ABL & 8)) {
+                    mfma_row(0, af0, wf0);
+                    mfma_row(1, af0, wf0);
+                    mfma_row(0, af1, wf1);
+                    mfma_row(1, af1, wf1);
+                }
+                __builtin_amdgcn_sched_barrier(0);
+                STAMP(t4);
+                if (ABL & 2048) { acc_reads += (unsigned)(t1 - t0); acc_vm += (unsigned)(t2 - t1); acc_bar1 += (unsigned)(t3 - t2); acc_mfma += (unsigned)(t4 - t3); }
+                if (!(ABL & 32) && !(grp && kt == KL)) __builtin_amdgcn_s_barrier();
+                ac = a1;
+                wc = (wc + 1) & 3;
+            }
 #undef STAMP
-        if (ABL & 2048) tk2 = __builtin_readcyclecounter();
-        if ((ABL & 2048) && blockIdx.x == gridDim.x / 2 && lane == 0) {
-            float* dbg = const_cast<float*>(bias) + N + wave * 8;
-            dbg[0] = (float)acc_reads / KT; dbg[1] = (float)acc_vm / KT; dbg[2] = (float)acc_bar1 / KT;
-            dbg[3] = (float)acc_mfma / KT; dbg[4] = (float)acc_bar2 / (KT - 1);
-            dbg[5] = (float)(tk1 - tk0); dbg[6] = (float)(tk2 - tk1);
-        }
-    }
-    asm volatile("s_waitcnt vmcnt(0)" ::: "memory");
-
-    constexpr int STG_ROW = OSPLIT ? 144 : 272, STG_PLANE = 64 * STG_ROW;
-    unsigned char* stg = smem + wave * (OSPLIT ? 2 * STG_PLANE : STG_PLANE);
-    __syncthreads();
-    float chk = 0.f;
-#pragma unroll
-    for (int j = 0; j < 2; ++j) {
-#pragma unroll
-        for (int g = 0; g < 4; ++g) {
-            const int cl = j * 32 + 8 * g + 4 * lh, col = n0 + wn * 64 + cl;
-            const float4 bv = bias ? *reinterpret_cast<const float4*>(bias + col) : make_float4(0.f, 0.f, 0.f, 0.f);
+            if (ABL & 2048) { tk2 = __builtin_readcyclecounter(); cyc_loop += (unsigned)(tk2 - tk1); }
+        }
+
+        constexpr int STG_ROW = OSPLIT ? 80 : 144, STG_PLANE = 32 * STG_ROW, STG_SLOT = 5120;
+        static_assert((OSPLIT ? 2 : 1) * STG_PLANE <= STG_SLOT && 6 * STG_SLOT <= PA_BYTES && 2 * STG_SLOT <= W_BYTES, "epilogue slots");
+        unsigned char* stg = wave < 6 ? smem + (ac == 0 ? PA_STAGES - 1 : ac - 1) * PA_BYTES + wave * STG_SLOT
+                                      : smem + PW_BASE + ((wc + PW_STAGES - 1) & 3) * W_BYTES + (wave - 6) * STG_SLOT;
+        asm volatile("s_waitcnt vmcnt(0)" ::: "memory");
+#pragma unroll
+        for (int j = 0; j < 2; ++j) {
+            float4 bv[4];
+#pragma unroll
+            for (int g = 0; g < 4; ++g)
+                bv[g] = bias ? *reinterpret_cast<const float4*>(bias + n0 + wn * 64 + j * 32 + 8 * g + 4 * lh) : make_float4(0.f, 0.f, 0.f, 0.f);
 #pragma unroll
             for (int i = 0; i < 2; ++i) {
-                const int rl = i * 32 + l31, row = m0 + wm * 64 + rl;
-                float v[4];
-#pragma unroll
-                for (int c = 0; c < 4; ++c) {
-                    v[c] = hi[i][j][4 * g + c] + lo[i][j][4 * g + c] * LO_INV + (c == 0 ? bv.x : c == 1 ? bv.y : c == 2 ? bv.z : bv.w);
-                    if (ACT == 1) v[c] = gelu_tanh_f(v[c]);
-                }
-                if (OSPLIT) {
-                    f16x4 h, l;
-                    split4(make_float4(opaque_f32(v[0]), opaque_f32(v[1]), opaque_f32(v[2]), opaque_f32(v[3])), h, l);
-                    *reinterpret_cast<f16x4*>(stg + rl * STG_ROW + cl * 2) = h;
-                    *reinterpret_cast<f16x4*>(stg + STG_PLANE + rl * STG_ROW + cl * 2) = l;
-                    if (row < M) {
-#pragma unroll
-                        for (int c = 0; c < 4; ++c) chk = __builtin_fmaf((float)h[c], 0.f, chk);
+                const int rq = m0 + wm * 64 + i * 32, cq = n0 + wn * 64 + j * 32;
+#pragma unroll
+                for (int g = 0; g < 4; ++g) {
+                    const int cl = 8 * g + 4 * lh, row = rq + l31;
+                    float v[4];
+#pragma unroll
+                    for (int c = 0; c < 4; ++c) {
+                        v[c] = hi[i][j][4 * g + c] + lo[i][j][4 * g + c] * LO_INV + (c == 0 ? bv[g].x : c == 1 ? bv[g].y : c == 2 ? bv[g].z : bv[g].w);
+                        if (ACT == 1) v[c] = gelu_tanh_f(v[c]);
                     }
-                } else {
-                    *reinterpret_cast<float4*>(stg + rl * STG_ROW + cl * 4) = make_float4(v[0], v[1], v[2], v[3]);
-                    if (row < M) {
-#pragma unroll
-                        for (int c = 0; c < 4; ++c) chk = __builtin_fmaf(v[c], 0.f, chk);
+                    if (OSPLIT) {
+                        f16x4 h, l;
+                        split4(make_float4(opaque_f32(v[0]), opaque_f32(v[1]), opaque_f32(v[2]), opaque_f32(v[3])), h, l);
+                        *reinterpret_cast<f16x4*>(stg + l31 * STG_ROW + cl * 2) = h;
+                        *reinterpret_cast<f16x4*>(stg + STG_PLANE + l31 * STG_ROW + cl * 2) = l;
+                        if (row < M) {
+#pragma unroll
+                            for (int c = 0; c < 4; ++c) chk = __builtin_fmaf((float)h[c], 0.f, chk);
+                        }
+                    } else {
+                        *reinterpret_cast<float4*>(stg + l31 * STG_ROW + cl * 4) = make_float4(v[0], v[1], v[2], v[3]);
+                        if (row < M) {
+#pragma unroll
+                            for (int c = 0; c < 4; ++c) chk = __builtin_fmaf(v[c], 0.f, chk);
+                        }
                     }
                 }
-            }
-        }
-    }
-    if (OSPLIT) {
-#pragma unroll
-        for (int p = 0; p < 2; ++p)
-#pragma unroll
-            for (int pass = 0; pass < 8; ++pass) {
-                const int rl = pass * 8 + (lane >> 3), seg = lane & 7, row = m0 + wm * 64 + rl;
-                const f16x8 val = *reinterpret_cast<const f16x8*>(stg + p * STG_PLANE + rl * STG_ROW + seg * 16);
-                if (row < M) *reinterpret_cast<f16x8*>(oblk + split_blk_index(row, n0 + wn * 64 + seg * 8, p, N / 32)) = val;
-            }
-    } else {
-#pragma unroll
-        for (int pass = 0; pass < 16; ++pass) {
-            const int rl = pass * 4 + (lane >> 4), seg = lane & 15, row = m0 + wm * 64 + rl;
-            float4 val = *reinterpret_cast<const float4*>(stg + rl * STG_ROW + seg * 16);
-            if (row < M) {
-                const int col = n0 + wn * 64 + seg * 4;
-                if (RES) {
-                    const float4 r = *reinterpret_cast<const float4*>(res.resid + (size_t)row * res.ldr + col);
-                    if (res.gate) {
-                        const int b = row / res.T, t = row - b * res.T;
-                        const float4 g = *reinterpret_cast<const float4*>(res.gate + b * res.gsb + t * res.gst + col);
-                        val.x = r.x + g.x * val.x; val.y = r.y + g.y * val.y; val.z = r.z + g.z * val.z; val.w = r.w + g.w * val.w;
-                    } else {
-                        val.x += r.x; val.y += r.y; val.z += r.z; val.w += r.w;
+                __builtin_amdgcn_fence(__ATOMIC_ACQ_REL, "wavefront");
+                if (OSPLIT) {
+#pragma unroll
+                    for (int p = 0; p < 2; ++p)
+#pragma unroll
+                        for (int pass = 0; pass < 2; ++pass) {
+                            const int rl = pass * 16 + (lane >> 2), seg = lane & 3, row = rq + rl;
+                            const f16x8 val = *reinterpret_cast<const f16x8*>(stg + p * STG_PLANE + rl * STG_ROW + seg * 16);
+                            if (row < M) *reinterpret_cast<f16x8*>(oblk + split_blk_index(row, cq + seg * 8, p, N / 32)) = val;
+                        }
+                } else {
+#pragma unroll
+                    for (int pass = 0; pass < 4; ++pass) {
+                        const int rl = (pass >> 1) * 16 + (pass & 1) * 4 + ((lane >> 3) & 1) * 8 + (lane >> 4), seg = lane & 7, row = rq + rl;
+                        float4 val = *reinterpret_cast<const float4*>(stg + rl * STG_ROW + seg * 16);
+                        if (row < M) {
+                            const int col = cq + seg * 4;
+                            if (RES) {
+                                const float4 r = *reinterpret_cast<const float4*>(res.resid + (size_t)row * res.ldr + col);
+                                if (res.gate) {
+                                    const int b = row / res.T, t = row - b * res.T;
+                                    const float4 g = *reinterpret_cast<const float4*>(res.gate + b * res.gsb + t * res.gst + col);
+                                    val.x = r.x + g.x * val.x; val.y = r.y + g.y * val.y; val.z = r.z + g.z * val.z; val.w = r.w + g.w * val.w;
+                                } else {
+                                    val.x += r.x; val.y += r.y; val.z += r.z; val.w += r.w;
+                                }
+                            }
+                            *reinterpret_cast<float4*>(out + (size_t)row * ldo + col) = val;
+                        }
                     }
                 }
-                *reinterpret_cast<float4*>(out + (size_t)row * ldo + col) = val;
-            }
-        }
-    }
+                __builtin_amdgcn_fence(__ATOMIC_ACQ_REL, "wavefront");
+            }
+        }
+        if (ABL & 2048) {
+            asm volatile("s_waitcnt vmcnt(0)" ::: "memory");
+            tkp = __builtin_readcyclecounter();
+            cyc_epi += (unsigned)(tkp - tk2);
+            ++walked;
+        }
+        if (tile + G < T) __syncthreads();
+    }
+
     if (overflow && chk != 0.f) atomicOr(overflow, 1);
-    if ((ABL & 2048) && blockIdx.x == gridDim.x / 2 && lane == 0) {
-        asm volatile("s_waitcnt vmcnt(0)" ::: "memory");
-        const_cast<float*>(bias)[N + wave * 8 + 7] = (float)(__builtin_readcyclecounter() - tk2);
+    if ((ABL & 2048) && PP && blockIdx.x == gridDim.x / 2 && lane == 0) {
+        float* dbg = const_cast<float*>(bias) + N + wave * 8;
+        const float its = (float)KT * walked;
+        dbg[0] = (float)acc_reads / its; dbg[1] = (float)acc_vm / its; dbg[2] = (float)acc_bar1 / its;
+        dbg[3] = (float)acc_mfma / its; dbg[4] = (float)acc_bar2 / ((float)(KT - 1) * walked);
+        dbg[5] = (float)cyc_pre / walked; dbg[6] = (float)cyc_loop / walked; dbg[7] = (float)cyc_epi / walked;
     }
     if ((ABL & 2048) && overflow && tid == 0) {
         asm volatile("s_waitcnt vmcnt(0)" ::: "memory");
@@ -536,6 +567,25 @@
     if (overflow && chk != 0.f) atomicOr(overflow, 1);
 }
 
+static std::atomic<int> g_walk_cap{0};
+
+static int walk_workgroups(int tiles)
+{
+    int cap = g_walk_cap.load(std::memory_order_relaxed);
+    if (cap <= 0) {
+        static std::atomic<int> cus[64];
+        int dev = 0;
+        if (hipGetDevice(&dev) != hipSuccess || dev < 0 || dev >= 64) dev = 0;
+        cap = cus[dev].load(std::memory_order_relaxed);
+        if (cap <= 0) {
+            int n = 0;
+            if (hipDeviceGetAttribute(&n, hipDeviceAttributeMultiprocessorCount, dev) != hipSuccess || n <= 0) n = 256;
+            cus[dev].store(cap = n, std::memory_order_relaxed);
+        }
+    }
+    return tiles < cap ? tiles : cap;
+}
+
 static int launch_splitk_partials(const void* a_blk, const void* packed, float* ws, int M, int N, int K, int ksplit, int* overflow, hipStream_t stream)
 {
     const int mblocks = (M + BM - 1) / BM, nblocks = N / BN;
@@ -612,7 +662,7 @@
     if (rc != SELFTOK_OK || M == 0) return rc;
     const bool osplit = out_blk != nullptr;
     const int mblocks = (M + BM - 1) / BM, nblocks = N / BN;
-    const dim3 grid((unsigned)(mblocks * nblocks));
+    const dim3 grid((unsigned)walk_workgroups(mblocks * nblocks));
     const _Float16* ab = (const _Float16*)a_blk;
     _Float16* ob = (_Float16*)out_blk;
 #ifdef SELFTOK_GEMM_ABLATE
@@ -638,7 +688,7 @@
     const int rc = check_split_linear_residual("linear_f16x2_split_residual", a_blk, packed, bias, resid, ldr, gate, gate_stride_b, gate_stride_t, T, out, ldo, M, N, K);
     if (rc != SELFTOK_OK || M == 0) return rc;
     const int mblocks = (M + BM - 1) / BM, nblocks = N / BN;
-    hipLaunchKernelGGL((linear_f16x2_pre_kernel<0, 0, 1, 0, 1>), dim3((unsigned)(mblocks * nblocks)), dim3(512), 0, stream,
+    hipLaunchKernelGGL((linear_f16x2_pre_kernel<0, 0, 1, 0, 1>), dim3((unsigned)walk_workgroups(mblocks * nblocks)), dim3(512), 0, stream,
                        (const _Float16*)a_blk, (const _Float16*)packed, bias, out, (_Float16*)nullptr, ldo,
                        M, N, K, overflow, mblocks, nblocks, ResArgs{resid, ldr, gate, gate_stride_b, gate_stride_t, T});
     return check_launch("linear_f16x2_pre_kernel(residual)");
@@ -666,6 +716,11 @@
 
 extern "C" {
 
+int selftok_linear_f16x2_walk_cap(int cap)
+{
+    return g_walk_cap.exchange(cap > 0 ? cap : 0, std::memory_order_relaxed);
+}
+
 size_t selftok_linear_f16x2_splitk_workspace_bytes(int M, int N, int ksplit)
 {
     if (M <= 0 || N <= 0 || ksplit <= 1) return 0;
diff --git a/selftoktokenizer_amd/csrc/gemm_split_shared.h b/selftoktokenizer_amd/csrc/gemm_split_shared.h
--- a/selftoktokenizer_amd/csrc/gemm_split_shared.h
+++ b/selftoktokenizer_amd/csrc/gemm_split_shared.h
@@ -18,9 +18,8 @@
 constexpr int W_BYTES = 2 * W_P;
 constexpr int GROUP_M = 4;
 
-__device__ __forceinline__ void tile_of_workgroup(int mblocks, int nblocks, int& mb, int& nb)
+__device__ __forceinline__ void tile_of_workgroup(int orig, int T, int mblocks, int nblocks, int& mb, int& nb)
 {
-    const int T = gridDim.x, orig = blockIdx.x;
     const int q8 = T >> 3, r8 = T & 7, xcd = orig & 7, idx = orig >> 3;
     const int w = (xcd < r8 ? xcd * (q8 + 1) : r8 * (q8 + 1) + (xcd - r8) * q8) + idx;
     const int per_group = GROUP_M * nblocks;
diff --git a/selftoktokenizer_amd/ops.py b/selftoktokenizer_amd/ops.py
--- a/selftoktokenizer_amd/ops.py
+++ b/selftoktokenizer_amd/ops.py
@@ -363,6 +363,10 @@
     _lib.check(getattr(lib, name)(_p(xs.data), _p(packed), _p(bias), None if out_split else _p(out), _p(out.data) if out_split else None, N, M, N, K,
                                   LINEAR_GELU if gelu else 0, *tail), name)
     return out if out_split else out.reshape(*lead, N)
+
+
+def linear_f16x2_walk_cap(cap: int = 0) -> int:
+    return int(_lib.load().selftok_linear_f16x2_walk_cap(int(cap)))
 
 
 def linear_f16x2_split(xs: SplitAct, packed: torch.Tensor, bias, N: int, gelu: bool = False, overflow: torch.Tensor = None,
```

After: 3.205 (median of 2 runs). No clear change (+0.0%).
